# freewym/espresso

Hardware: AMD Instinct MI355X
Metric: audio-hours/sec training (LibriSpeech Conformer-12 + CTC) (higher is better)
Workload: dtype bf16

## Files before the change

### espresso_amd/csrc/engine.hip

```cpp
#include <hip/hip_runtime.h>
#include <stdint.h>
#include <stdlib.h>
#include <string.h>

#include <functional>
#include <cstdio>
#include <map>
#include <mutex>
#include <vector>

#include "espresso_amd.h"

void ea_gemm_corun_hint(int on);

namespace {

struct Arena {
  char* base;
  size_t off;
  size_t peak;
  template <typename T>
  T* get(size_t n) {
    off = (off + 255) & ~(size_t)255;
    T* p = base ? reinterpret_cast<T*>(base + off) : nullptr;
// ... 435 lines not shown

static bool keep_bits_on_side(Ctx& c, const AttnSaved& a, const EaLayerShape& sh, uint64_t seed, const EaAttnParams* w = nullptr,
                              const void* pe = nullptr) {
  if (!(a.bits && attn_fused(sh) && !c.dry && c.rc == 0 && g_flash_bits_side && side_init(c.s))) return false;
  hipEvent_t e0 = g_side.ev[g_side.next];
  g_side.next = (g_side.next + 1) % 32;
  if (hipEventRecord(e0, c.s) != hipSuccess || hipStreamWaitEvent(g_side.stream, e0, 0) != hipSuccess) c.rc = -1;
  RUN(ea_flash_keep_bits(a.bits, sh.H, sh.B, sh.T, seed + kProbs, drop_thr(sh.p_attn), g_side.stream));
  if (w && pe && sh.pos_mode != 1) {
    const int R = 2 * sh.T - 1, C = sh.C;
    G gpp(pe, w->wpos, a.pp, R, C, C, C, C, C);
    gemm_on(c, gpp, g_side.stream);
    c.pp_early = true;
  }
  return true;
}

static void attn_fwd(Ctx& c, const AttnSaved& a, const EaLayerShape& sh, const EaAttnParams& w, const void* x, void* y,
                     const int* key_len, const float* attn_mask, const void* pe, uint64_t seed) {
  const int B = sh.B, T = sh.T, C = sh.C, H = sh.H, M = B * T, dh = C / H, Z = H * B, Sp = pad8(T), R = 2 * T - 1, Rp = pad8(R);
  const float scaling = 1.0f / sqrtf((float)dh);
  Arena& sc = *c.scratch;
  const size_t mark = sc.off;
  bool bits_on_side = c.bits_early;
  c.bits_early = false;
  if (!bits_on_side) bits_on_side = keep_bits_on_side(c, a, sh, seed);
  RUN(ea_layernorm_fwd(x, w.ln_g, w.ln_b, a.xn, a.mean, a.rstd, M, C, 1e-5f, nullptr, 0, 0, 1.f, c.s));
  G gq(a.xn, w.wqkv, a.qkv, M, 3 * C, C, C, C, 3 * C);
  gq.bias(w.bqkv);
  const bool learned = sh.pos_mode == 1;
  const uint16_t* pp = learned ? (const uint16_t*)pe : a.pp;
  const uint16_t* qvv = learned ? a.qu : a.qv;
  const bool split = learned ? gq.qsplit(a.qu, nullptr, nullptr, nullptr, C, C, scaling)
                             : gq.qsplit(a.qu, a.qv, w.pos_u, w.pos_v, C, C, scaling);
  gemm(c, gq);
  if (!split) {
    if (learned) RUN(ea_relpos_q_prep(a.qkv, 3 * C, nullptr, nullptr, a.qu, nullptr, M, C, scaling, c.s));
    else RUN(ea_relpos_q_prep(a.qkv, 3 * C, w.pos_u, w.pos_v, a.qu, a.qv, M, C, scaling, c.s));
  }
  if (attn_fused(sh)) {
    if (!learned && !c.pp_early) {
      G gpp(pe, w.wpos, a.pp, R, C, C, C, C, C);
      gemm(c, gpp);
    }
    c.pp_early = false;
    if (bits_on_side) {
      hipEvent_t e1 = g_side.ev[g_side.next];
      g_side.next = (g_side.next + 1) % 32;
      if (c.rc == 0 && (hipEventRecord(e1, g_side.stream) != hipSuccess || hipStreamWaitEvent(c.s, e1, 0) != hipSuccess)) c.rc = -1;
    }
    RUN(ea_flash_attention_fwd(a.qu, qvv, C, a.qkv + C, a.qkv + 2 * C, 3 * C, pp, C, key_len, a.o, C, a.lse, H, B, T, T, dh,
                               bits_on_side ? 4 : 0, seed + kProbs, drop_thr(sh.p_attn), drop_scale(sh.p_attn), a.bits, c.s));
    G go(a.o, w.wo, y, M, C, C, C, C, C);
    go.bias(w.bo).drop(sh.p_drop, seed + kAttnOut).resid(x, C);
    gemm(c, go);
    sc.off = mark;
    return;
  }
  float* ac = sc.get<float>((size_t)Z * T * Sp);
  float* bd = sc.get<float>((size_t)Z * T * Rp);
  G gac(a.qu, a.qkv + C, ac, T, T, dh, C, 3 * C, Sp);
  gac.f32().batch(Z, B, dh, (long)T * C, dh, (long)T * 3 * C, (long)B * T * Sp, (long)T * Sp);
  gemm(c, gac);
  if (!learned) {
    G gpp(pe, w.wpos, a.pp, R, C, C, C, C, C);
    gemm(c, gpp);
  }
  G gbd(qvv, pp, bd, T, R, dh, C, C, Rp);
  gbd.f32().batch(Z, B, dh, (long)T * C, dh, 0, (long)B * T * Rp, (long)T * Rp);
  gemm(c, gbd);
  RUN(ea_relpos_softmax_fwd(ac, bd, key_len, attn_mask, a.P, sh.p_attn > 0.f ? a.Pd : nullptr, H, B, T, T, Sp, Rp, Sp, 0,
                            seed + kProbs, drop_thr(sh.p_attn), drop_scale(sh.p_attn), c.s));
  G gpv(a.Pd, a.qkv + 2 * C, a.o, T, dh, T, Sp, 3 * C, C);
  gpv.bks().batch(Z, B, (long)B * T * Sp, (long)T * Sp, dh, (long)T * 3 * C, dh, (long)T * C);
  gemm(c, gpv);
  G go(a.o, w.wo, y, M, C, C, C, C, C);
  go.bias(w.bo).drop(sh.p_drop, seed + kAttnOut).resid(x, C);
  gemm(c, go);
  sc.off = mark;
}

static void attn_bwd_tail(Ctx& c, const AttnSaved& a, const EaLayerShape& sh, const EaAttnParams& w, const EaAttnGrads& gw,
                          const void* x, const void* dy, void* dx, const void* pe, uint16_t* dqkv, uint16_t* t1, uint16_t* t2,
                          uint16_t* dBD, const uint16_t* wqkvt, const Pre& next, float* dpe, bool have_dq = false) {
  const int B = sh.B, T = sh.T, C = sh.C, H = sh.H, M = B * T, dh = C / H, R = 2 * T - 1, Rp = pad_bd(R);
  Arena& sc = *c.scratch;
  const bool learned = sh.pos_mode == 1;
  const int tiles = ((R + 127) / 128) * H;
  int sk = (768 + tiles - 1) / tiles;
  if (sk > (B * T) / 256) sk = (B * T) / 256;
  if (sk < 1) sk = 1;
  if (learned) {
    G gpp(dBD, a.qu, dpe, R, dh, B * T, Rp, C, C);
    gpp.aks().bks().f32().batch(H, 1, (long)B * T * Rp, 0, dh, 0, dh, 0);
    gpp.p.splitk = sk;
    if (sk > 1) gpp.p.workspace = sc.get<float>((size_t)sk * H * R * dh);
    if (c.df) {
      gemm(c, gpp);
    } else {
      fork(c);
      gemm_on(c, gpp, wstream(c));
    }
  } else {
    float* dppT32 = sc.get<float>((size_t)C * Rp);
    uint16_t* dppT = sc.get<uint16_t>((size_t)C * Rp);
    G gpp(a.qv, dBD, dppT32, dh, R, B * T, C, Rp, Rp);
    gpp.aks().bks().f32().batch(H, 1, dh, 0, (long)B * T * Rp, 0, (long)dh * Rp, 0);
    gpp.p.splitk = sk;
    if (sk > 1) gpp.p.workspace = sc.get<float>((size_t)sk * H * R * dh);
    const int wt_tiles = ((C + 63) / 64) * ((C + 127) / 128);
    int sk2 = (512 + wt_tiles - 1) / wt_tiles;
    if (sk2 > R / 256) sk2 = R / 256;
    if (sk2 < 1) sk2 = 1;
    G gw2(dppT, pe, gw.wpos, C, C, R, Rp, C, C);
    gw2.bks().f32().acc();
    gw2.p.splitk = sk2;
    if (sk2 > 1) gw2.p.workspace = sc.get<float>((size_t)sk2 * C * C);
    static const bool gpp_grouped = getenv("EA_GPP_SPLITK") == nullptr;
    const bool in_group = c.df && gpp_grouped && dh % 64 == 0 && c.df->grp.count + H + 3 <= EA_WGRAD_MAX;
    if (in_group) {
      for (int h = 0; h < H; ++h) {
        EaWgradProblem& q = c.df->grp.p[c.df->grp.count++];
        if (c.dry) continue;
        q.dy = a.qv + (size_t)h * dh; q.x = dBD + (size_t)h * B * T * Rp; q.dW = dppT32 + (size_t)h * dh * Rp; q.dbias = nullptr;
        q.M = B * T; q.N = dh; q.K = R; q.ld_dy = C; q.ld_x = Rp; q.ldw = Rp;
      }
      if (!c.dry) {
        const EaGemmParams p2 = gw2.p;
        const long ncast = (long)C * Rp;
        c.df->pre.push_back([=](hipStream_t st) { return hipMemsetAsync(dppT32, 0, (size_t)ncast * sizeof(float), st) == hipSuccess ? 0 : -1; });
        c.df->ops.push_back([=](hipStream_t st) {
          int rc = ea_cast_f32_to_bf16(dppT32, dppT, ncast, st);
          if (rc == 0) rc = ea_gemm_bf16(&p2, st);
          return rc;
        });
      }
    } else if (c.df) {
      if (!c.dry) {
        const EaGemmParams p1 = gpp.p, p2 = gw2.p;
        const long ncast = (long)C * Rp;
        c.df->ops.push_back([=](hipStream_t st) {
          int rc = ea_gemm_bf16(&p1, st);
          if (rc == 0) rc = ea_cast_f32_to_bf16(dppT32, dppT, ncast, st);
          if (rc == 0) rc = ea_gemm_bf16(&p2, st);
          return rc;
        });
      }
    } else {
      fork(c);
      gemm_on(c, gpp, wstream(c));
      RUN(ea_cast_f32_to_bf16(dppT32, dppT, (long)C * Rp, wstream(c)));
      gemm_on(c, gw2, wstream(c));
    }
    bias_grad(c, t1, gw.pos_u, M, C, C);
    bias_grad(c, t2, gw.pos_v, M, C, C);
  }
  if (!have_dq) RUN(ea_add2_strided_bf16(t1, C, t2, C, dqkv, 3 * C, M, C, c.s));
  fork(c);
  wgrad(c, dqkv, 3 * C, a.xn, C, gw.wqkv, M, 3 * C, C, gw.bqkv);
  uint16_t* dxn = sc.get<uint16_t>((size_t)M * C);
  dgrad(c, dqkv, w.wqkv, wqkvt, dxn, M, C, 3 * C);
  ln_bwd_block(c, x, dxn, w.ln_g, a.mean, a.rstd, dx, gw.ln_g, gw.ln_b, M, C, dy, next);
}

static void attn_bwd(Ctx& c, const AttnSaved& a, const EaLayerShape& sh, const EaAttnParams& w, const EaAttnGrads& gw, const void* x,
                     const void* dy, void* dx, const int* key_len, const void* pe, uint64_t seed, const uint16_t* wqkvt,
                     const uint16_t* wot, const uint16_t* pre, const Pre& next, float* dpe = nullptr) {
  const int B = sh.B, T = sh.T, C = sh.C, H = sh.H, M = B * T, dh = C / H, Z = H * B, Sp = pad8(T), R = 2 * T - 1, Rp = pad_bd(R);
  const float scaling = 1.0f / sqrtf((float)dh);
  Arena& sc = *c.scratch;
  const size_t mark = sc.off;
  const void* g = dy;
  if (pre) {
    g = pre;
  } else if (sh.p_drop > 0.f) {
    uint16_t* gg = sc.get<uint16_t>((size_t)M * C);
    RUN(ea_scale_dropout_bf16(dy, nullptr, gg, (long)M * C, 1.f, 0.f, seed + kAttnOut, drop_thr(sh.p_drop), drop_scale(sh.p_drop), c.s));
    g = gg;
  }
  fork(c);
  wgrad(c, g, C, a.o, C, gw.wo, M, C, C, gw.bo);
  uint16_t* dO = sc.get<uint16_t>((size_t)M * C);
  dgrad(c, g, w.wo, wot, dO, M, C, C);
  if (attn_fused(sh)) {
    uint16_t* dqkv = sc.get<uint16_t>((size_t)M * 3 * C);
    uint16_t* t1 = sc.get<uint16_t>((size_t)M * C);
    uint16_t* t2 = sc.get<uint16_t>((size_t)M * C);
    uint16_t* dBD = sc.get<uint16_t>((size_t)Z * T * Rp);
    float* Dd = sc.get<float>((size_t)Z * T);
    static const bool fused_dq = getenv("EA_NO_FUSED_DQ") == nullptr;
    RUN(ea_flash_attention_bwd(a.qu, sh.pos_mode == 1 ? a.qu : a.qv, C, a.qkv + C, a.qkv + 2 * C, 3 * C,
                               sh.pos_mode == 1 ? (const uint16_t*)pe : a.pp, C, key_len, a.o, dO, C, a.lse, Dd, t1, t2, C, dBD,
                               Rp, dqkv + C, dqkv + 2 * C, 3 * C, H, B, T, T, dh, (sh.scratch_clean && c.overlap) ? 2 : 0, scaling, seed + kProbs,
                               drop_thr(sh.p_attn),
                               drop_scale(sh.p_attn), a.bits, fused_dq ? dqkv : nullptr, 3 * C, c.s));
    attn_bwd_tail(c, a, sh, w, gw, x, dy, dx, pe, dqkv, t1, t2, dBD, wqkvt, next, dpe, fused_dq);
    release(c, mark);
    return;
  }
  float* dPd = sc.get<float>((size_t)Z * T * Sp);
  G gdp(dO, a.qkv + 2 * C, dPd, T, T, dh, C, 3 * C, Sp);
  gdp.f32().batch(Z, B, dh, (long)T * C, dh, (long)T * 3 * C, (long)B * T * Sp, (long)T * Sp);
  gemm(c, gdp);
  uint16_t* dqkv = sc.get<uint16_t>((size_t)M * 3 * C);
  G gdv(a.Pd, dO, dqkv + 2 * C, T, dh, T, Sp, C, 3 * C);
  gdv.aks().bks().batch(Z, B, (long)B * T * Sp, (long)T * Sp, dh, (long)T * C, dh, (long)T * 3 * C);
  gemm(c, gdv);
  uint16_t* dAC = sc.get<uint16_t>((size_t)Z * T * Sp);
  uint16_t* dBD = sc.get<uint16_t>((size_t)Z * T * Rp);
  RUN(ea_relpos_softmax_bwd(a.P, dPd, dAC, dBD, H, B, T, T, Sp, Sp, Rp, seed + kProbs, drop_thr(sh.p_attn), drop_scale(sh.p_attn), c.s));
  G gdk(dAC, a.qu, dqkv + C, T, dh, T, Sp, C, 3 * C);
  gdk.aks().bks().batch(Z, B, (long)B * T * Sp, (long)T * Sp, dh, (long)T * C, dh, (long)T * 3 * C);
  gemm(c, gdk);
  uint16_t* t1 = sc.get<uint16_t>((size_t)M * C);
  G gt1(dAC, a.qkv + C, t1, T, dh, T, Sp, 3 * C, C);
  gt1.bks().alpha(scaling).batch(Z, B, (long)B * T * Sp, (long)T * Sp, dh, (long)T * 3 * C, dh, (long)T * C);
  gemm(c, gt1);
  uint16_t* t2 = sc.get<uint16_t>((size_t)M * C);
  G gt2(dBD, sh.pos_mode == 1 ? (const uint16_t*)pe : a.pp, t2, T, dh, R, Rp, C, C);
  gt2.bks().alpha(scaling).batch(Z, B, (long)B * T * Rp, (long)T * Rp, dh, 0, dh, (long)T * C);
  gemm(c, gt2);
  attn_bwd_tail(c, a, sh, w, gw, x, dy, dx, pe, dqkv, t1, t2, dBD, wqkvt, next, dpe);
  release(c, mark);
}

struct BnRing {
  double* st[2] = {nullptr, nullptr};
  float* red[2] = {nullptr, nullptr};
  int si = 0, ri = 0, cap = 0;
  bool ok = false, failed = false, dirty = false;
};
static std::mutex g_bn_mu;
static std::map<std::pair<int, hipStream_t>, BnRing> g_bn_rings;
static BnRing* bn_ring(hipStream_t owner, int C) {
  int cur = 0, dev = 0;
  if (hipGetDevice(&cur) != hipSuccess) return nullptr;
  dev = cur;
  if (owner != nullptr) {
    hipDevice_t d;
    if (hipStreamGetDevice(owner, &d) == hipSuccess) dev = (int)d;
  }
  std::lock_guard<std::mutex> lk(g_bn_mu);
  BnRing& R = g_bn_rings[std::make_pair(dev, owner)];
  if (R.failed) return nullptr;
  if (!R.ok) {
    const int cap = 2048;
    if (dev != cur && hipSetDevice(dev) != hipSuccess) { R.failed = true; return nullptr; }
    const size_t bytes = 2 * (size_t)(2 * cap) * (sizeof(double) + sizeof(float));
    char* base = nullptr;
    const bool ok = hipMalloc(reinterpret_cast<void**>(&base), bytes) == hipSuccess && hipMemsetAsync(base, 0, bytes, owner) == hipSuccess;
    if (dev != cur) (void)hipSetDevice(cur);
    if (!ok) { R.failed = true; return nullptr; }
    R.st[0] = reinterpret_cast<double*>(base);
    R.st[1] = R.st[0] + 2 * cap;
    R.red[0] = reinterpret_cast<float*>(R.st[1] + 2 * cap);
    R.red[1] = R.red[0] + 2 * cap;
    R.cap = cap;
    R.ok = true;
  }
  if (C > R.cap) return nullptr;
  if (R.dirty) {
    const size_t bytes = 2 * (size_t)(2 * R.cap) * (sizeof(double) + sizeof(float));
    if (hipMemsetAsync(R.st[0], 0, bytes, owner) != hipSuccess) return nullptr;
    R.dirty = false;
  }
  return &R;
}

struct ConvSaved {
  float *mean, *rstd, *mr;
  uint16_t *xn, *Y, *U, *Z, *Hh;
};
static ConvSaved conv_saved(Arena& sv, const EaLayerShape& sh) {
  const int M = sh.B * sh.T, C = sh.C;
  ConvSaved s;
  s.mean = sv.get<float>(M);
  s.rstd = sv.get<float>(M);
  s.mr = sv.get<float>(2 * C);
  s.xn = sv.get<uint16_t>((size_t)M * C);
  s.Y = sv.get<uint16_t>((size_t)M * 2 * C);
  s.U = sv.get<uint16_t>((size_t)M * C);
  s.Z = sv.get<uint16_t>((size_t)M * C);
  s.Hh = sv.get<uint16_t>((size_t)M * C);
  return s;
}

static void conv_fwd(Ctx& c, const ConvSaved& s, const EaLayerShape& sh, const EaConvParams& w, const void* x, void* y, uint64_t seed) {
  const int B = sh.B, T = sh.T, C = sh.C, M = B * T;
  Arena& sc = *c.scratch;
  const size_t mark = sc.off;
  RUN(ea_layernorm_fwd(x, w.ln_g, w.ln_b, s.xn, s.mean, s.rstd, M, C, 1e-5f, nullptr, 0, 0, 1.f, c.s));
  G g1(s.xn, w.pw1, s.Y, M, 2 * C, C, C, C, 2 * C);
  gemm(c, g1);
  static const bool bn_fused = getenv("EA_BN_UNFUSED") == nullptr;
  const bool ring = sh.training && bn_fused && C <= 2048;
  BnRing* R = nullptr;
  if (ring && !c.dry && c.rc == 0 && !(R = bn_ring(c.s, C))) c.rc = -1;
  double* stats = nullptr;
  if (sh.training && !ring) {
    stats = sc.get<double>(2 * C);
    if (!c.dry && c.rc == 0) c.rc = hipMemsetAsync(stats, 0, 2 * C * sizeof(double), c.s) == hipSuccess ? 0 : -1;
  }
  if (R && c.rc == 0) stats = R->st[R->si];
  RUN(ea_glu_dwconv_fwd(s.Y, w.dw, s.U, s.Z, stats, B, T, C, sh.KW, c.s));
  if (ring) {
    if (R) {
      if (c.rc == 0) RUN(ea_bn_act_fwd_train(s.Z, stats, s.mr, w.bn_rm, w.bn_rv, w.bn_g, w.bn_b, s.Hh, M, C, EA_ACT_SILU, (float)M, 1e-5f, 0.1f,
                                             R->st[R->si ^ 1], 2 * R->cap, c.s));
      if (c.rc == 0) R->si ^= 1;
      else R->dirty = true;
    }
  } else {
    if (sh.training) RUN(ea_bn_finalize(stats, s.mr, w.bn_rm, w.bn_rv, C, (float)M, 1e-5f, 0.1f, c.s));
    else RUN(ea_bn_from_running(w.bn_rm, w.bn_rv, s.mr, C, 1e-5f, c.s));
    RUN(ea_bn_act_fwd(s.Z, s.mr, w.bn_g, w.bn_b, s.Hh, M, C, EA_ACT_SILU, c.s));
  }
  G g2(s.Hh, w.pw2, y, M, C, C, C, C, C);
  g2.drop(sh.p_drop, seed + kConvOut).resid(x, C);
  gemm(c, g2);
  sc.off = mark;
}

static void conv_bwd(Ctx& c, const ConvSaved& s, const EaLayerShape& sh, const EaConvParams& w, const EaConvGrads& gw, const void* x,
                     const void* dy, void* dx, uint64_t seed, const uint16_t* pw1t, const uint16_t* pw2t, const uint16_t* pre,
                     const Pre& next) {
  const int B = sh.B, T = sh.T, C = sh.C, M = B * T;
  Arena& sc = *c.scratch;
  const size_t mark = sc.off;
  const void* g = dy;
  if (pre) {
    g = pre;
  } else if (sh.p_drop > 0.f) {
    uint16_t* gg = sc.get<uint16_t>((size_t)M * C);
    RUN(ea_scale_dropout_bf16(dy, nullptr, gg, (long)M * C, 1.f, 0.f, seed + kConvOut, drop_thr(sh.p_drop), drop_scale(sh.p_drop), c.s));
    g = gg;
  }
  fork(c);
  wgrad(c, g, C, s.Hh, C, gw.pw2, M, C, C);
  uint16_t* dH = sc.get<uint16_t>((size_t)M * C);
  dgrad(c, g, w.pw2, pw2t, dH, M, C, C);
  static const bool bn_fused = getenv("EA_BN_UNFUSED") == nullptr;
  const bool ring = bn_fused && C <= 2048;
  BnRing* R = nullptr;
  if (ring && !c.dry && c.rc == 0 && !(R = bn_ring(c.s, C))) c.rc = -1;
  float* red = nullptr;
  if (!ring) {
    red = sc.get<float>(2 * C);
    if (!c.dry && c.rc == 0) c.rc = hipMemsetAsync(red, 0, 2 * C * sizeof(float), c.s) == hipSuccess ? 0 : -1;
  }
// ... 670 lines not shown
```

### espresso_amd/csrc/flash_attention.hip

```cpp
#include "common.h"
#include "espresso_amd.h"
#include "flash_internal.h"

namespace {

typedef short bf16x4_t __attribute__((ext_vector_type(4)));

constexpr int DH = 64;
constexpr int TQ = 64, TK = 64;
constexpr int ROWB = DH * 2;
constexpr int BDP = 18;

__device__ __forceinline__ uint32_t off16(int row, int chunk) { return (uint32_t)(row * ROWB + ((chunk ^ (row & 7)) << 4)); }




__device__ __forceinline__ int xcd_remap(int id, int total) {
  const int xcd = id & 7, q = total >> 3, r = total & 7;
  return (xcd < r ? xcd * (q + 1) : r * (q + 1) + (xcd - r) * q) + (id >> 3);
}

template <int NP>
struct RowRegs { uint4 v[NP]; };
template <int NP>
__device__ __forceinline__ void load_rows(RowRegs<NP>& r, const bf16_t* src, long ld, int row0, int limit, int tid) {
#pragma unroll
  for (int p = 0; p < NP; ++p) {
    const int g = row0 + (tid >> 3) + 32 * p;
    r.v[p] = make_uint4(0, 0, 0, 0);
    if (g >= 0 && g < limit) r.v[p] = *reinterpret_cast<const uint4*>(src + (long)g * ld + (tid & 7) * 8);
  }
}
template <int NP>
__device__ __forceinline__ void store_rows(char* s, const RowRegs<NP>& r, int tid) {
#pragma unroll
  for (int p = 0; p < NP; ++p) *reinterpret_cast<uint4*>(s + off16((tid >> 3) + 32 * p, tid & 7)) = r.v[p];
}
struct BlkRegs { uint4 v[4]; };
__device__ __forceinline__ void load_blk(BlkRegs& r, const bf16_t* src, long ld, int row0, int limit, int t) {
#pragma unroll
  for (int jj = 0; jj < 4; ++jj) {
    const int g = row0 + (t >> 3) * 4 + jj;
    r.v[jj] = make_uint4(0, 0, 0, 0);
    if (g >= 0 && g < limit) r.v[jj] = *reinterpret_cast<const uint4*>(src + (long)g * ld + (t & 7) * 8);
  }
}
__device__ __forceinline__ void store_blk_rows(char* s, const BlkRegs& r, int t) {
#pragma unroll
  for (int jj = 0; jj < 4; ++jj) *reinterpret_cast<uint4*>(s + off16((t >> 3) * 4 + jj, t & 7)) = r.v[jj];
}
template <int NR>
__device__ __forceinline__ void store_blk_t(char* s, const BlkRegs& r, int t) {
  const int rq = t >> 3, dc = t & 7;
  const uint32_t w[4][4] = {{r.v[0].x, r.v[0].y, r.v[0].z, r.v[0].w}, {r.v[1].x, r.v[1].y, r.v[1].z, r.v[1].w},
                            {r.v[2].x, r.v[2].y, r.v[2].z, r.v[2].w}, {r.v[3].x, r.v[3].y, r.v[3].z, r.v[3].w}};
#pragma unroll
  for (int q = 0; q < 4; ++q) {
    uint2 lo, hi;
    lo.x = (w[0][q] & 0xffffu) | (w[1][q] << 16);
    lo.y = (w[2][q] & 0xffffu) | (w[3][q] << 16);
    hi.x = (w[0][q] >> 16) | (w[1][q] & 0xffff0000u);
    hi.y = (w[2][q] >> 16) | (w[3][q] & 0xffff0000u);
    const int d = dc * 8 + 2 * q;
    *reinterpret_cast<uint2*>(s + d * (NR * 2) + ((rq ^ (d & 15)) << 3)) = lo;
    *reinterpret_cast<uint2*>(s + (d + 1) * (NR * 2) + ((rq ^ ((d + 1) & 15)) << 3)) = hi;
  }
}
template <int NR>
__device__ __forceinline__ bf16x4_t read_t(const char* s, int d, int chunk) {
  return *reinterpret_cast<const bf16x4_t*>(s + d * (NR * 2) + ((chunk ^ (d & 15)) << 3));
}

__device__ __forceinline__ f32x4_t mfma32(bf16x8_t a, bf16x8_t b, f32x4_t c) {
  return __builtin_amdgcn_mfma_f32_16x16x32_bf16(__builtin_bit_cast(__attribute__((ext_vector_type(8))) __bf16, a),
                                                 __builtin_bit_cast(__attribute__((ext_vector_type(8))) __bf16, b), c, 0, 0, 0);
}
__device__ __forceinline__ f32x4_t mfma16(bf16x4_t a, bf16x4_t b, f32x4_t c) {
  return __builtin_amdgcn_mfma_f32_16x16x16bf16_1k(a, b, c, 0, 0, 0);
}

template <bool RELPOS>
__global__ __launch_bounds__(256, 2) void flash_fwd_kernel(const FlashFwdArgs a) {
  __shared__ __attribute__((aligned(16))) char sK[TK * ROWB];
  __shared__ __attribute__((aligned(16))) char sVt[DH * ROWB];
  __shared__ __attribute__((aligned(16))) char sPP[RELPOS ? 128 * ROWB : 16];
  __shared__ float sBD[RELPOS ? 4 * 80 * BDP : 1];

  const int tid = threadIdx.x, lane = tid & 63, w = tid >> 6;
  const int li = lane & 15, g4 = lane >> 4;
  const int vid = xcd_remap(blockIdx.x, gridDim.x);
  const int z = vid / a.nq, qt = vid % a.nq;
  const int h = z / a.B, b = z % a.B;
  const int T = a.T, S = a.S;
  const int i0 = qt * TQ;
  const int i = i0 + 16 * w + li;
  const int kl = a.klen ? min(a.klen[b], S) : S;

  bf16x8_t qu[2], qv[2];
#pragma unroll
  for (int ks = 0; ks < 2; ++ks) {
    uint4 u = make_uint4(0, 0, 0, 0), v = make_uint4(0, 0, 0, 0);
    if (i < T) {
      const long o = ((long)b * T + i) * a.ldq + h * DH + ks * 32 + g4 * 8;
      u = *reinterpret_cast<const uint4*>(a.qu + o);
      if (RELPOS) v = *reinterpret_cast<const uint4*>(a.qv + o);
    }
    qu[ks] = __builtin_bit_cast(bf16x8_t, u);
    qv[ks] = __builtin_bit_cast(bf16x8_t, v);
  }

  f32x4_t acc_o[4];
#pragma unroll
  for (int dt = 0; dt < 4; ++dt) acc_o[dt] = (f32x4_t){0.f, 0.f, 0.f, 0.f};
  float m_run = -INFINITY, l_run = 0.f;

  const bf16_t* Kb = a.k + (long)b * S * a.ldkv + h * DH;
  const bf16_t* Vb = a.v + (long)b * S * a.ldkv + h * DH;
  const bf16_t* PPb = RELPOS ? a.pp + h * DH : nullptr;
  const int R = 2 * T - 1;
  float* bd = sBD + (RELPOS ? w * 80 * BDP : 0);
  const int c0w = 48 - 16 * w;

  int jend = kl;
  if (a.causal) jend = min(jend, i0 + TQ + (S - T));
  RowRegs<2> rK;
  BlkRegs rV;
  RowRegs<4> rP;
  auto load_tile = [&](int j0) {
    load_rows<2>(rK, Kb, a.ldkv, j0, S, tid);
    if (tid < 128) load_blk(rV, Vb, a.ldkv, j0, S, tid);
    if (RELPOS) load_rows<4>(rP, PPb, a.ldpp, (T - 1) - (i0 + TQ - 1) + j0, R, tid);
  };
  if (jend > 0) load_tile(0);
  for (int j0 = 0; j0 < jend; j0 += TK) {
    __syncthreads();
    store_rows<2>(sK, rK, tid);
    if (tid < 128) store_blk_t<64>(sVt, rV, tid);
    if (RELPOS) store_rows<4>(sPP, rP, tid);
    __syncthreads();
    if (j0 + TK < jend) load_tile(j0 + TK);

    f32x4_t acc_s[4];
#pragma unroll
    for (int jt = 0; jt < 4; ++jt) acc_s[jt] = (f32x4_t){0.f, 0.f, 0.f, 0.f};
#pragma unroll
    for (int ks = 0; ks < 2; ++ks)
#pragma unroll
      for (int jt = 0; jt < 4; ++jt) {
        const bf16x8_t kf = *reinterpret_cast<const bf16x8_t*>(sK + off16(jt * 16 + li, ks * 4 + g4));
        acc_s[jt] = mfma32(kf, qu[ks], acc_s[jt]);
      }
    if (RELPOS) {
#pragma unroll
      for (int ct = 0; ct < 5; ++ct) {
// ... 364 lines not shown
  if (j0 >= kl) ibeg = T;
  BlkRegs rQ;
  RowRegs<2> rQv;
  RowRegs<4> rP;
  float rLse = 0.f, rD = 0.f;
  auto load_tile = [&](int i0) {
    if (tid < 128) load_blk(rQ, Qub, a.ldq, i0, T, tid);
    else load_blk(rQ, dOb, a.ldo, i0, T, tid - 128);
    if (RELPOS) {
      load_rows<2>(rQv, Qvb, a.ldq, i0, T, tid);
      load_rows<4>(rP, PPb, a.ldpp, (T - 1) - (i0 + TQ - 1) + j0, R, tid);
    }
    if (tid < TQ) {
      const int ii = i0 + tid;
      rLse = ii < T ? a.lse[(long)z * T + ii] : 0.f;
      rD = ii < T ? a.D[(long)z * T + ii] : 0.f;
    }
  };
  if (ibeg < T) load_tile(ibeg);
  for (int i0 = ibeg; i0 < T; i0 += TQ) {
    __syncthreads();
    if (tid < 128) {
      store_blk_rows(sQu, rQ, tid);
      store_blk_t<64>(sQut, rQ, tid);
    } else {
      store_blk_rows(sdO, rQ, tid - 128);
      store_blk_t<64>(sdOt, rQ, tid - 128);
    }
    if (RELPOS) {
      store_rows<2>(sQv, rQv, tid);
      store_rows<4>(sPP, rP, tid);
    }
    if (tid < TQ) {
      sLse[tid] = rLse;
      sD[tid] = rD;
    }
    __syncthreads();
    if (i0 + TQ < T) load_tile(i0 + TQ);

#pragma unroll
    for (int it = 0; it < 4; ++it) {
      f32x4_t s = (f32x4_t){0.f, 0.f, 0.f, 0.f}, dp = s;
#pragma unroll
      for (int ks = 0; ks < 2; ++ks) {
        const bf16x8_t qf = *reinterpret_cast<const bf16x8_t*>(sQu + off16(it * 16 + li, ks * 4 + g4));
        s = mfma32(qf, kf[ks], s);
        const bf16x8_t gf = *reinterpret_cast<const bf16x8_t*>(sdO + off16(it * 16 + li, ks * 4 + g4));
        dp = mfma32(gf, vf[ks], dp);
      }
      if (RELPOS) {
        const int cbase = 48 - 16 * it + 16 * w;
        wave_lds_sync();
#pragma unroll
        for (int ct = 0; ct < 2; ++ct) {
          f32x4_t t = (f32x4_t){0.f, 0.f, 0.f, 0.f};
#pragma unroll
          for (int ks = 0; ks < 2; ++ks) {
            const bf16x8_t qf = *reinterpret_cast<const bf16x8_t*>(sQv + off16(it * 16 + li, ks * 4 + g4));
            const bf16x8_t pf = *reinterpret_cast<const bf16x8_t*>(sPP + off16(cbase + ct * 16 + li, ks * 4 + g4));
            t = mfma32(qf, pf, t);
          }
#pragma unroll
          for (int r = 0; r < 4; ++r) bd[(g4 * 4 + r) * 33 + ct * 16 + li] = t[r];
        }
        wave_lds_sync();
#pragma unroll
        for (int r = 0; r < 4; ++r) s[r] += bd[(g4 * 4 + r) * 33 + 15 - (g4 * 4 + r) + li];
      }
      float ps[4], dsv[4];
#pragma unroll
      for (int r = 0; r < 4; ++r) {
        const int il = it * 16 + g4 * 4 + r;
        const int i = i0 + il;
        const bool masked = j >= kl || i >= T || (a.causal && j > i + (S - T));
        const float p = masked ? 0.f : __expf(s[r] - sLse[il]);
        float keep = 1.f;
        if (a.thr) keep = ea_keep(a.seed, ((uint64_t)z * T + (uint64_t)i) * (uint64_t)S + (uint64_t)j, a.thr, a.inv_keep);
        ps[r] = p * keep;
        dsv[r] = p * (dp[r] * keep - sD[il]);
      }
      const bf16x4_t pb = pack4(ps[0], ps[1], ps[2], ps[3]);
      const bf16x4_t db = pack4(dsv[0], dsv[1], dsv[2], dsv[3]);
#pragma unroll
      for (int dt = 0; dt < 4; ++dt) {
        acc_dv[dt] = mfma16(read_t<64>(sdOt, dt * 16 + li, it * 4 + g4), pb, acc_dv[dt]);
        acc_dk[dt] = mfma16(read_t<64>(sQut, dt * 16 + li, it * 4 + g4), db, acc_dk[dt]);
      }
    }
  }
  if (j < S) {
    bf16_t* ok = a.dk + ((long)b * S + j) * a.lddkv + h * DH;
    bf16_t* ov = a.dv + ((long)b * S + j) * a.lddkv + h * DH;
#pragma unroll
    for (int dt = 0; dt < 4; ++dt) {
      uint2 pk;
      pk.x = pack_bf2(acc_dk[dt][0], acc_dk[dt][1]);
      pk.y = pack_bf2(acc_dk[dt][2], acc_dk[dt][3]);
      *reinterpret_cast<uint2*>(ok + dt * 16 + g4 * 4) = pk;
      pk.x = pack_bf2(acc_dv[dt][0], acc_dv[dt][1]);
      pk.y = pack_bf2(acc_dv[dt][2], acc_dv[dt][3]);
      *reinterpret_cast<uint2*>(ov + dt * 16 + g4 * 4) = pk;
    }
  }
}

}

extern "C" int ea_flash_attention_supported(int dh, int T, int S, int relpos) {
  return dh == DH && T > 0 && S > 0 && (!relpos || T == S);
}

extern "C" long ea_flash_keep_bits_bytes(int H, int B, int T) {
  const long nkt = (T + TK - 1) / TK;
  return (long)H * B * nkt * (nkt * 64) * 4 * (long)sizeof(uint16_t);
}

extern "C" int ea_flash_keep_bits(void* keep_bits, int H, int B, int T, uint64_t drop_seed, uint32_t drop_thr, hipStream_t stream) {
  if (H <= 0 || B <= 0 || T <= 0 || !keep_bits) return keep_bits ? 0 : -2;
  return ea_rp_keep_bits((uint16_t*)keep_bits, H, B, T, drop_seed, drop_thr, stream);
}

extern "C" int ea_flash_attention_fwd(const void* qu, const void* qv, long ldq, const void* k, const void* v, long ldkv,
                                      const void* pp, long ldpp, const int* key_len, void* out, long ldo, float* lse, int H,
                                      int B, int T, int S, int dh, int causal, uint64_t drop_seed, uint32_t drop_thr,
                                      float drop_scale, void* keep_bits, hipStream_t stream) {
  if (H <= 0 || B <= 0 || T <= 0) return 0;
  const bool relpos = qv != nullptr;
  if (!ea_flash_attention_supported(dh, T, S, relpos) || (relpos && !pp)) return -2;
  if ((ldq | ldkv | ldo) % 8 || (relpos && ldpp % 8)) return -2;
  if ((((uintptr_t)qu | (uintptr_t)qv | (uintptr_t)k | (uintptr_t)v | (uintptr_t)pp) & 15) || ((uintptr_t)out & 7)) return -2;
  FlashFwdArgs a;
  a.qu = (const bf16_t*)qu; a.qv = (const bf16_t*)qv; a.ldq = ldq;
  a.k = (const bf16_t*)k; a.v = (const bf16_t*)v; a.ldkv = ldkv;
  a.pp = (const bf16_t*)pp; a.ldpp = ldpp;
  a.klen = key_len;
  a.out = (bf16_t*)out; a.ldo = ldo;
  a.lse = lse;
  a.H = H; a.B = B; a.T = T; a.S = S; a.causal = causal & 1; a.nq = (T + TQ - 1) / TQ;
  a.seed = drop_seed; a.thr = drop_thr; a.inv_keep = drop_scale;
  a.bits = (const uint16_t*)keep_bits;
  if (ea_rp_eligible(relpos, T, S, causal, drop_thr, keep_bits)) {
    if (drop_thr && !(causal & 4)) {
      const int rc = ea_rp_keep_bits((uint16_t*)keep_bits, H, B, T, drop_seed, drop_thr, stream);
      if (rc) return rc;
    }
    return ea_rp_fwd(a, stream);
  }
  const dim3 grid((unsigned)(a.nq * H * B));
  if (relpos) hipLaunchKernelGGL(flash_fwd_kernel<true>, grid, dim3(256), 0, stream, a);
  else hipLaunchKernelGGL(flash_fwd_kernel<false>, grid, dim3(256), 0, stream, a);
  return EA_CHECK_LAUNCH();
}

extern "C" int ea_flash_attention_bwd(const void* qu, const void* qv, long ldq, const void* k, const void* v, long ldkv,
                                      const void* pp, long ldpp, const int* key_len, const void* out, const void* dout, long ldo,
                                      const float* lse, float* D, void* t1, void* t2, long ldt, void* dBD, int ld_bd, void* dk,
                                      void* dv, long lddkv, int H, int B, int T, int S, int dh, int causal, float scaling,
                                      uint64_t drop_seed, uint32_t drop_thr, float drop_scale, const void* keep_bits,
                                      void* dq, long lddq, hipStream_t stream) {
  if (H <= 0 || B <= 0 || T <= 0) return 0;
  const bool relpos = qv != nullptr;
  if (!ea_flash_attention_supported(dh, T, S, relpos)) return -2;
  if (relpos && (!pp || !t2 || !dBD || ld_bd < 2 * T - 1 || ld_bd % 8 || ((uintptr_t)dBD & 15))) return -2;
  if ((ldq | ldkv | ldo | ldt | lddkv) % 8 || (relpos && ldpp % 8)) return -2;
  if (((uintptr_t)qu | (uintptr_t)qv | (uintptr_t)k | (uintptr_t)v | (uintptr_t)pp | (uintptr_t)out | (uintptr_t)dout) & 15) return -2;
  if (((uintptr_t)t1 | (uintptr_t)t2 | (uintptr_t)dk | (uintptr_t)dv | (uintptr_t)dq) & 7) return -2;
  if (dq && (!relpos || lddq % 4)) return -2;
  FlashBwdArgs a;
  a.qu = (const bf16_t*)qu; a.qv = (const bf16_t*)qv; a.ldq = ldq;
  a.k = (const bf16_t*)k; a.v = (const bf16_t*)v; a.ldkv = ldkv;
  a.pp = (const bf16_t*)pp; a.ldpp = ldpp;
  a.klen = key_len;
  a.out = (const bf16_t*)out; a.dout = (const bf16_t*)dout; a.ldo = ldo;
  a.lse = lse; a.D = D;
  a.t1 = (bf16_t*)t1; a.t2 = (bf16_t*)t2; a.ldt = ldt;
  a.dq = (bf16_t*)dq; a.lddq = lddq;
  a.dBD = (bf16_t*)dBD; a.ld_bd = ld_bd;
  a.dk = (bf16_t*)dk; a.dv = (bf16_t*)dv; a.lddkv = lddkv;
  a.H = H; a.B = B; a.T = T; a.S = S; a.causal = causal & 1; a.dbd_prezeroed = (causal >> 1) & 1;
  a.nq = (T + TQ - 1) / TQ; a.nk = (S + TK - 1) / TK;
  a.scaling = scaling;
  a.seed = drop_seed; a.thr = drop_thr; a.inv_keep = drop_scale;
  a.bits = (const uint16_t*)keep_bits;
  if (ea_rp_eligible(relpos, T, S, causal, drop_thr, keep_bits)) return ea_rp_bwd(a, stream);
  const dim3 gq((unsigned)(a.nq * H * B)), gk((unsigned)(a.nk * H * B));
  if (relpos) {
    hipLaunchKernelGGL(flash_bwd_q_kernel<true>, gq, dim3(256), 0, stream, a);
    hipLaunchKernelGGL(flash_bwd_kv_kernel<true>, gk, dim3(256), 0, stream, a);
  } else {
    hipLaunchKernelGGL(flash_bwd_q_kernel<false>, gq, dim3(256), 0, stream, a);
    hipLaunchKernelGGL(flash_bwd_kv_kernel<false>, gk, dim3(256), 0, stream, a);
  }
  return EA_CHECK_LAUNCH();
}
```

### espresso_amd/csrc/flash_internal.h

```cpp
#pragma once
#include "common.h"

struct FlashFwdArgs {
  const bf16_t* qu; const bf16_t* qv; long ldq;
  const bf16_t* k; const bf16_t* v; long ldkv;
  const bf16_t* pp; long ldpp;
  const int* klen;
  bf16_t* out; long ldo;
  float* lse;
  int H, B, T, S, causal, nq;
  uint64_t seed; uint32_t thr; float inv_keep;
  const uint16_t* bits;
};

struct FlashBwdArgs {
  const bf16_t* qu; const bf16_t* qv; long ldq;
  const bf16_t* k; const bf16_t* v; long ldkv;
  const bf16_t* pp; long ldpp;
  const int* klen;
  const bf16_t* out; const bf16_t* dout; long ldo;
  const float* lse;
  float* D;
  bf16_t* t1; bf16_t* t2; long ldt;
  bf16_t* dq; long lddq;
  bf16_t* dBD; int ld_bd;
  bf16_t* dk; bf16_t* dv; long lddkv;
  int H, B, T, S, causal, nq, nk, dbd_prezeroed;
  float scaling;
  uint64_t seed; uint32_t thr; float inv_keep;
  const uint16_t* bits;
  unsigned long long* prof;
  int dbg;
};

bool ea_rp_eligible(bool relpos, int T, int S, int causal, uint32_t thr, const void* bits);
int ea_rp_keep_bits(uint16_t* bits, int H, int B, int T, uint64_t seed, uint32_t thr, hipStream_t stream);
int ea_rp_fwd(const FlashFwdArgs& a, hipStream_t stream);
int ea_rp_bwd(const FlashBwdArgs& a, hipStream_t stream);
```

### espresso_amd/csrc/flash_relpos.hip

```cpp
#include "flash_internal.h"

namespace {

typedef short bf16x4_t __attribute__((ext_vector_type(4)));
typedef const __attribute__((address_space(1))) void* gptr_t;
typedef __attribute__((address_space(3))) void* lptr_t;
typedef __attribute__((address_space(3))) bf16x4_t* lds_b4_t;

constexpr int DH = 64, TQ = 64, TK = 64;
constexpr int IMG = 64 * 128;
constexpr int BDP = 18;
constexpr int BNC = 80 * BDP * 4;
constexpr int OBP = 88;
constexpr int PP_OFF = 4 * IMG, BNC_OFF = 7 * IMG;
constexpr int LDS_BYTES = 7 * IMG + 4 * BNC;
constexpr int AUX_OFF = LDS_BYTES;
constexpr int LDS_BYTES_KV = LDS_BYTES + 1024;
constexpr float LOG2E = 1.4426950408889634f;

__device__ __forceinline__ int swz(int r) { return ((r >> 2) & 1) | (((r >> 1) & 1) << 1) | ((((r >> 2) ^ (r >> 3)) & 1) << 2); }

__device__ __forceinline__ int xcd_remap(int id, int total) {
  const int xcd = id & 7, q = total >> 3, r = total & 7;
  return (xcd < r ? xcd * (q + 1) : r * (q + 1) + (xcd - r) * q) + (id >> 3);
}
__device__ __forceinline__ f32x4_t mfma32(bf16x8_t a, bf16x8_t b, f32x4_t c) {
  return __builtin_amdgcn_mfma_f32_16x16x32_bf16(__builtin_bit_cast(__attribute__((ext_vector_type(8))) __bf16, a),
                                                 __builtin_bit_cast(__attribute__((ext_vector_type(8))) __bf16, b), c, 0, 0, 0);
}
__device__ __forceinline__ f32x4_t mfma16(bf16x4_t a, bf16x4_t b, f32x4_t c) {
  return __builtin_amdgcn_mfma_f32_16x16x16bf16_1k(a, b, c, 0, 0, 0);
}
__device__ __forceinline__ bf16x8_t cat(bf16x4_t lo, bf16x4_t hi) { return __builtin_shufflevector(lo, hi, 0, 1, 2, 3, 4, 5, 6, 7); }
__device__ __forceinline__ bf16x4_t pack4(float a, float b, float c, float d) {
  uint2 pk;
  pk.x = pack_bf2(a, b);
  pk.y = pack_bf2(c, d);
  return __builtin_bit_cast(bf16x4_t, pk);
}
__device__ __forceinline__ uint32_t lds_addr(const void* p) { return (uint32_t)(uintptr_t)p; }
template <int O0, int O1, int O2, int O3>
__device__ __forceinline__ void trr16(const uint32_t (&ad)[4], uint2 (&o)[16]) {
  asm volatile(
      "ds_read_b64_tr_b16 %0, %16 offset:%20\n\tds_read_b64_tr_b16 %1, %16 offset:%21\n\t"
      "ds_read_b64_tr_b16 %2, %16 offset:%22\n\tds_read_b64_tr_b16 %3, %16 offset:%23\n\t"
      "ds_read_b64_tr_b16 %4, %17 offset:%20\n\tds_read_b64_tr_b16 %5, %17 offset:%21\n\t"
      "ds_read_b64_tr_b16 %6, %17 offset:%22\n\tds_read_b64_tr_b16 %7, %17 offset:%23\n\t"
      "ds_read_b64_tr_b16 %8, %18 offset:%20\n\tds_read_b64_tr_b16 %9, %18 offset:%21\n\t"
      "ds_read_b64_tr_b16 %10, %18 offset:%22\n\tds_read_b64_tr_b16 %11, %18 offset:%23\n\t"
      "ds_read_b64_tr_b16 %12, %19 offset:%20\n\tds_read_b64_tr_b16 %13, %19 offset:%21\n\t"
      "ds_read_b64_tr_b16 %14, %19 offset:%22\n\tds_read_b64_tr_b16 %15, %19 offset:%23\n\t"
      "s_waitcnt lgkmcnt(0)"
      : "=&v"(o[0]), "=&v"(o[1]), "=&v"(o[2]), "=&v"(o[3]), "=&v"(o[4]), "=&v"(o[5]), "=&v"(o[6]), "=&v"(o[7]), "=&v"(o[8]),
        "=&v"(o[9]), "=&v"(o[10]), "=&v"(o[11]), "=&v"(o[12]), "=&v"(o[13]), "=&v"(o[14]), "=&v"(o[15])
      : "v"(ad[0]), "v"(ad[1]), "v"(ad[2]), "v"(ad[3]), "i"(O0), "i"(O1), "i"(O2), "i"(O3)
      : "memory");
}
template <int O0, int O1, int O2, int O3>
__device__ __forceinline__ void trr8(const uint32_t (&ad)[2], uint2 (&o)[8]) {
  asm volatile(
      "ds_read_b64_tr_b16 %0, %8 offset:%10\n\tds_read_b64_tr_b16 %1, %8 offset:%11\n\t"
      "ds_read_b64_tr_b16 %2, %8 offset:%12\n\tds_read_b64_tr_b16 %3, %8 offset:%13\n\t"
      "ds_read_b64_tr_b16 %4, %9 offset:%10\n\tds_read_b64_tr_b16 %5, %9 offset:%11\n\t"
      "ds_read_b64_tr_b16 %6, %9 offset:%12\n\tds_read_b64_tr_b16 %7, %9 offset:%13\n\t"
      "s_waitcnt lgkmcnt(0)"
      : "=&v"(o[0]), "=&v"(o[1]), "=&v"(o[2]), "=&v"(o[3]), "=&v"(o[4]), "=&v"(o[5]), "=&v"(o[6]), "=&v"(o[7])
      : "v"(ad[0]), "v"(ad[1]), "i"(O0), "i"(O1), "i"(O2), "i"(O3)
      : "memory");
}
__device__ __forceinline__ void trr20(const uint32_t (&ad)[20], uint2 (&o)[20]) {
  asm volatile(
      "ds_read_b64_tr_b16 %0, %20\n\tds_read_b64_tr_b16 %1, %21\n\tds_read_b64_tr_b16 %2, %22\n\tds_read_b64_tr_b16 %3, %23\n\t"
      "ds_read_b64_tr_b16 %4, %24\n\tds_read_b64_tr_b16 %5, %25\n\tds_read_b64_tr_b16 %6, %26\n\tds_read_b64_tr_b16 %7, %27\n\t"
      "ds_read_b64_tr_b16 %8, %28\n\tds_read_b64_tr_b16 %9, %29\n\tds_read_b64_tr_b16 %10, %30\n\tds_read_b64_tr_b16 %11, %31\n\t"
      "ds_read_b64_tr_b16 %12, %32\n\tds_read_b64_tr_b16 %13, %33\n\tds_read_b64_tr_b16 %14, %34\n\tds_read_b64_tr_b16 %15, %35\n\t"
      "ds_read_b64_tr_b16 %16, %36\n\tds_read_b64_tr_b16 %17, %37\n\tds_read_b64_tr_b16 %18, %38\n\tds_read_b64_tr_b16 %19, %39\n\t"
      "s_waitcnt lgkmcnt(0)"
      : "=&v"(o[0]), "=&v"(o[1]), "=&v"(o[2]), "=&v"(o[3]), "=&v"(o[4]), "=&v"(o[5]), "=&v"(o[6]), "=&v"(o[7]), "=&v"(o[8]),
        "=&v"(o[9]), "=&v"(o[10]), "=&v"(o[11]), "=&v"(o[12]), "=&v"(o[13]), "=&v"(o[14]), "=&v"(o[15]), "=&v"(o[16]),
        "=&v"(o[17]), "=&v"(o[18]), "=&v"(o[19])
      : "v"(ad[0]), "v"(ad[1]), "v"(ad[2]), "v"(ad[3]), "v"(ad[4]), "v"(ad[5]), "v"(ad[6]), "v"(ad[7]), "v"(ad[8]), "v"(ad[9]),
        "v"(ad[10]), "v"(ad[11]), "v"(ad[12]), "v"(ad[13]), "v"(ad[14]), "v"(ad[15]), "v"(ad[16]), "v"(ad[17]), "v"(ad[18]),
        "v"(ad[19])
      : "memory");
}
__device__ __forceinline__ uint2 lds_u2(const char* p) {
  const float* f = reinterpret_cast<const float*>(p);
  return make_uint2(__float_as_uint(f[0]), __float_as_uint(f[1]));
}
__device__ __forceinline__ bf16x8_t cat2(uint2 lo, uint2 hi) {
  return __builtin_bit_cast(bf16x8_t, make_uint4(lo.x, lo.y, hi.x, hi.y));
}
__device__ __forceinline__ void tr_image(const char* img, const uint32_t (&tro)[4], bf16x8_t (&f)[8]) {
  const uint32_t b = lds_addr(img);
  const uint32_t ad[4] = {b + tro[0], b + tro[1], b + tro[2], b + tro[3]};
  uint2 o[16];
  trr16<0, 2048, 4096, 6144>(ad, o);
#pragma unroll
  for (int dt = 0; dt < 4; ++dt) {
    f[dt * 2 + 0] = cat2(o[dt * 4 + 0], o[dt * 4 + 1]);
    f[dt * 2 + 1] = cat2(o[dt * 4 + 2], o[dt * 4 + 3]);
  }
}
__device__ __forceinline__ bf16x8_t ldf(const char* p) { return *reinterpret_cast<const bf16x8_t*>(p); }
__device__ __forceinline__ void wave_lds_sync() {
  __builtin_amdgcn_fence(__ATOMIC_RELEASE, "wavefront");
  __builtin_amdgcn_wave_barrier();
  __builtin_amdgcn_fence(__ATOMIC_ACQUIRE, "wavefront");
}
__device__ __forceinline__ float fexp2(float x) { return __builtin_amdgcn_exp2f(x); }

#ifdef RP_PROF
#define PROF_DECL unsigned long long prof_t = __builtin_amdgcn_s_memtime(); unsigned prof_acc[10] = {0, 0, 0, 0, 0, 0, 0, 0, 0, 0};
#define PROF_MARK(k) { const unsigned long long n_ = __builtin_amdgcn_s_memtime(); prof_acc[k] += (unsigned)(n_ - prof_t); prof_t = n_; }
#define PROF_DUMP(kern) if (a.prof && (threadIdx.x & 63) == 0) { unsigned long long* o_ = a.prof + ((long)(kern) * 8192 + (long)blockIdx.x * 4 + (threadIdx.x >> 6)) * 10; for (int k_ = 0; k_ < 10; ++k_) o_[k_] = prof_acc[k_]; }
#else
#define PROF_DECL
#define PROF_MARK(k)
#define PROF_DUMP(kern)
#endif

struct LaneK {
  int lane, w, li, g4;
  uint32_t offk[2];
  uint32_t tro[4];
  uint32_t bd_w;
  uint32_t bd_r;
};
__device__ __forceinline__ LaneK lane_consts() {
  LaneK L;
  const int tid = threadIdx.x;
  L.lane = tid & 63;
  L.w = __builtin_amdgcn_readfirstlane(tid >> 6);
  L.li = L.lane & 15;
  L.g4 = L.lane >> 4;
#pragma unroll
  for (int ks = 0; ks < 2; ++ks) L.offk[ks] = L.li * 128 + (((ks * 4 + L.g4) ^ swz(L.li)) << 4);
  const int rowl = 4 * L.g4 + (L.li >> 2);
#pragma unroll
  for (int dt = 0; dt < 4; ++dt)
    L.tro[dt] = rowl * 128 + (((dt * 2 + ((L.li & 3) >> 1)) ^ swz(rowl)) << 4) + (L.li & 1) * 8;
  L.bd_w = (L.g4 * 4) * BDP + L.li;
  L.bd_r = (15 - L.li + L.g4 * 4) * BDP + L.li;
  return L;
}

struct ImgSrc {
  const bf16_t* p[2];
  long ld;
  int rmax;
};
__device__ __forceinline__ ImgSrc img_src(const bf16_t* base, long ld, int rmax, int w, int lane) {
  ImgSrc s;
  s.ld = ld;
  s.rmax = rmax;
#pragma unroll
  for (int n = 0; n < 2; ++n) {
    const int r = (w + 4 * n) * 8 + (lane >> 3);
    s.p[n] = base + (long)r * ld + (((lane & 7) ^ swz(r)) << 3);
  }
  return s;
}
__device__ __forceinline__ void issue_img(char* dst, const ImgSrc& s, int row0, int w, int lane) {
  if (row0 >= 0 && row0 + 63 <= s.rmax) {
    const long off = (long)row0 * s.ld;
#pragma unroll
    for (int n = 0; n < 2; ++n)
      __builtin_amdgcn_global_load_lds((gptr_t)(s.p[n] + off), (lptr_t)(dst + (w + 4 * n) * 1024), 16, 0, 0);
  } else {
#pragma unroll
    for (int n = 0; n < 2; ++n) {
      const int r = (w + 4 * n) * 8 + (lane >> 3);
      const int g = min(max(row0 + r, 0), s.rmax);
      __builtin_amdgcn_global_load_lds((gptr_t)(s.p[n] + (long)(g - r) * s.ld), (lptr_t)(dst + (w + 4 * n) * 1024), 16, 0, 0);
    }
  }
}

__device__ __forceinline__ void add_band(f32x4_t (&acc_s)[4], const bf16x8_t (&qv)[2], const char* blk_lo, const char* blk_hi,
                                         float* bd, const LaneK& L) {
  bf16x8_t pf[2][2];
  auto frag = [&](int ct, bf16x8_t (&f)[2]) {
    const int q = ct - L.w + 3;
    const char* p = ((q >> 2) ? blk_hi : blk_lo) + (q & 3) * 2048;
    f[0] = ldf(p + L.offk[0]);
    f[1] = ldf(p + L.offk[1]);
  };
  frag(0, pf[0]);
#pragma unroll
  for (int ct = 0; ct < 5; ++ct) {
    if (ct + 1 < 5) frag(ct + 1, pf[(ct + 1) & 1]);
    f32x4_t t = (f32x4_t){0.f, 0.f, 0.f, 0.f};
    t = mfma32(pf[ct & 1][0], qv[0], t);
    t = mfma32(pf[ct & 1][1], qv[1], t);
#pragma unroll
    for (int r = 0; r < 4; ++r) bd[L.bd_w + (ct * 16 + r) * BDP] = t[r];
    if (ct >= 1) {
      const int jt = ct - 1;
#pragma unroll
      for (int r = 0; r < 4; ++r) acc_s[jt][r] += bd[L.bd_r + (jt * 16 + r) * BDP];
    }
  }
}

__device__ __forceinline__ uint32_t keep_mask(uint32_t piece, int k) { return (uint32_t)__builtin_amdgcn_sbfe((int)piece, k, 1); }
__device__ __forceinline__ float fand(float x, uint32_t m) { return __uint_as_float(__float_as_uint(x) & m); }

__global__ __launch_bounds__(256) void keep_bits_kernel(uint16_t* bits, uint64_t seed, uint32_t thr, int Z, int T, int nkt) {
  const int Tpad = nkt * 64;
  const long n = (long)Z * nkt * Tpad * 4;
  const long stride = (long)gridDim.x * 256;
  for (long id = (long)blockIdx.x * 256 + threadIdx.x; id < n; id += stride) {
    const int g = (int)(id & 3);
    long t = id >> 2;
    const int i = (int)(t % Tpad);
    t /= Tpad;
    const int kt = (int)(t % nkt);
    const int z = (int)(t / nkt);
    uint32_t piece = 0;
    if (i < T) {
      const uint64_t rowbase = ((uint64_t)z * T + (uint64_t)i) * (uint64_t)T;
#pragma unroll
      for (int jt = 0; jt < 4; ++jt)
#pragma unroll
        for (int r = 0; r < 4; ++r) {
          const int j = kt * 64 + jt * 16 + g * 4 + r;
          if (j < T && ea_hash(seed, rowbase + (uint64_t)j) >= thr) piece |= 1u << (jt * 4 + r);
        }
    }
    bits[id] = (uint16_t)piece;
  }
}

template <bool DROP>
__global__ __launch_bounds__(256, 2) void rp_fwd_kernel(const FlashFwdArgs a) {
  __shared__ __attribute__((aligned(16))) char lds[LDS_BYTES];
  const LaneK L = lane_consts();
  const int lane = L.lane, w = L.w, li = L.li, g4 = L.g4;
  const int vid = xcd_remap(blockIdx.x, gridDim.x);
  const int z = vid / a.nq, qt = vid % a.nq;
  const int h = z / a.B, b = z % a.B;
  const int T = a.T;
  const int i0 = qt * TQ;
  const int i = i0 + 16 * w + li;
  const int kl = a.klen ? min(a.klen[b], T) : T;
  const int nt = (kl + TK - 1) / TK;
  const int nkt = (T + TK - 1) / TK;

  bf16x8_t qu[2], qv[2];
  {
    const int ic = min(i, T - 1);
    const long o = ((long)b * T + ic) * a.ldq + h * DH + g4 * 8;
#pragma unroll
    for (int ks = 0; ks < 2; ++ks) {
      qu[ks] = __builtin_bit_cast(bf16x8_t, *reinterpret_cast<const uint4*>(a.qu + o + ks * 32));
      qv[ks] = __builtin_bit_cast(bf16x8_t, *reinterpret_cast<const uint4*>(a.qv + o + ks * 32));
    }
  }
  const bf16_t* Kb = a.k + (long)b * T * a.ldkv + h * DH;
  const bf16_t* Vb = a.v + (long)b * T * a.ldkv + h * DH;
  const bf16_t* PPb = a.pp + h * DH;
  const int R = 2 * T - 1;
  const ImgSrc srcK = img_src(Kb, a.ldkv, T - 1, w, lane), srcV = img_src(Vb, a.ldkv, T - 1, w, lane);
  const ImgSrc srcP = img_src(PPb, a.ldpp, R - 1, w, lane);
  const int pbase = (T - 1) - (i0 + TQ - 1);
  float* bd = reinterpret_cast<float*>(lds + BNC_OFF + w * BNC);
  const uint32_t* bitp = DROP ? reinterpret_cast<const uint32_t*>(a.bits) + (((long)z * nkt) * (nkt * 64) + i) * 2 + (g4 >> 1) : nullptr;
  const long bit_step = (long)nkt * 64 * 2;
  const int ksh = (g4 & 1) * 16;

  f32x4_t acc_o[4];
#pragma unroll
  for (int dt = 0; dt < 4; ++dt) acc_o[dt] = (f32x4_t){0.f, 0.f, 0.f, 0.f};
  float m_run = -INFINITY, l_run = 0.f;
  uint32_t piece = 0, piece_next = 0;

  if (nt > 0) {
    issue_img(lds, srcK, 0, w, lane);
    issue_img(lds + IMG, srcV, 0, w, lane);
    issue_img(lds + PP_OFF, srcP, pbase, w, lane);
    issue_img(lds + PP_OFF + IMG, srcP, pbase + 64, w, lane);
    if (DROP) piece_next = bitp[0];
  }
  int slot_lo = 0;
  for (int t = 0; t < nt; ++t) {
    const int j0 = t * TK;
    asm volatile("s_waitcnt vmcnt(0)" ::: "memory");
    __builtin_amdgcn_s_barrier();
    const int slot_hi = slot_lo == 2 ? 0 : slot_lo + 1;
    const int slot_nx = slot_hi == 2 ? 0 : slot_hi + 1;
    if (DROP) {
      piece = piece_next;
      asm volatile("" : "+v"(piece));
    }
    if (t + 1 < nt) {
      if (DROP) piece_next = bitp[(long)(t + 1) * bit_step];
      char* st = lds + ((t + 1) & 1) * 2 * IMG;
      issue_img(st, srcK, j0 + TK, w, lane);
      issue_img(st + IMG, srcV, j0 + TK, w, lane);
      issue_img(lds + PP_OFF + slot_nx * IMG, srcP, pbase + 64 * (t + 2), w, lane);
    }
    const char* sK = lds + (t & 1) * 2 * IMG;
    const char* sV = sK + IMG;

    f32x4_t acc_s[4];
#pragma unroll
    for (int jt = 0; jt < 4; ++jt) acc_s[jt] = (f32x4_t){0.f, 0.f, 0.f, 0.f};
    {
      bf16x8_t fr[2][2];
      fr[0][0] = ldf(sK + L.offk[0]);
      fr[0][1] = ldf(sK + L.offk[1]);
#pragma unroll
      for (int jt = 0; jt < 4; ++jt) {
        if (jt + 1 < 4) {
          fr[(jt + 1) & 1][0] = ldf(sK + (jt + 1) * 2048 + L.offk[0]);
          fr[(jt + 1) & 1][1] = ldf(sK + (jt + 1) * 2048 + L.offk[1]);
        }
        acc_s[jt] = mfma32(fr[jt & 1][0], qu[0], acc_s[jt]);
        acc_s[jt] = mfma32(fr[jt & 1][1], qu[1], acc_s[jt]);
      }
    }
    add_band(acc_s, qv, lds + PP_OFF + slot_lo * IMG, lds + PP_OFF + slot_hi * IMG, bd, L);

    if (j0 + TK > kl) {
#pragma unroll
      for (int jt = 0; jt < 4; ++jt)
#pragma unroll
        for (int r = 0; r < 4; ++r)
          if (j0 + jt * 16 + g4 * 4 + r >= kl) acc_s[jt][r] = -INFINITY;
    }
    float tmax = fmaxf(fmaxf(acc_s[0][0], acc_s[0][1]), fmaxf(acc_s[0][2], acc_s[0][3]));
#pragma unroll
    for (int jt = 1; jt < 4; ++jt) tmax = fmaxf(tmax, fmaxf(fmaxf(acc_s[jt][0], acc_s[jt][1]), fmaxf(acc_s[jt][2], acc_s[jt][3])));
    tmax = fmaxf(tmax, __shfl_xor(tmax, 16, 64));
    tmax = fmaxf(tmax, __shfl_xor(tmax, 32, 64));
    const float m_new = fmaxf(m_run, tmax);
    const float msc = (m_new == -INFINITY) ? 0.f : m_new * LOG2E;
    const float alpha = fexp2(m_run * LOG2E - msc);
    float psum = 0.f;
#pragma unroll
    for (int jt = 0; jt < 4; ++jt)
#pragma unroll
      for (int r = 0; r < 4; ++r) {
        const float p = fexp2(fmaf(acc_s[jt][r], LOG2E, -msc));
        psum += p;
        acc_s[jt][r] = DROP ? fand(p, keep_mask(piece, ksh + jt * 4 + r)) : p;
      }
    l_run = l_run * alpha + psum;
    m_run = m_new;
#pragma unroll
    for (int dt = 0; dt < 4; ++dt)
#pragma unroll
      for (int r = 0; r < 4; ++r) acc_o[dt][r] *= alpha;

    {
      bf16x8_t vf[8];
      tr_image(sV, L.tro, vf);
#pragma unroll
      for (int kb = 0; kb < 2; ++kb) {
        const bf16x8_t pb = cat(pack4(acc_s[2 * kb][0], acc_s[2 * kb][1], acc_s[2 * kb][2], acc_s[2 * kb][3]),
                                pack4(acc_s[2 * kb + 1][0], acc_s[2 * kb + 1][1], acc_s[2 * kb + 1][2], acc_s[2 * kb + 1][3]));
#pragma unroll
        for (int dt = 0; dt < 4; ++dt) acc_o[dt] = mfma32(vf[dt * 2 + kb], pb, acc_o[dt]);
      }
    }
    slot_lo = slot_hi;
  }

  l_run += __shfl_xor(l_run, 16, 64);
  l_run += __shfl_xor(l_run, 32, 64);
  if (i < T) {
    const float inv = (DROP ? a.inv_keep : 1.f) / l_run;
    bf16_t* o = a.out + ((long)b * T + i) * a.ldo + h * DH;
#pragma unroll
    for (int dt = 0; dt < 4; ++dt) {
      uint2 pk;
      pk.x = pack_bf2(acc_o[dt][0] * inv, acc_o[dt][1] * inv);
      pk.y = pack_bf2(acc_o[dt][2] * inv, acc_o[dt][3] * inv);
      *reinterpret_cast<uint2*>(o + dt * 16 + g4 * 4) = pk;
    }
    if (a.lse && g4 == 0) a.lse[(long)z * T + i] = m_run + __logf(l_run);
  }
}

template <bool DROP, bool WANT_PD>
__device__ __forceinline__ void softmax_bwd_tile(f32x4_t (&acc_s)[4], const f32x4_t (&acc_dp)[4], bf16x4_t (&dsb)[4], bf16x4_t (&pdb)[4],
                                                 float lse2, float Di, float inv_keep, uint32_t piece, int ksh, int jrel_end, int g4) {
#pragma unroll
  for (int jt = 0; jt < 4; ++jt) {
    float ds[4], pd[4];
#pragma unroll
    for (int r = 0; r < 4; ++r) {
      float p = fexp2(fmaf(acc_s[jt][r], LOG2E, -lse2));
      if (jrel_end < 64 && jt * 16 + g4 * 4 + r >= jrel_end) p = 0.f;
      float dp = acc_dp[jt][r];
      if (DROP) {
        const uint32_t m = keep_mask(piece, ksh + jt * 4 + r);
        dp = fand(dp * inv_keep, m);
        if (WANT_PD) pd[r] = fand(p * inv_keep, m);
      } else if (WANT_PD) {
        pd[r] = p;
      }
      ds[r] = p * (dp - Di);
    }
    dsb[jt] = pack4(ds[0], ds[1], ds[2], ds[3]);
    if (WANT_PD) pdb[jt] = pack4(pd[0], pd[1], pd[2], pd[3]);
  }
}

template <bool DROP>
__global__ __launch_bounds__(256, 2) void rp_bwd_q_kernel(const FlashBwdArgs a) {
  __shared__ __attribute__((aligned(16))) char lds[LDS_BYTES];
  const LaneK L = lane_consts();
  const int lane = L.lane, w = L.w, li = L.li, g4 = L.g4;
  const int vid = xcd_remap(blockIdx.x, gridDim.x);
  const int z = vid / a.nq, qt = vid % a.nq;
  const int h = z / a.B, b = z % a.B;
  const int T = a.T;
  const int i0 = qt * TQ;
  const int i = i0 + 16 * w + li;
  const int kl = a.klen ? min(a.klen[b], T) : T;
  const int nt = (kl + TK - 1) / TK;
  const int nkt = (T + TK - 1) / TK;

  bf16x8_t qu[2], qv[2], dO[2];
  float Di = 0.f;
  {
    const int ic = min(i, T - 1);
    const long oq = ((long)b * T + ic) * a.ldq + h * DH + g4 * 8;
    const long oo = ((long)b * T + ic) * a.ldo + h * DH + g4 * 8;
#pragma unroll
    for (int ks = 0; ks < 2; ++ks) {
      qu[ks] = __builtin_bit_cast(bf16x8_t, *reinterpret_cast<const uint4*>(a.qu + oq + ks * 32));
      qv[ks] = __builtin_bit_cast(bf16x8_t, *reinterpret_cast<const uint4*>(a.qv + oq + ks * 32));
      const uint4 g = *reinterpret_cast<const uint4*>(a.dout + oo + ks * 32);
      const uint4 o = *reinterpret_cast<const uint4*>(a.out + oo + ks * 32);
      dO[ks] = __builtin_bit_cast(bf16x8_t, g);
      const uint32_t wg[4] = {g.x, g.y, g.z, g.w}, wo[4] = {o.x, o.y, o.z, o.w};
#pragma unroll
      for (int e = 0; e < 4; ++e)
        Di += __uint_as_float(wg[e] << 16) * __uint_as_float(wo[e] << 16) +
              __uint_as_float(wg[e] & 0xffff0000u) * __uint_as_float(wo[e] & 0xffff0000u);
    }
  }
  Di += __shfl_xor(Di, 16, 64);
  Di += __shfl_xor(Di, 32, 64);
  const float lse2 = (i < T) ? a.lse[(long)z * T + i] * LOG2E : INFINITY;
  if (i < T && g4 == 0 && a.D) a.D[(long)z * T + i] = Di;

  f32x4_t acc_t1[4], acc_t2[4];
#pragma unroll
  for (int dt = 0; dt < 4; ++dt) {
    acc_t1[dt] = (f32x4_t){0.f, 0.f, 0.f, 0.f};
    acc_t2[dt] = (f32x4_t){0.f, 0.f, 0.f, 0.f};
  }
  const bf16_t* Kb = a.k + (long)b * T * a.ldkv + h * DH;
  const bf16_t* Vb = a.v + (long)b * T * a.ldkv + h * DH;
  const bf16_t* PPb = a.pp + h * DH;
  const int R = 2 * T - 1;
  const ImgSrc srcK = img_src(Kb, a.ldkv, T - 1, w, lane), srcV = img_src(Vb, a.ldkv, T - 1, w, lane);
  const ImgSrc srcP = img_src(PPb, a.ldpp, R - 1, w, lane);
  const int pbase = (T - 1) - (i0 + TQ - 1);
  float* bd = reinterpret_cast<float*>(lds + BNC_OFF + w * BNC);
  bf16_t* ob = reinterpret_cast<bf16_t*>(bd);
  const uint32_t* bitp = DROP ? reinterpret_cast<const uint32_t*>(a.bits) + (((long)z * nkt) * (nkt * 64) + i) * 2 + (g4 >> 1) : nullptr;
  const long bit_step = (long)nkt * 64 * 2;
  const int ksh = (g4 & 1) * 16;
  uint2 mlo, mhi;
  {
    uint32_t m[4], n[4];
#pragma unroll
    for (int e = 0; e < 4; ++e) {
      m[e] = (4 * g4 + e >= 15 - li) ? 0xffffu : 0u;
      n[e] = (64 + 4 * g4 + e <= 78 - li) ? 0xffffu : 0u;
    }
    mlo = make_uint2(m[0] | (m[1] << 16), m[2] | (m[3] << 16));
    mhi = make_uint2(n[0] | (n[1] << 16), n[2] | (n[3] << 16));
  }
  const int ob_w = li * (OBP - 1) + 15 + g4 * 4;
  const char* ob_rd = reinterpret_cast<const char*>(ob) + li * (OBP * 2) + g4 * 8;

  uint32_t piece = 0, piece_next = 0;
  int jcov = 0;
  uint32_t dbd_pk[8];
  int dbd_j0 = -1;
  auto store_dbd = [&]() {
    const int j = dbd_j0 + lane;
    if (dbd_j0 >= 0 && j < T) {
      const int row_w = i0 + 16 * w, nrow = T - row_w;
      bf16_t* dp = a.dBD + ((long)z * T + row_w) * a.ld_bd + (T - 1 - row_w) + j;
      if (nrow >= 16) {
#pragma unroll
        for (int iw = 0; iw < 16; ++iw) dp[(long)iw * (a.ld_bd - 1)] = (bf16_t)(dbd_pk[iw >> 1] >> (16 * (iw & 1)));
      } else {
#pragma unroll
        for (int iw = 0; iw < 16; ++iw)
          if (iw < nrow) dp[(long)iw * (a.ld_bd - 1)] = (bf16_t)(dbd_pk[iw >> 1] >> (16 * (iw & 1)));
      }
    }
  };
  if (nt > 0) {
    issue_img(lds, srcK, 0, w, lane);
    issue_img(lds + IMG, srcV, 0, w, lane);
    issue_img(lds + PP_OFF, srcP, pbase, w, lane);
    issue_img(lds + PP_OFF + IMG, srcP, pbase + 64, w, lane);
    if (DROP) piece_next = bitp[0];
  }
  int slot_lo = 0;
  PROF_DECL
  for (int t = 0; t < nt; ++t) {
    const int j0 = t * TK;
    jcov = min(T, j0 + TK);
    PROF_MARK(9)
    asm volatile("s_waitcnt vmcnt(0)" ::: "memory");
    __builtin_amdgcn_s_barrier();
    PROF_MARK(0)
    store_dbd();
    const int slot_hi = slot_lo == 2 ? 0 : slot_lo + 1;
    const int slot_nx = slot_hi == 2 ? 0 : slot_hi + 1;
    if (DROP) {
      piece = piece_next;
      asm volatile("" : "+v"(piece));
    }
    if (t + 1 < nt) {
      if (DROP) piece_next = bitp[(long)(t + 1) * bit_step];
      char* st = lds + ((t + 1) & 1) * 2 * IMG;
      issue_img(st, srcK, j0 + TK, w, lane);
      issue_img(st + IMG, srcV, j0 + TK, w, lane);
      issue_img(lds + PP_OFF + slot_nx * IMG, srcP, pbase + 64 * (t + 2), w, lane);
    }
    PROF_MARK(1)
    const char* sK = lds + (t & 1) * 2 * IMG;
    const char* sV = sK + IMG;
    const char* blk_lo = lds + PP_OFF + slot_lo * IMG;
    const char* blk_hi = lds + PP_OFF + slot_hi * IMG;

    f32x4_t acc_s[4], acc_dp[4];
#pragma unroll
    for (int jt = 0; jt < 4; ++jt) {
      acc_s[jt] = (f32x4_t){0.f, 0.f, 0.f, 0.f};
      acc_dp[jt] = (f32x4_t){0.f, 0.f, 0.f, 0.f};
    }
    {
      bf16x8_t fr[2][4];
      auto frag = [&](int jt, bf16x8_t (&f)[4]) {
        f[0] = ldf(sK + jt * 2048 + L.offk[0]);
        f[1] = ldf(sK + jt * 2048 + L.offk[1]);
        f[2] = ldf(sV + jt * 2048 + L.offk[0]);
        f[3] = ldf(sV + jt * 2048 + L.offk[1]);
      };
      frag(0, fr[0]);
#pragma unroll
      for (int jt = 0; jt < 4; ++jt) {
        if (jt + 1 < 4) frag(jt + 1, fr[(jt + 1) & 1]);
        acc_s[jt] = mfma32(fr[jt & 1][0], qu[0], acc_s[jt]);
        acc_dp[jt] = mfma32(fr[jt & 1][2], dO[0], acc_dp[jt]);
        acc_s[jt] = mfma32(fr[jt & 1][1], qu[1], acc_s[jt]);
        acc_dp[jt] = mfma32(fr[jt & 1][3], dO[1], acc_dp[jt]);
      }
    }
    PROF_MARK(2)
    add_band(acc_s, qv, blk_lo, blk_hi, bd, L);
    PROF_MARK(3)
    bf16x4_t dsb[4], pdb[4];
    softmax_bwd_tile<DROP, false>(acc_s, acc_dp, dsb, pdb, lse2, Di, a.inv_keep, piece, ksh, kl - j0, g4);
    PROF_MARK(4)

    if (!(a.dbg & 4)) {
      bf16x8_t kf[8];
      tr_image(sK, L.tro, kf);
#pragma unroll
      for (int kb = 0; kb < 2; ++kb) {
        const bf16x8_t db = cat(dsb[2 * kb], dsb[2 * kb + 1]);
#pragma unroll
        for (int dt = 0; dt < 4; ++dt) acc_t1[dt] = mfma32(kf[dt * 2 + kb], db, acc_t1[dt]);
      }
    }
    PROF_MARK(5)
    wave_lds_sync();
#pragma unroll
    for (int jt = 0; jt < 4; ++jt) {
      const uint2 pk = __builtin_bit_cast(uint2, dsb[jt]);
      ob[ob_w + jt * 16 + 0] = (bf16_t)(pk.x & 0xffffu);
      ob[ob_w + jt * 16 + 1] = (bf16_t)(pk.x >> 16);
      ob[ob_w + jt * 16 + 2] = (bf16_t)(pk.y & 0xffffu);
      ob[ob_w + jt * 16 + 3] = (bf16_t)(pk.y >> 16);
    }
    wave_lds_sync();
    if (!(a.dbg & 2)) {
      uint32_t ad[20];
      uint2 pf[20];
#pragma unroll
      for (int q16 = 0; q16 < 5; ++q16) {
        const int qq = q16 - w + 3;
        const uint32_t pbk = lds_addr(((qq >> 2) ? blk_hi : blk_lo) + (qq & 3) * 2048);
#pragma unroll
        for (int dt = 0; dt < 4; ++dt) ad[q16 * 4 + dt] = pbk + L.tro[dt];
      }
      trr20(ad, pf);
#pragma unroll
      for (int cb = 0; cb < 2; ++cb) {
        uint2 blo = lds_u2(ob_rd + cb * 64);
        const uint2 bhi = lds_u2(ob_rd + cb * 64 + 32);
        if (cb == 0) {
          blo.x &= mlo.x;
          blo.y &= mlo.y;
        }
        const bf16x8_t db = cat2(blo, bhi);
#pragma unroll
        for (int dt = 0; dt < 4; ++dt) acc_t2[dt] = mfma32(cat2(pf[(2 * cb) * 4 + dt], pf[(2 * cb + 1) * 4 + dt]), db, acc_t2[dt]);
      }
      uint2 bl = lds_u2(ob_rd + 128);
      bl.x &= mhi.x;
      bl.y &= mhi.y;
#pragma unroll
      for (int dt = 0; dt < 4; ++dt)
        acc_t2[dt] = mfma16(__builtin_bit_cast(bf16x4_t, pf[16 + dt]), __builtin_bit_cast(bf16x4_t, bl), acc_t2[dt]);
    }
    PROF_MARK(6)
    if (!(a.dbg & 1)) {
      const bf16_t* bs = ob + 15 + lane;
#pragma unroll
      for (int k = 0; k < 8; ++k)
        dbd_pk[k] = (uint32_t)bs[(2 * k) * (OBP - 1)] | ((uint32_t)bs[(2 * k + 1) * (OBP - 1)] << 16);
      dbd_j0 = j0;
    }
    wave_lds_sync();
    slot_lo = slot_hi;
    PROF_MARK(7)
  }
  store_dbd();

  if (i < T) {
    bf16_t* o1 = a.t1 + ((long)b * T + i) * a.ldt + h * DH;
    bf16_t* o2 = a.t2 + ((long)b * T + i) * a.ldt + h * DH;
#pragma unroll
    for (int dt = 0; dt < 4; ++dt) {
      uint2 pk;
      pk.x = pack_bf2(acc_t1[dt][0] * a.scaling, acc_t1[dt][1] * a.scaling);
      pk.y = pack_bf2(acc_t1[dt][2] * a.scaling, acc_t1[dt][3] * a.scaling);
      *reinterpret_cast<uint2*>(o1 + dt * 16 + g4 * 4) = pk;
      pk.x = pack_bf2(acc_t2[dt][0] * a.scaling, acc_t2[dt][1] * a.scaling);
      pk.y = pack_bf2(acc_t2[dt][2] * a.scaling, acc_t2[dt][3] * a.scaling);
      *reinterpret_cast<uint2*>(o2 + dt * 16 + g4 * 4) = pk;
    }
    if (a.dq) {
      bf16_t* oq = a.dq + ((long)b * T + i) * a.lddq + h * DH;
#pragma unroll
      for (int dt = 0; dt < 4; ++dt) {
        uint2 pk;
        pk.x = pack_bf2((acc_t1[dt][0] + acc_t2[dt][0]) * a.scaling, (acc_t1[dt][1] + acc_t2[dt][1]) * a.scaling);
        pk.y = pack_bf2((acc_t1[dt][2] + acc_t2[dt][2]) * a.scaling, (acc_t1[dt][3] + acc_t2[dt][3]) * a.scaling);
        *reinterpret_cast<uint2*>(oq + dt * 16 + g4 * 4) = pk;
      }
    }
  }
  PROF_MARK(9)
  if (!a.dbd_prezeroed) {
    for (int iw = 0; iw < 16; ++iw) {
      const int row = i0 + 16 * w + iw;
      if (row >= T) break;
      const int lo = T - 1 - row, hi = lo + jcov;
      bf16_t* dr = a.dBD + ((long)z * T + row) * a.ld_bd;
      for (int c = lane; c * 8 < a.ld_bd; c += 64) {
        const int e0 = c * 8;
        if (e0 + 8 <= lo || e0 >= hi) {
          *reinterpret_cast<uint4*>(dr + e0) = make_uint4(0, 0, 0, 0);
        } else if (e0 < lo || e0 + 8 > hi) {
#pragma unroll
          for (int e = 0; e < 8; ++e)
            if (e0 + e < lo || e0 + e >= hi) dr[e0 + e] = 0;
        }
      }
    }
  }
  PROF_MARK(8)
  PROF_DUMP(0)
}

template <bool DROP>
__global__ __launch_bounds__(256, 2) void rp_bwd_kv_kernel(const FlashBwdArgs a) {
  __shared__ __attribute__((aligned(16))) char lds[LDS_BYTES_KV];
  const LaneK L = lane_consts();
  const int lane = L.lane, w = L.w, li = L.li, g4 = L.g4;
  const int vid = xcd_remap(blockIdx.x, gridDim.x);
  const int z = vid / a.nk, kt = vid % a.nk;
  const int h = z / a.B, b = z % a.B;
  const int T = a.T;
  const int j0 = kt * TK;
  const int kl = a.klen ? min(a.klen[b], T) : T;
  const int nq = (j0 < kl) ? a.nq : 0;
  const int nkt = a.nk;

  bf16x8_t kf[4][2], vf[4][2];
#pragma unroll
  for (int jt = 0; jt < 4; ++jt) {
    const int j = min(j0 + jt * 16 + li, T - 1);
    const long o = ((long)b * T + j) * a.ldkv + h * DH + g4 * 8;
#pragma unroll
    for (int ks = 0; ks < 2; ++ks) {
      kf[jt][ks] = __builtin_bit_cast(bf16x8_t, *reinterpret_cast<const uint4*>(a.k + o + ks * 32));
      vf[jt][ks] = __builtin_bit_cast(bf16x8_t, *reinterpret_cast<const uint4*>(a.v + o + ks * 32));
    }
  }
  f32x4_t acc_dk[4], acc_dv[4];
#pragma unroll
  for (int dt = 0; dt < 4; ++dt) {
    acc_dk[dt] = (f32x4_t){0.f, 0.f, 0.f, 0.f};
    acc_dv[dt] = (f32x4_t){0.f, 0.f, 0.f, 0.f};
  }
  const bf16_t* Qub = a.qu + (long)b * T * a.ldq + h * DH;
  const bf16_t* Qvb = a.qv + (long)b * T * a.ldq + h * DH;
  const bf16_t* dOb = a.dout + (long)b * T * a.ldo + h * DH;
  const bf16_t* PPb = a.pp + h * DH;
  const int R = 2 * T - 1;
  const ImgSrc srcQ = img_src(Qub, a.ldq, T - 1, w, lane), srcG = img_src(dOb, a.ldo, T - 1, w, lane);
  const ImgSrc srcP = img_src(PPb, a.ldpp, R - 1, w, lane);
  const int pb0 = (T - 1) - (TQ - 1) + j0;
  float* bd = reinterpret_cast<float*>(lds + BNC_OFF + w * BNC);
  char* exw = lds + BNC_OFF + w * BNC;
  const uint32_t exo = li * 128 + ((((g4 >> 1) ^ swz(li))) << 4) + (g4 & 1) * 8;
  uint32_t exr[2], trk[2];
#pragma unroll
  for (int hh = 0; hh < 2; ++hh) {
    const int rl = 8 * (g4 & 1) + 4 * hh + (li >> 2);
    exr[hh] = (g4 >> 1) * BNC + rl * 128 + (((2 * w + ((li & 3) >> 1)) ^ swz(rl)) << 4) + (li & 1) * 8;
    const int rr = 8 * g4 + 4 * hh + (li >> 2);
    trk[hh] = rr * 128 + ((((li & 3) >> 1) ^ swz(rr)) << 4) + (li & 1) * 8;
  }
  const char* exbase = lds + BNC_OFF;
  const uint32_t* bitp = DROP ? reinterpret_cast<const uint32_t*>(a.bits) + (((long)z * nkt + kt) * (nkt * 64) + 16 * w + li) * 2 + (g4 >> 1) : nullptr;
  const int ksh = (g4 & 1) * 16;

  bf16x8_t qv[2], qv_next[2];
  uint32_t piece_next = 0;
  auto row_loads = [&](int i0, int stage) {
    const int i = i0 + 16 * w + li;
    const int ic = min(i, T - 1);
    const long o = (long)ic * a.ldq + g4 * 8;
    qv_next[0] = __builtin_bit_cast(bf16x8_t, *reinterpret_cast<const uint4*>(Qvb + o));
    qv_next[1] = __builtin_bit_cast(bf16x8_t, *reinterpret_cast<const uint4*>(Qvb + o + 32));
    if (DROP) piece_next = bitp[(long)i0 * 2];
    if (w < 2) {
      const float* src = (w == 0 ? a.lse : a.D) + (long)z * T + min(i0 + lane, T - 1);
      __builtin_amdgcn_global_load_lds((gptr_t)src, (lptr_t)(lds + AUX_OFF + stage * 512 + w * 256), 4, 0, 0);
    }
  };
  if (nq > 0) {
    issue_img(lds, srcQ, 0, w, lane);
    issue_img(lds + IMG, srcG, 0, w, lane);
    issue_img(lds + PP_OFF, srcP, pb0, w, lane);
    issue_img(lds + PP_OFF + 2 * IMG, srcP, pb0 + 64, w, lane);
    row_loads(0, 0);
  }
  int slot_lo = 0;
  PROF_DECL
  for (int it = 0; it < nq; ++it) {
    const int i0 = it * TQ;
    PROF_MARK(9)
    asm volatile("s_waitcnt vmcnt(0)" ::: "memory");
    __builtin_amdgcn_s_barrier();
    PROF_MARK(0)
    const int slot_hi = slot_lo == 0 ? 2 : slot_lo - 1;
    const int slot_nx = slot_lo == 2 ? 0 : slot_lo + 1;
    qv[0] = qv_next[0];
    qv[1] = qv_next[1];
    const float* aux = reinterpret_cast<const float*>(lds + AUX_OFF + (it & 1) * 512) + 16 * w + li;
    const float lse_raw = aux[0], Di = aux[64];
    uint32_t piece = piece_next;
    {
      uint4 q0 = __builtin_bit_cast(uint4, qv[0]), q1 = __builtin_bit_cast(uint4, qv[1]);
      asm volatile("" : "+v"(q0.x), "+v"(q0.y), "+v"(q0.z), "+v"(q0.w), "+v"(q1.x), "+v"(q1.y), "+v"(q1.z), "+v"(q1.w), "+v"(piece));
      qv[0] = __builtin_bit_cast(bf16x8_t, q0);
      qv[1] = __builtin_bit_cast(bf16x8_t, q1);
    }
    const float lse2 = (i0 + 16 * w + li < T) ? lse_raw * LOG2E : INFINITY;
    if (it + 1 < nq) {
      row_loads(i0 + TQ, (it + 1) & 1);
      char* st = lds + ((it + 1) & 1) * 2 * IMG;
      issue_img(st, srcQ, i0 + TQ, w, lane);
      issue_img(st + IMG, srcG, i0 + TQ, w, lane);
      issue_img(lds + PP_OFF + slot_nx * IMG, srcP, pb0 - 64 * (it + 1), w, lane);
    }
    PROF_MARK(1)
    const char* sQ = lds + (it & 1) * 2 * IMG;
    const char* sG = sQ + IMG;
    bf16x8_t qu[2], dO[2];
#pragma unroll
    for (int ks = 0; ks < 2; ++ks) {
      qu[ks] = ldf(sQ + w * 2048 + L.offk[ks]);
      dO[ks] = ldf(sG + w * 2048 + L.offk[ks]);
    }
    f32x4_t acc_s[4], acc_dp[4];
#pragma unroll
    for (int jt = 0; jt < 4; ++jt) {
      acc_s[jt] = (f32x4_t){0.f, 0.f, 0.f, 0.f};
      acc_dp[jt] = (f32x4_t){0.f, 0.f, 0.f, 0.f};
    }
#pragma unroll
    for (int ks = 0; ks < 2; ++ks)
#pragma unroll
      for (int jt = 0; jt < 4; ++jt) {
        acc_s[jt] = mfma32(kf[jt][ks], qu[ks], acc_s[jt]);
        acc_dp[jt] = mfma32(vf[jt][ks], dO[ks], acc_dp[jt]);
      }
    PROF_MARK(2)
    add_band(acc_s, qv, lds + PP_OFF + slot_lo * IMG, lds + PP_OFF + slot_hi * IMG, bd, L);
    PROF_MARK(3)
    bf16x4_t dsb[4], pdb[4];
    softmax_bwd_tile<DROP, true>(acc_s, acc_dp, dsb, pdb, lse2, Di, a.inv_keep, piece, ksh, kl - j0, g4);
    PROF_MARK(4)
    wave_lds_sync();
#pragma unroll
    for (int jt = 0; jt < 4; ++jt) {
      *reinterpret_cast<bf16x4_t*>(exw + (exo ^ (jt << 5))) = dsb[jt];
      *reinterpret_cast<bf16x4_t*>(exw + 2048 + (exo ^ (jt << 5))) = pdb[jt];
    }
    PROF_MARK(5)
    asm volatile("s_waitcnt lgkmcnt(0)" ::: "memory");
    __builtin_amdgcn_s_barrier();
    PROF_MARK(6)
    {
      const uint32_t eb = lds_addr(exbase);
      const uint32_t ead[2] = {eb + exr[0], eb + exr[1]};
      uint2 bx[8];
      trr8<0, 2048, 2 * BNC, 2 * BNC + 2048>(ead, bx);
      const uint32_t qb = lds_addr(sQ);
#pragma unroll
      for (int half = 0; half < 2; ++half) {
        const int d0 = half * 2;
        const uint32_t aad[4] = {qb + (trk[0] ^ (uint32_t)(d0 << 5)), qb + (trk[1] ^ (uint32_t)(d0 << 5)),
                                 qb + (trk[0] ^ (uint32_t)((d0 + 1) << 5)), qb + (trk[1] ^ (uint32_t)((d0 + 1) << 5))};
        uint2 ax[16];
        trr16<0, 4096, IMG, IMG + 4096>(aad, ax);
#pragma unroll
        for (int dd = 0; dd < 2; ++dd)
#pragma unroll
          for (int ks2 = 0; ks2 < 2; ++ks2) {
            const bf16x8_t aq = cat2(ax[(dd * 2 + 0) * 4 + ks2], ax[(dd * 2 + 1) * 4 + ks2]);
            const bf16x8_t ag = cat2(ax[(dd * 2 + 0) * 4 + 2 + ks2], ax[(dd * 2 + 1) * 4 + 2 + ks2]);
            acc_dk[d0 + dd] = mfma32(aq, cat2(bx[0 * 4 + 2 * ks2], bx[1 * 4 + 2 * ks2]), acc_dk[d0 + dd]);
            acc_dv[d0 + dd] = mfma32(ag, cat2(bx[0 * 4 + 2 * ks2 + 1], bx[1 * 4 + 2 * ks2 + 1]), acc_dv[d0 + dd]);
          }
      }
    }
    slot_lo = slot_nx;
    PROF_MARK(7)
  }
  const int j = j0 + 16 * w + li;
  if (j < T) {
    bf16_t* ok = a.dk + ((long)b * T + j) * a.lddkv + h * DH;
    bf16_t* ov = a.dv + ((long)b * T + j) * a.lddkv + h * DH;
#pragma unroll
    for (int dt = 0; dt < 4; ++dt) {
      uint2 pk;
      pk.x = pack_bf2(acc_dk[dt][0], acc_dk[dt][1]);
      pk.y = pack_bf2(acc_dk[dt][2], acc_dk[dt][3]);
      *reinterpret_cast<uint2*>(ok + dt * 16 + g4 * 4) = pk;
      pk.x = pack_bf2(acc_dv[dt][0], acc_dv[dt][1]);
      pk.y = pack_bf2(acc_dv[dt][2], acc_dv[dt][3]);
      *reinterpret_cast<uint2*>(ov + dt * 16 + g4 * 4) = pk;
    }
  }
  PROF_MARK(8)
  PROF_DUMP(1)
}

}

static int g_rp_on = [] { const char* e = getenv("EA_FLASH_V1"); return e && e[0] == '1' ? 0 : 1; }();
extern "C" int ea_set_flash_relpos(int on) {
  const int prev = g_rp_on;
  g_rp_on = on ? 1 : 0;
  return prev;
}
bool ea_rp_eligible(bool relpos, int T, int S, int causal, uint32_t thr, const void* bits) {
  return g_rp_on && relpos && T == S && !(causal & 1) && (thr == 0 || bits != nullptr);
}

int ea_rp_keep_bits(uint16_t* bits, int H, int B, int T, uint64_t seed, uint32_t thr, hipStream_t stream) {
  const int nkt = (T + TK - 1) / TK;
  const long n = (long)H * B * nkt * (nkt * 64) * 4;
  static const long cap = [] { const char* e = getenv("EA_KEEP_BITS_WGS"); return e ? atol(e) : 256L; }();
  long blocks = (n + 255) / 256;
  if (cap > 0 && blocks > cap) blocks = cap;
  hipLaunchKernelGGL(keep_bits_kernel, dim3((unsigned)blocks), dim3(256), 0, stream, bits, seed, thr, H * B, T, nkt);
  return EA_CHECK_LAUNCH();
}

int ea_rp_fwd(const FlashFwdArgs& a, hipStream_t stream) {
  const dim3 grid((unsigned)(a.nq * a.H * a.B));
  if (a.thr) hipLaunchKernelGGL(rp_fwd_kernel<true>, grid, dim3(256), 0, stream, a);
  else hipLaunchKernelGGL(rp_fwd_kernel<false>, grid, dim3(256), 0, stream, a);
  return EA_CHECK_LAUNCH();
}

int ea_rp_bwd(const FlashBwdArgs& a_in, hipStream_t stream) {
  static const int dbg = [] { const char* e = getenv("EA_RP_DBG"); return e ? atoi(e) : 0; }();
  FlashBwdArgs a = a_in;
  a.dbg = dbg;
  a.prof = nullptr;
#ifdef RP_PROF
  static unsigned long long* prof_buf = nullptr;
  static const int prof_on = [] { const char* e = getenv("EA_RP_PROF"); return e && e[0] == '1' ? 1 : 0; }();
  if (prof_on) {
    if (!prof_buf) hipMalloc(&prof_buf, 2 * 8192 * 10 * sizeof(unsigned long long));
    hipMemsetAsync(prof_buf, 0, 2 * 8192 * 10 * sizeof(unsigned long long), stream);
    a.prof = prof_buf;
  }
#endif
  const dim3 gq((unsigned)(a.nq * a.H * a.B)), gk((unsigned)(a.nk * a.H * a.B));
  if (a.thr) {
    hipLaunchKernelGGL(rp_bwd_q_kernel<true>, gq, dim3(256), 0, stream, a);
    hipLaunchKernelGGL(rp_bwd_kv_kernel<true>, gk, dim3(256), 0, stream, a);
  } else {
    hipLaunchKernelGGL(rp_bwd_q_kernel<false>, gq, dim3(256), 0, stream, a);
    hipLaunchKernelGGL(rp_bwd_kv_kernel<false>, gk, dim3(256), 0, stream, a);
  }
#ifdef RP_PROF
  if (a.prof) {
    static int calls = 0;
    if (++calls == 20) {
      hipStreamSynchronize(stream);
      static unsigned long long h[2 * 8192 * 10];
      hipMemcpy(h, a.prof, sizeof(h), hipMemcpyDeviceToHost);
      const char* names[2] = {"Q ", "KV"};
      const int nw[2] = {(int)gq.x * 4, (int)gk.x * 4};
      for (int k = 0; k < 2; ++k) {
        double sum[10] = {0};
        int cnt = 0;
        for (int wv = 0; wv < nw[k] && wv < 8192; ++wv) {
          const unsigned long long* o = h + ((long)k * 8192 + wv) * 10;
          unsigned long long tot = 0;
          for (int p = 0; p < 10; ++p) tot += o[p];
          if (!tot) continue;
          ++cnt;
          for (int p = 0; p < 10; ++p) sum[p] += (double)o[p];
        }
        fprintf(stderr, "[rp prof] %s waves %d, mean s_memtime ticks per wave by phase:", names[k], cnt);
        for (int p = 0; p < 10; ++p) fprintf(stderr, " p%d=%.0f", p, cnt ? sum[p] / cnt : 0.0);
        fprintf(stderr, "\n");
      }
    }
  }
#endif
  return EA_CHECK_LAUNCH();
}
```

### espresso_amd/kernels.py

```python
import ctypes
from typing import Optional

import torch

from . import _lib
from ._lib import EaGemmParams, check

ACT_NONE, ACT_RELU, ACT_SILU = 0, 1, 2
_ACT = {None: 0, "none": 0, "relu": 1, "silu": 2, "swish": 2}


def _stream():
    return ctypes.c_void_p(torch._C._cuda_getCurrentRawStream(torch._C._cuda_getDevice()))


def _p(t: Optional[torch.Tensor]):
    if t is None:
        return None
    if not t.is_cuda:
        raise RuntimeError("espresso_amd kernels need device tensors (no CPU path)")
    return ctypes.c_void_p(t.data_ptr())


def drop_params(p: float):
# ... 80 lines not shown
        ws = torch.empty(p.splitk * batch * M * N, dtype=torch.float32, device=C.device)
        p.workspace = ws.data_ptr()
    if qsplit is not None:
        q_u, q_v, pos_u, pos_v, qn, ld_q, qscale = qsplit
        assert q_u.dtype == torch.bfloat16 and (q_v is None or q_v.dtype == torch.bfloat16)
        assert (pos_u is None or pos_u.dtype == torch.float32) and (pos_v is None or pos_v.dtype == torch.float32)
        p.q_u, p.q_v, p.pos_u, p.pos_v = _p(q_u), _p(q_v), _p(pos_u), _p(pos_v)
        p.qsplit_n, p.ld_q, p.qscale = int(qn), int(ld_q), float(qscale)
    check(_lib.lib().ea_gemm_bf16(ctypes.byref(p), _stream()), "ea_gemm_bf16")
    return C


def layernorm_fwd(x, gamma, beta, eps=1e-5, row_zero=None, drop_p=0.0, drop_seed=0, save_stats=True, out_f32=False):
    M, C = x.shape
    assert x.dtype == torch.bfloat16 and x.is_contiguous()
    y = torch.empty(M, C, dtype=torch.float32, device=x.device) if out_f32 else torch.empty_like(x)
    mean = torch.empty(M, dtype=torch.float32, device=x.device) if save_stats else None
    rstd = torch.empty(M, dtype=torch.float32, device=x.device) if save_stats else None
    thr, scale = drop_params(drop_p)
    fn = _lib.lib().ea_layernorm_fwd_f32out if out_f32 else _lib.lib().ea_layernorm_fwd
    check(fn(_p(x), _p(gamma), _p(beta), _p(y), _p(mean), _p(rstd), M, C, eps, _p(row_zero), drop_seed, thr, scale, _stream()),
          "ea_layernorm_fwd")
    return y, mean, rstd


def layernorm_bwd(x, dy, gamma, mean, rstd, dgamma, dbeta, row_zero=None, drop_p=0.0, drop_seed=0, dx_add=None):
    M, C = x.shape
    assert dy.is_contiguous() and dy.dtype in (torch.bfloat16, torch.float32)
    dx = torch.empty_like(x)
    thr, scale = drop_params(drop_p)
    ws = torch.empty(_lib.lib().ea_layernorm_bwd_workspace_bytes(M, C) // 4, dtype=torch.float32, device=x.device)
    fn = _lib.lib().ea_layernorm_bwd_f32dy if dy.dtype == torch.float32 else _lib.lib().ea_layernorm_bwd
    check(fn(_p(x), _p(dy), _p(gamma), _p(mean), _p(rstd), _p(dx), _p(dgamma), _p(dbeta), M, C, _p(row_zero), drop_seed, thr, scale,
             _p(dx_add), _p(ws), _stream()), "ea_layernorm_bwd")
    return dx


def cast_f32_to_bf16(src, dst=None):
    if dst is None:
        dst = torch.empty(src.shape, dtype=torch.bfloat16, device=src.device)
    check(_lib.lib().ea_cast_f32_to_bf16(_p(src), _p(dst), src.numel(), _stream()), "ea_cast_f32_to_bf16")
    return dst


def cast_f32_to_bf16_rows(src, ld_dst):
    M, N = src.shape
    assert src.dtype == torch.float32 and src.stride(1) == 1 and ld_dst >= N
    dst = torch.empty(M, ld_dst, dtype=torch.bfloat16, device=src.device)
    check(_lib.lib().ea_cast_f32_to_bf16_rows(_p(src), src.stride(0), _p(dst), ld_dst, M, N, _stream()), "ea_cast_f32_to_bf16_rows")
    return dst if ld_dst == N else dst[:, :N]


def cast_bf16_to_f32(src, dst=None):
    if dst is None:
        dst = torch.empty(src.shape, dtype=torch.float32, device=src.device)
    check(_lib.lib().ea_cast_bf16_to_f32(_p(src), _p(dst), src.numel(), _stream()), "ea_cast_bf16_to_f32")
    return dst


def scale_dropout(x, a=1.0, y=None, b=0.0, drop_p=0.0, drop_seed=0, out=None):
    assert x.dtype == torch.bfloat16 and x.is_contiguous()
    if out is None:
        out = torch.empty_like(x)
    thr, scale = drop_params(drop_p)
    check(_lib.lib().ea_scale_dropout_bf16(_p(x), _p(y), _p(out), x.numel(), a, b, drop_seed, thr, scale, _stream()),
          "ea_scale_dropout_bf16")
    return out


def colsum(X, out, M, N, ld):
    assert X.dtype == torch.bfloat16 and out.dtype == torch.float32
    check(_lib.lib().ea_colsum_bf16(_p(X), _p(out), M, N, ld, _stream()), "ea_colsum_bf16")
    return out


def colsum_ptr(X_ptr: int, out, M, N, ld):
    check(_lib.lib().ea_colsum_bf16(ctypes.c_void_p(X_ptr), _p(out), M, N, ld, _stream()), "ea_colsum_bf16")
    return out


def zero_rows(x, row_zero):
    M, C = x.shape
    check(_lib.lib().ea_zero_rows_bf16(_p(x), _p(row_zero), M, C, _stream()), "ea_zero_rows_bf16")
    return x


def relpos_q_prep(qkv, ldq, u, v, M, C, scaling, want_qv=True):
    qu = torch.empty(M, C, dtype=torch.bfloat16, device=qkv.device)
    qv = torch.empty(M, C, dtype=torch.bfloat16, device=qkv.device) if want_qv else None
    check(_lib.lib().ea_relpos_q_prep(_p(qkv), ldq, _p(u), _p(v), _p(qu), _p(qv), M, C, scaling, _stream()),
          "ea_relpos_q_prep")
    return qu, qv


def relpos_softmax_fwd(ac, bd, key_len, attn_mask, H, B, T, S, ld_ac, ld_bd, ld_p, causal=False, drop_p=0.0,
                       drop_seed=0):
    P = torch.empty(H * B * T, ld_p, dtype=torch.bfloat16, device=ac.device)
    Pd = torch.empty_like(P) if drop_p > 0 else None
    thr, scale = drop_params(drop_p)
    check(
        _lib.lib().ea_relpos_softmax_fwd(_p(ac), _p(bd), _p(key_len), _p(attn_mask), _p(P), _p(Pd), H, B, T, S, ld_ac,
                                         ld_bd, ld_p, int(causal), drop_seed, thr, scale, _stream()),
        "ea_relpos_softmax_fwd",
    )
    return P, (Pd if Pd is not None else P)


def flash_attention_supported(dh, T, S, relpos):
    return bool(_lib.lib().ea_flash_attention_supported(dh, T, S, int(relpos)))


def flash_keep_bits_buffer(H, B, T, device):
    return torch.empty(int(_lib.lib().ea_flash_keep_bits_bytes(H, B, T)) // 2, dtype=torch.int16, device=device)


def flash_attention_fwd(qu, qv, k, v, pp, key_len, H, B, T, S, ldq, ldkv, ldpp=0, causal=False, drop_p=0.0, drop_seed=0,
                        want_lse=True, want_bits=False):
    dh = 64
    out = torch.empty(B * T, H * dh, dtype=torch.bfloat16, device=qu.device)
    lse = torch.empty(H * B, T, dtype=torch.float32, device=qu.device) if want_lse else None
    thr, scale = drop_params(drop_p)
    bits = None
    if want_bits and thr and qv is not None and T == S and not causal:
        bits = flash_keep_bits_buffer(H, B, T, qu.device)
    check(
        _lib.lib().ea_flash_attention_fwd(_p(qu), _p(qv), ldq, _p(k), _p(v), ldkv, _p(pp), ldpp, _p(key_len), _p(out),
                                          H * dh, _p(lse), H, B, T, S, dh, int(causal), drop_seed, thr, scale, _p(bits), _stream()),
        "ea_flash_attention_fwd",
    )
    return (out, lse, bits) if want_bits else (out, lse)


def flash_attention_bwd(qu, qv, k, v, pp, key_len, out, dout, lse, dk, dv, H, B, T, S, ldq, ldkv, lddkv, ldpp=0, causal=False,
                        scaling=1.0, drop_p=0.0, drop_seed=0, keep_bits=None, dq=None, lddq=0):
    dh = 64
    C = H * dh
    relpos = qv is not None
    t1 = torch.empty(B * T, C, dtype=torch.bfloat16, device=qu.device)
    t2 = torch.empty_like(t1) if relpos else None
    Rp = (2 * T - 1 + 7) // 8 * 8
    dBD = torch.empty(H * B * T, Rp, dtype=torch.bfloat16, device=qu.device) if relpos else None
    D = torch.empty(H * B, T, dtype=torch.float32, device=qu.device)
    thr, scale = drop_params(drop_p)
    check(
        _lib.lib().ea_flash_attention_bwd(_p(qu), _p(qv), ldq, _p(k), _p(v), ldkv, _p(pp), ldpp, _p(key_len), _p(out), _p(dout),
                                          C, _p(lse), _p(D), _p(t1), _p(t2), C, _p(dBD), Rp, _p(dk), _p(dv), lddkv, H, B, T, S,
                                          dh, int(causal), scaling, drop_seed, thr, scale, _p(keep_bits), _p(dq), lddq,
                                          _stream()),
        "ea_flash_attention_bwd",
    )
    return t1, t2, dBD


def relpos_softmax_bwd(P, dPd, H, B, T, S, ld_p, ld_dp, ld_bd, want_bd=True, drop_p=0.0, drop_seed=0):
    dAC = torch.empty(H * B * T, ld_p, dtype=torch.bfloat16, device=P.device)
    dBD = torch.empty(H * B * T, ld_bd, dtype=torch.bfloat16, device=P.device) if want_bd else None
    thr, scale = drop_params(drop_p)
    check(
        _lib.lib().ea_relpos_softmax_bwd(_p(P), _p(dPd), _p(dAC), _p(dBD), H, B, T, S, ld_p, ld_dp, ld_bd, drop_seed,
                                         thr, scale, _stream()),
        "ea_relpos_softmax_bwd",
    )
    return dAC, dBD


def add2_strided(a, lda, b, ldb, out, ldo, M, C, out_off=0):
    check(
        _lib.lib().ea_add2_strided_bf16(_p(a), lda, _p(b), ldb, ctypes.c_void_p(out.data_ptr() + 2 * out_off), ldo, M,
                                        C, _stream()),
        "ea_add2_strided_bf16",
    )
    return out


def glu_dwconv_fwd(Y, w, B, T, C, KW, stats):
    U = torch.empty(B * T, C, dtype=torch.bfloat16, device=Y.device)
    Z = torch.empty(B * T, C, dtype=torch.bfloat16, device=Y.device)
    check(_lib.lib().ea_glu_dwconv_fwd(_p(Y), _p(w), _p(U), _p(Z), _p(stats), B, T, C, KW, _stream()),
          "ea_glu_dwconv_fwd")
    return U, Z


def bn_finalize(stats, C, n, eps, momentum, running_mean=None, running_var=None):
    mean_rstd = torch.empty(2, C, dtype=torch.float32, device=stats.device)
    check(_lib.lib().ea_bn_finalize(_p(stats), _p(mean_rstd), _p(running_mean), _p(running_var), C, float(n), eps,
                                    momentum, _stream()), "ea_bn_finalize")
    return mean_rstd


def bn_from_running(running_mean, running_var, eps):
    C = running_mean.numel()
    mean_rstd = torch.empty(2, C, dtype=torch.float32, device=running_mean.device)
    check(_lib.lib().ea_bn_from_running(_p(running_mean), _p(running_var), _p(mean_rstd), C, eps, _stream()),
          "ea_bn_from_running")
    return mean_rstd


def bn_act_fwd(Z, mean_rstd, gamma, beta, act):
    M, C = Z.shape
    H = torch.empty_like(Z)
    check(_lib.lib().ea_bn_act_fwd(_p(Z), _p(mean_rstd), _p(gamma), _p(beta), _p(H), M, C, _ACT[act], _stream()),
          "ea_bn_act_fwd")
    return H


def conv1_bn_bwd(X, Z, dH, mean_rstd, gamma, beta, dgamma, dbeta, dW, dbias, B, T, F, CO, sy, sx, act, training=True):
    from . import functional as _F

    red = _F._pool_zeros((2, CO), torch.float32, Z.device)
    check(_lib.lib().ea_conv1_bn_bwd(_p(X), _p(Z), _p(dH), _p(mean_rstd), _p(gamma), _p(beta), _p(red), _p(dgamma), _p(dbeta), _p(dW),
                                     _p(dbias), B, T, F, CO, sy, sx, _ACT[act], int(training), _stream()), "ea_conv1_bn_bwd")


def bn_act_bwd(Z, dH, mean_rstd, gamma, beta, dgamma, dbeta, act, training=True):
    M, C = Z.shape
    from . import functional as _F

    red = _F._pool_zeros((2, C), torch.float32, Z.device)
    dZ = torch.empty_like(Z)
    check(
        _lib.lib().ea_bn_act_bwd(_p(Z), _p(dH), _p(mean_rstd), _p(gamma), _p(beta), _p(red), _p(dZ), _p(dgamma),
                                 _p(dbeta), M, C, _ACT[act], int(training), _stream()),
        "ea_bn_act_bwd",
    )
    return dZ


def glu_dwconv_bwd(dZ, Y, U, w, dw, B, T, C, KW):
    dY = torch.empty(B * T, 2 * C, dtype=torch.bfloat16, device=Y.device)
    ws = torch.empty(int(_lib.lib().ea_dwconv_wgrad_workspace_bytes(B, T, C, KW)), dtype=torch.uint8, device=Y.device)
    check(_lib.lib().ea_glu_dwconv_bwd(_p(dZ), _p(Y), _p(U), _p(w), _p(dY), _p(dw), _p(ws), B, T, C, KW, _stream()),
          "ea_glu_dwconv_bwd")
    return dY


def conv1_fwd(X, W, bias, B, T, F, CO, sy, sx, stats):
    To, Fo = (T - 1) // sy + 1, (F - 1) // sx + 1
    Z = torch.empty(B * To * Fo, CO, dtype=torch.bfloat16, device=X.device)
    check(_lib.lib().ea_conv1_fwd(_p(X), _p(W), _p(bias), _p(Z), _p(stats), B, T, F, CO, sy, sx, _stream()),
          "ea_conv1_fwd")
    return Z


def conv1_wgrad(X, dZ, dW, dbias, B, T, F, CO, sy, sx):
    check(_lib.lib().ea_conv1_wgrad(_p(X), _p(dZ), _p(dW), _p(dbias), B, T, F, CO, sy, sx, _stream()), "ea_conv1_wgrad")


def conv3x3_fwd(X, W16, bias, B, T, F, Cin, Cout, sy, sx, stats=None):
    To, Fo = (T - 1) // sy + 1, (F - 1) // sx + 1
    Z = torch.empty((B * To * Fo, Cout), dtype=torch.bfloat16, device=X.device)
    check(_lib.lib().ea_conv3x3_fwd(_p(X), _p(W16), _p(bias), _p(Z), _p(stats), B, T, F, Cin, Cout, sy, sx, _stream()), "ea_conv3x3_fwd")
    return Z


def conv3x3_dgrad(dZ, Wd16, B, T, F, Cin, Cout, sy, sx):
    dX = torch.empty((B * T * F, Cin), dtype=torch.bfloat16, device=dZ.device)
    check(_lib.lib().ea_conv3x3_dgrad(_p(dZ), _p(Wd16), _p(dX), B, T, F, Cin, Cout, sy, sx, _stream()), "ea_conv3x3_dgrad")
    return dX


def conv3x3_wgrad(X, dZ, dW, B, T, F, Cin, Cout, sy, sx, param_layout=False):
    lib = _lib.lib()
    nb = lib.ea_conv3x3_wgrad_workspace_bytes(B, T, F, Cin, Cout, sy, sx)
    ws = torch.empty(nb, dtype=torch.uint8, device=X.device)
    fn = lib.ea_conv3x3_wgrad_param_layout if param_layout else lib.ea_conv3x3_wgrad
    check(fn(_p(X), _p(dZ), _p(dW), _p(ws), B, T, F, Cin, Cout, sy, sx, _stream()), "ea_conv3x3_wgrad")
    return dW


def im2col3x3(A, B, T, F, C, sy, sx):
    To, Fo = (T - 1) // sy + 1, (F - 1) // sx + 1
    col = torch.empty(B * To * Fo, 9 * C, dtype=torch.bfloat16, device=A.device)
    check(_lib.lib().ea_im2col3x3(_p(A), _p(col), B, T, F, C, sy, sx, _stream()), "ea_im2col3x3")
    return col


def col2im3x3(dcol, B, T, F, C, sy, sx):
    dA = torch.empty(B * T * F, C, dtype=torch.bfloat16, device=dcol.device)
    check(_lib.lib().ea_col2im3x3(_p(dcol), _p(dA), B, T, F, C, sy, sx, _stream()), "ea_col2im3x3")
    return dA


def colstats(X, stats):
    M, C = X.shape
    check(_lib.lib().ea_colstats_bf16(_p(X), _p(stats), M, C, _stream()), "ea_colstats_bf16")
    return stats


def log_softmax(x, M, V, ld):
    out = torch.empty(M, V, dtype=torch.float32, device=x.device)
    if x.dtype == torch.float32:
        check(_lib.lib().ea_log_softmax_f32(_p(x), ld, _p(out), M, V, _stream()), "ea_log_softmax_f32")
    else:
        assert x.dtype == torch.bfloat16
        check(_lib.lib().ea_log_softmax_bf16(_p(x), ld, _p(out), M, V, _stream()), "ea_log_softmax_bf16")
    return out


def ctc_loss_fwd(lprobs, targets, in_len, tgt_len, B, T, V, Lmax, blank):
    assert lprobs.dtype == torch.float32 and lprobs.is_contiguous()
    assert targets.dtype == torch.int32 and in_len.dtype == torch.int32 and tgt_len.dtype == torch.int32
    dev = lprobs.device
    nll = torch.empty(B, dtype=torch.float32, device=dev)
    ws = torch.empty(int(_lib.lib().ea_ctc_workspace_bytes(B, T, Lmax)), dtype=torch.uint8, device=dev)
    check(
        _lib.lib().ea_ctc_loss(_p(lprobs), _p(targets), _p(in_len), _p(tgt_len), _p(nll), _p(ws), B, T, V, Lmax, blank,
# ... 303 lines not shown
```

### include/espresso_amd.h

```cpp
#ifndef ESPRESSO_AMD_H
#define ESPRESSO_AMD_H

#include <stdint.h>

#ifdef __cplusplus
extern "C" {
#endif

typedef struct ihipStream_t* ea_stream_t;

int ea_version(void);

enum { EA_ACT_NONE = 0, EA_ACT_RELU = 1, EA_ACT_SILU = 2 };

typedef struct EaGemmParams {
  const void* A;
  const void* B;
  void* C;
  void* C2;
  const float* bias;
  const void* resid;
  const void* aux;
  int M, N, K, batch, zdiv;
  int a_kstrided, b_kstrided, c_f32, accumulate, resid_f32, act;
  long lda, ldb, ldc, ldc2, ldr, ldaux;
  long sA_hi, sA_lo, sB_hi, sB_lo, sC_hi, sC_lo, sR_hi, sR_lo, sX_hi, sX_lo;
  float alpha, out_scale;
  uint64_t drop_seed;
  uint32_t drop_thr;
  float drop_scale;
  int splitk, kchunk;
  void* workspace;
  void* q_u;
  void* q_v;
  const float* pos_u;
  const float* pos_v;
  long ld_q;
  int qsplit_n;
  float qscale;
} EaGemmParams;

int ea_gemm_bf16(const EaGemmParams* p, ea_stream_t stream);
long ea_gemm_splitk_workspace_bytes(int M, int N, int batch, int splitk);
int ea_set_gemm_variant(int v);
int ea_set_gemm_xcd_swizzle(int mask);
int ea_set_gemm_glds(int stages);
long ea_set_gemm_nt_store_min_bytes(long bytes);
int ea_set_gemm_w8(int mode);
int ea_gemm_profile_enable(int on);
long ea_gemm_profile_read(double* total_ms, double* total_flops);
int ea_gemm_profile_bytes(double* total_bytes);
long ea_gemm_profile_dump(const char* path);

#define EA_WGRAD_MAX 16
typedef struct EaWgradProblem {
  const void* dy;
  const void* x;
  float* dW;
  float* dbias;
  int M, N, K;
  long ld_dy, ld_x, ldw;
} EaWgradProblem;
typedef struct EaWgradGroup {
  int count;
  EaWgradProblem p[EA_WGRAD_MAX];
} EaWgradGroup;
int ea_wgrad_group(const EaWgradGroup* group, ea_stream_t stream);
int ea_set_wgrad_transposing_reads(int on);
int ea_set_wgrad_w8(int mode);

int ea_layernorm_fwd(const void* x, const float* gamma, const float* beta, void* y, float* mean, float* rstd,
                     int M, int C, float eps, const uint8_t* row_zero, uint64_t drop_seed, uint32_t drop_thr,
                     float drop_scale, ea_stream_t stream);
int ea_layernorm_fwd_f32out(const void* x, const float* gamma, const float* beta, float* y, float* mean, float* rstd,
                            int M, int C, float eps, const uint8_t* row_zero, uint64_t drop_seed, uint32_t drop_thr,
                            float drop_scale, ea_stream_t stream);
int ea_layernorm_bwd_f32dy(const void* x, const float* dy, const float* gamma, const float* mean, const float* rstd,
                           void* dx, float* dgamma, float* dbeta, int M, int C, const uint8_t* row_zero,
                           uint64_t drop_seed, uint32_t drop_thr, float drop_scale, const void* dx_add,
                           void* workspace, ea_stream_t stream);
long ea_layernorm_bwd_workspace_bytes(int M, int C);
int ea_layernorm_bwd(const void* x, const void* dy, const float* gamma, const float* mean, const float* rstd,
                     void* dx, float* dgamma, float* dbeta, int M, int C, const uint8_t* row_zero,
                     uint64_t drop_seed, uint32_t drop_thr, float drop_scale, const void* dx_add,
                     void* workspace, ea_stream_t stream);
int ea_layernorm_bwd_dx(const void* x, const void* dy, const float* gamma, const float* mean, const float* rstd, void* dx,
                        float* dgamma, float* dbeta, int M, int C, const uint8_t* row_zero, uint64_t drop_seed,
                        uint32_t drop_thr, float drop_scale, const void* dx_add, void* workspace, ea_stream_t stream);
int ea_layernorm_param_reduce(const void* workspace, float* dgamma, float* dbeta, int M, int C, ea_stream_t stream);
#define EA_LNRED_MAX 8
typedef struct EaLnReduceItem { const void* workspace; float* dgamma; float* dbeta; int M, C; } EaLnReduceItem;
typedef struct EaLnReduceGroup { int count; EaLnReduceItem item[EA_LNRED_MAX]; } EaLnReduceGroup;
int ea_layernorm_param_reduce_group(const EaLnReduceGroup* group, ea_stream_t stream);
int ea_layernorm_bwd_dx2(const void* x, const void* dy, const float* gamma, const float* mean, const float* rstd, void* dx,
                         float* dgamma, float* dbeta, int M, int C, const void* dx_add, void* workspace, void* out2, float a2,
                         uint64_t seed2, uint32_t thr2, float scale2, ea_stream_t stream);
int ea_layernorm_fwd2(const void* x, const float* g1, const float* b1, void* y1, float* mean1, float* rstd1, const float* g2,
                      const float* b2, void* y2, float* mean2, float* rstd2, int M, int C, float eps, ea_stream_t stream);
int ea_layernorm_bwd2_dx(const void* x1, const void* dy1, const float* gamma1, const float* mean1, const float* rstd1,
                         const void* dx_add, void* ws1, const void* x2, const float* gamma2, const float* mean2, const float* rstd2,
                         void* ws2, void* dx, int M, int C, void* out2, float a2, uint64_t seed2, uint32_t thr2, float scale2,
                         ea_stream_t stream);

int ea_cast_f32_to_bf16(const float* src, void* dst, long n, ea_stream_t stream);
int ea_transpose_bf16_batch(const void* const* src, void* const* dst, const int* rows, const int* cols, int n, ea_stream_t stream);
int ea_audio_probe(const char* path, long* num_samples, int* sample_rate, int* channels, int* bits);
long ea_audio_read_i16(const char* path, int16_t* dst, long capacity, int* sample_rate);
int ea_audio_verify(const char* path);
int ea_audio_read_batch_i16(const char* const* paths, int n, int16_t* dst, const long* offsets, int num_threads, long* lengths,
                            int* sample_rates);

int ea_cast_f32_to_bf16_rows(const float* src, long ld_src, void* dst, long ld_dst, long M, int N, ea_stream_t stream);
int ea_cast_bf16_to_f32(const void* src, float* dst, long n, ea_stream_t stream);
int ea_scale_dropout_bf16(const void* x, const void* y, void* out, long n, float a, float b, uint64_t seed,
                          uint32_t thr, float inv_keep, ea_stream_t stream);
int ea_colsum_bf16(const void* X, float* out, int M, int N, long ld, ea_stream_t stream);
int ea_embedding_fwd(const int* tokens, const int* positions, const float* W, const float* pos_table, void* out, int M,
                     int C, float scale, ea_stream_t stream);
int ea_embedding_bwd(const int* tokens, const void* dy, float* dW, int M, int C, float scale, int pad_idx,
                     ea_stream_t stream);
int ea_zero_rows_bf16(void* x, const uint8_t* row_zero, int M, int C, ea_stream_t stream);

int ea_flash_attention_supported(int dh, int T, int S, int relpos);
int ea_flash_attention_fwd(const void* qu, const void* qv, long ldq, const void* k, const void* v, long ldkv,
                           const void* pp, long ldpp, const int* key_len, void* out, long ldo, float* lse, int H, int B,
                           int T, int S, int dh, int causal, uint64_t drop_seed, uint32_t drop_thr, float drop_scale,
                           void* keep_bits, ea_stream_t stream);
long ea_flash_keep_bits_bytes(int H, int B, int T);
int ea_set_flash_relpos(int on);
int ea_flash_keep_bits(void* keep_bits, int H, int B, int T, uint64_t drop_seed, uint32_t drop_thr, ea_stream_t stream);
int ea_flash_attention_bwd(const void* qu, const void* qv, long ldq, const void* k, const void* v, long ldkv,
                           const void* pp, long ldpp, const int* key_len, const void* out, const void* dout, long ldo,
                           const float* lse, float* D, void* t1, void* t2, long ldt, void* dBD, int ld_bd, void* dk,
                           void* dv, long lddkv, int H, int B, int T, int S, int dh, int causal, float scaling,
                           uint64_t drop_seed, uint32_t drop_thr, float drop_scale, const void* keep_bits,
                           void* dq, long lddq, ea_stream_t stream);

int ea_relpos_q_prep(const void* qkv, long ldq, const float* u, const float* v, void* qu, void* qv, int M,
                     int C, float scaling, ea_stream_t stream);
int ea_relpos_softmax_fwd(const float* ac, const float* bd, const int* key_len, const float* attn_mask, void* P,
                          void* Pd, int H, int B, int T, int S, int ld_ac, int ld_bd, int ld_p, int causal,
                          uint64_t drop_seed, uint32_t drop_thr, float drop_scale, ea_stream_t stream);
int ea_relpos_softmax_bwd(const void* P, const float* dPd, void* dAC, void* dBD, int H, int B, int T, int S,
                          int ld_p, int ld_dp, int ld_bd, uint64_t drop_seed, uint32_t drop_thr,
                          float drop_scale, ea_stream_t stream);
int ea_add2_strided_bf16(const void* a, long lda, const void* b, long ldb, void* out, long ldo, int M, int C,
                         ea_stream_t stream);

int ea_glu_dwconv_fwd(const void* Y, const float* w, void* U, void* Z, double* stats, int B, int T, int C, int KW,
                      ea_stream_t stream);
int ea_bn_finalize(const double* stats, float* mean_rstd, float* running_mean, float* running_var, int C, float n,
                   float eps, float momentum, ea_stream_t stream);
int ea_bn_from_running(const float* running_mean, const float* running_var, float* mean_rstd, int C, float eps,
                       ea_stream_t stream);
int ea_bn_act_fwd(const void* Z, const float* mean_rstd, const float* gamma, const float* beta, void* H, long M,
                  int C, int act, ea_stream_t stream);
int ea_bn_act_bwd(const void* Z, const void* dH, const float* mean_rstd, const float* gamma, const float* beta,
                  float* red, void* dZ, float* dgamma, float* dbeta, long M, int C, int act, int training,
                  ea_stream_t stream);
long ea_dwconv_wgrad_workspace_bytes(int B, int T, int C, int KW);
int ea_glu_dwconv_bwd(const void* dZ, const void* Y, const void* U, const float* w, void* dY, float* dw,
                      void* wgrad_ws, int B, int T, int C, int KW, ea_stream_t stream);
int ea_dwconv_bwd_weight(const void* dZ, const void* U, float* dw, void* wgrad_ws, int B, int T, int C, int KW, ea_stream_t stream);
int ea_bn_act_fwd_train(const void* Z, const double* stats, float* mean_rstd, float* running_mean, float* running_var,
                        const float* gamma, const float* beta, void* H, long M, int C, int act, float n, float eps,
                        float momentum, double* zero_next, int zero_n, ea_stream_t stream);
int ea_bn_act_bwd_fused(const void* Z, const void* dH, const float* mean_rstd, const float* gamma, const float* beta,
                        float* red, void* dZ, float* dgamma, float* dbeta, long M, int C, int act, int training,
                        float* zero_next, int zero_n, ea_stream_t stream);
int ea_bn_glu_dwconv_bwd_fused(const void* Z, const void* dH, const float* mean_rstd, const float* gamma, const float* beta, float* red,
                               void* dZ, float* dgamma, float* dbeta, int act, int training, float* zero_next, int zero_n,
                               const void* Y, const float* w, void* dY, int B, int T, int C, int KW, ea_stream_t stream);
int ea_bn_param_grad(const float* red, float* dgamma, float* dbeta, int C, ea_stream_t stream);
int ea_conv1_bn_bwd(const float* X, const void* Z, const void* dH, const float* mean_rstd, const float* gamma, const float* beta,
                    float* red, float* dgamma, float* dbeta, float* dW, float* dbias, int B, int T, int F, int CO, int sy, int sx,
                    int act, int training, ea_stream_t stream);

int ea_conv1_fwd(const float* X, const float* W, const float* bias, void* Z, double* stats, int B, int T, int F,
                 int CO, int sy, int sx, ea_stream_t stream);
int ea_conv1_wgrad(const float* X, const void* dZ, float* dW, float* dbias, int B, int T, int F, int CO, int sy,
                   int sx, ea_stream_t stream);
int ea_conv3x3_fwd(const void* X, const void* W, const float* bias, void* Z, double* stats, int B, int T, int F, int Cin,
                   int Cout, int sy, int sx, ea_stream_t stream);
int ea_conv3x3_dgrad(const void* dZ, const void* Wd, void* dX, int B, int T, int F, int Cin, int Cout, int sy, int sx,
                     ea_stream_t stream);
long ea_conv3x3_wgrad_workspace_bytes(int B, int T, int F, int Cin, int Cout, int sy, int sx);
int ea_conv3x3_wgrad(const void* X, const void* dZ, float* dW, void* workspace, int B, int T, int F, int Cin, int Cout, int sy,
                     int sx, ea_stream_t stream);
int ea_conv3x3_wgrad_param_layout(const void* X, const void* dZ, float* dW, void* workspace, int B, int T, int F, int Cin, int Cout,
                                  int sy, int sx, ea_stream_t stream);
int ea_im2col3x3(const void* A, void* col, int B, int T, int F, int C, int sy, int sx, ea_stream_t stream);
int ea_col2im3x3(const void* dcol, void* dA, int B, int T, int F, int C, int sy, int sx, ea_stream_t stream);
int ea_colstats_bf16(const void* X, double* stats, long M, int C, ea_stream_t stream);

int ea_log_softmax_f32(const float* in, long ld_in, float* out, long M, int V, ea_stream_t stream);
int ea_log_softmax_bf16(const void* in, long ld_in, float* out, long M, int V, ea_stream_t stream);
long ea_ctc_workspace_bytes(int B, int T, int Lmax);
int ea_ctc_loss(const float* lprobs, const int* targets, const int* in_len, const int* tgt_len, float* nll,
                void* workspace, int B, int T, int V, int Lmax, int blank, ea_stream_t stream);
int ea_ctc_grad(const float* lprobs, const void* workspace, const float* nll, const int* targets,
                const int* in_len, const int* tgt_len, void* dlogits, long ld_out, int dlogits_bf16, int B, int T,
                int V, int Lmax, int blank, float grad_scale, const float* grad_scale_dev, int zero_infinity,
                ea_stream_t stream);
int ea_ctc_greedy_decode(const void* x, long ld, int x_bf16, const int* in_len, int* best, float* bestv, int* tokens,
                         int* align, int* out_len, float* score, int B, int T, int V, int blank, int pad,
                         ea_stream_t stream);
int ea_label_smoothed_ce(const void* logits, long ld, int logits_bf16, const int* target, float* out_loss,
                         void* dlogits, long ld_out, int dlogits_bf16, long M, int V, int pad_idx, float eps,
                         float grad_scale, int smoothing, const float* prior, int tgt_len, ea_stream_t stream);

int ea_fbank_batch(const float* wav, const long* offsets, int B, const float* window, const float* twiddle,
                   const int* mel_start, const int* mel_len, const int* mel_woff, const float* mel_w,
                   const float* cmvn_mean, const float* cmvn_std, float* feat, float* utt_sum, int* out_len,
                   int Tmax, int nmel, int frame_len, int frame_shift, float preemph, float log_floor,
                   ea_stream_t stream);
int ea_fbank_batch_i16(const int16_t* wav, const long* offsets, int B, const float* window, const float* twiddle,
                   const int* mel_start, const int* mel_len, const int* mel_woff, const float* mel_w,
                   const float* cmvn_mean, const float* cmvn_std, float* feat, float* utt_sum, int* out_len,
                   int Tmax, int nmel, int frame_len, int frame_shift, float preemph, float log_floor,
                   ea_stream_t stream);
int ea_specaugment(float* feat, const int* lengths, const float* utt_sum, const int* fmask, const int* tmask,
                   int nf, int nt, int B, int Tmax, int nmel, int use_mean, float mask_value, ea_stream_t stream);

int ea_feature_stats(const float* feat, const int* lengths, double* acc, int B, int Tmax, int nmel, ea_stream_t stream);

int ea_grad_sumsq(const float* g, long n, float* out, ea_stream_t stream);
int ea_clip_coef(const float* sumsq, float pre_scale, const float* denom_dev, float max_norm, float* coef,
                 ea_stream_t stream);
int ea_adam_step(float* p, float* g, float* m, float* v, void* p_bf16, long n, const float* coef, float lr,
                 float beta1, float beta2, float eps, float weight_decay, int step, int zero_grad,
                 ea_stream_t stream);

typedef struct EaFfnParams { const float *ln_g, *ln_b; const void* w1; const float* b1; const void* w2; const float* b2; } EaFfnParams;
typedef struct EaFfnGrads { float *ln_g, *ln_b, *w1, *b1, *w2, *b2; } EaFfnGrads;
typedef struct EaAttnParams {
  const float *ln_g, *ln_b; const void* wqkv; const float* bqkv; const void* wo; const float* bo;
  const float *pos_u, *pos_v; const void* wpos;
} EaAttnParams;
typedef struct EaAttnGrads { float *ln_g, *ln_b, *wqkv, *bqkv, *wo, *bo, *pos_u, *pos_v, *wpos; } EaAttnGrads;
typedef struct EaConvParams {
  const float *ln_g, *ln_b; const void* pw1; const float* dw; const float *bn_g, *bn_b; float *bn_rm, *bn_rv; const void* pw2;
} EaConvParams;
typedef struct EaConvGrads { float *ln_g, *ln_b, *pw1, *dw, *bn_g, *bn_b, *pw2; } EaConvGrads;
typedef struct EaLayerGrads { EaFfnGrads ffn1; EaAttnGrads attn; EaConvGrads conv; EaFfnGrads ffn2; float *final_ln_g, *final_ln_b; } EaLayerGrads;
typedef struct EaConformerLayer {
  EaFfnParams ffn1; EaAttnParams attn; EaConvParams conv; EaFfnParams ffn2; const float *final_ln_g, *final_ln_b;
  EaLayerGrads grads;
  void* wt;
} EaConformerLayer;
typedef struct EaLayerShape {
  int B, T, C, H, F, KW, training; float p_drop, p_act, p_attn; uint64_t seed; int has_attn_mask;
  int scratch_clean;
  int pos_mode, act;
  int S;
  int defer;
  int wt_fresh;
} EaLayerShape;

enum {
  EA_SITE_FFN1_ACT = 0, EA_SITE_FFN1_OUT = 1, EA_SITE_ATTN_PROBS = 2, EA_SITE_ATTN_OUT = 3, EA_SITE_CONV_OUT = 4,
  EA_SITE_FFN2_ACT = 5, EA_SITE_FFN2_OUT = 6, EA_SITE_CROSS_PROBS = 7, EA_SITE_CROSS_OUT = 8
};
uint64_t ea_layer_dropout_seed(uint64_t layer_seed, int site);
int ea_dropout_hash_host(uint64_t seed, uint64_t idx0, long n, uint32_t* out);

int ea_set_backward_overlap(int on);
int ea_set_backward_deferred(int on);
int ea_set_backward_deferred_inline(int on);
int ea_backward_flush(ea_stream_t stream);
int ea_streams_share_queue(ea_stream_t a, ea_stream_t b);
int ea_side_stream_report(int* rejected, int* unprobed);
int ea_conformer_layer_workspace(const EaLayerShape* shape, long* saved_bytes, long* scratch_bytes);
int ea_conformer_layer_refresh_wt(const EaConformerLayer* layer, const EaLayerShape* shape, ea_stream_t stream);
int ea_conformer_layer_fwd(const EaConformerLayer* layer, const EaLayerShape* shape, const void* x_in, void* x_out,
                           const int* key_len, const float* attn_mask, const void* pe, void* saved, long saved_bytes,
                           void* scratch, long scratch_bytes, ea_stream_t stream);
int ea_conformer_layer_bwd(const EaConformerLayer* layer, const EaLayerShape* shape, const void* x_in, const void* dy,
                           void* dx, const int* key_len, const void* pe, void* saved, long saved_bytes, void* scratch,
                           long scratch_bytes, ea_stream_t stream);
typedef struct EaLayerChain {
  const EaConformerLayer* next; void* next_saved; long next_saved_bytes; int ln1_done;
  const EaConformerLayer* prev; void* prev_saved; long prev_saved_bytes; uint64_t prev_seed; void* prev_pre;
  int final_ln_done; const void* pre_in;
} EaLayerChain;
int ea_conformer_layer_fwd_chained(const EaConformerLayer* layer, const EaLayerShape* shape, const EaLayerChain* chain, const void* x_in,
                                   void* x_out, const int* key_len, const float* attn_mask, const void* pe, void* saved,
                                   long saved_bytes, void* scratch, long scratch_bytes, ea_stream_t stream);
int ea_conformer_layer_bwd_chained(const EaConformerLayer* layer, const EaLayerShape* shape, const EaLayerChain* chain, const void* x_in,
                                   const void* dy, void* dx, const int* key_len, const void* pe, void* saved, long saved_bytes,
// ... 93 lines not shown
```

Baseline: 5.361.

## Fuse relpos flash-attention backward into single KV-tiled kernel with in-kernel bias grads

Replaces the separate Q-side and KV-side relative-position flash backward kernels with a delta kernel, one KV-tiled backward kernel and a finish kernel. The main kernel writes per-key-tile dQ partials to an fp32 slab, and the finish kernel reduces them straight into the fused dqkv buffer. The pos_u/pos_v bias gradients are column-summed in-kernel instead of materialising the t1/t2 tensors and launching separate bias_grad passes. This removes the recomputation done in the separate Q kernel and the t1/t2 traffic, at the cost of a large fp32 workspace, extra reduction traffic and an additional launch.

Result: slower. 5.267 (median of 6 runs) (-1.7%).

```diff
diff --git a/espresso_amd/csrc/engine.hip b/espresso_amd/csrc/engine.hip
--- a/espresso_amd/csrc/engine.hip
+++ b/espresso_amd/csrc/engine.hip
@@ -611,8 +611,10 @@
       RUN(ea_cast_f32_to_bf16(dppT32, dppT, (long)C * Rp, wstream(c)));
       gemm_on(c, gw2, wstream(c));
     }
-    bias_grad(c, t1, gw.pos_u, M, C, C);
-    bias_grad(c, t2, gw.pos_v, M, C, C);
+    if (t1) {
+      bias_grad(c, t1, gw.pos_u, M, C, C);
+      bias_grad(c, t2, gw.pos_v, M, C, C);
+    }
   }
   if (!have_dq) RUN(ea_add2_strided_bf16(t1, C, t2, C, dqkv, 3 * C, M, C, c.s));
   fork(c);
@@ -643,17 +645,14 @@
   dgrad(c, g, w.wo, wot, dO, M, C, C);
   if (attn_fused(sh)) {
     uint16_t* dqkv = sc.get<uint16_t>((size_t)M * 3 * C);
-    uint16_t* t1 = sc.get<uint16_t>((size_t)M * C);
-    uint16_t* t2 = sc.get<uint16_t>((size_t)M * C);
     uint16_t* dBD = sc.get<uint16_t>((size_t)Z * T * Rp);
     float* Dd = sc.get<float>((size_t)Z * T);
-    static const bool fused_dq = getenv("EA_NO_FUSED_DQ") == nullptr;
-    RUN(ea_flash_attention_bwd(a.qu, sh.pos_mode == 1 ? a.qu : a.qv, C, a.qkv + C, a.qkv + 2 * C, 3 * C,
-                               sh.pos_mode == 1 ? (const uint16_t*)pe : a.pp, C, key_len, a.o, dO, C, a.lse, Dd, t1, t2, C, dBD,
-                               Rp, dqkv + C, dqkv + 2 * C, 3 * C, H, B, T, T, dh, (sh.scratch_clean && c.overlap) ? 2 : 0, scaling, seed + kProbs,
-                               drop_thr(sh.p_attn),
-                               drop_scale(sh.p_attn), a.bits, fused_dq ? dqkv : nullptr, 3 * C, c.s));
-    attn_bwd_tail(c, a, sh, w, gw, x, dy, dx, pe, dqkv, t1, t2, dBD, wqkvt, next, dpe, fused_dq);
+    float* ws = sc.get<float>((size_t)(ea_flash_relpos_bwd_workspace_bytes(H, B, T) + 3) / 4);
+    RUN(ea_flash_relpos_bwd(a.qu, sh.pos_mode == 1 ? a.qu : a.qv, C, a.qkv + C, a.qkv + 2 * C, 3 * C,
+                            sh.pos_mode == 1 ? (const uint16_t*)pe : a.pp, C, key_len, a.o, dO, C, a.lse, Dd, dBD, Rp, dqkv, 3 * C,
+                            dqkv + C, dqkv + 2 * C, 3 * C, gw.pos_u, gw.pos_v, H, B, T, (sh.scratch_clean && c.overlap) ? 2 : 0, scaling,
+                            seed + kProbs, drop_thr(sh.p_attn), drop_scale(sh.p_attn), a.bits, ws, c.s));
+    attn_bwd_tail(c, a, sh, w, gw, x, dy, dx, pe, dqkv, nullptr, nullptr, dBD, wqkvt, next, dpe, true);
     release(c, mark);
     return;
   }
diff --git a/espresso_amd/csrc/flash_attention.hip b/espresso_amd/csrc/flash_attention.hip
--- a/espresso_amd/csrc/flash_attention.hip
+++ b/espresso_amd/csrc/flash_attention.hip
@@ -1,6 +1,9 @@
 #include "common.h"
 #include "espresso_amd.h"
 #include "flash_internal.h"
+
+#include <map>
+#include <mutex>
 
 namespace {
 
@@ -671,21 +674,19 @@
   return EA_CHECK_LAUNCH();
 }
 
-extern "C" int ea_flash_attention_bwd(const void* qu, const void* qv, long ldq, const void* k, const void* v, long ldkv,
-                                      const void* pp, long ldpp, const int* key_len, const void* out, const void* dout, long ldo,
-                                      const float* lse, float* D, void* t1, void* t2, long ldt, void* dBD, int ld_bd, void* dk,
-                                      void* dv, long lddkv, int H, int B, int T, int S, int dh, int causal, float scaling,
-                                      uint64_t drop_seed, uint32_t drop_thr, float drop_scale, const void* keep_bits,
-                                      void* dq, long lddq, hipStream_t stream) {
-  if (H <= 0 || B <= 0 || T <= 0) return 0;
+static int bwd_args(FlashBwdArgs& a, const void* qu, const void* qv, long ldq, const void* k, const void* v, long ldkv, const void* pp,
+                    long ldpp, const int* key_len, const void* out, const void* dout, long ldo, const float* lse, float* D, void* t1,
+                    void* t2, long ldt, void* dBD, int ld_bd, void* dk, void* dv, long lddkv, int H, int B, int T, int S, int dh,
+                    int causal, float scaling, uint64_t drop_seed, uint32_t drop_thr, float drop_scale, const void* keep_bits,
+                    void* dq, long lddq) {
   const bool relpos = qv != nullptr;
   if (!ea_flash_attention_supported(dh, T, S, relpos)) return -2;
-  if (relpos && (!pp || !t2 || !dBD || ld_bd < 2 * T - 1 || ld_bd % 8 || ((uintptr_t)dBD & 15))) return -2;
+  if (relpos && (!pp || !dBD || ld_bd < 2 * T - 1 || ld_bd % 8 || ((uintptr_t)dBD & 15))) return -2;
   if ((ldq | ldkv | ldo | ldt | lddkv) % 8 || (relpos && ldpp % 8)) return -2;
   if (((uintptr_t)qu | (uintptr_t)qv | (uintptr_t)k | (uintptr_t)v | (uintptr_t)pp | (uintptr_t)out | (uintptr_t)dout) & 15) return -2;
   if (((uintptr_t)t1 | (uintptr_t)t2 | (uintptr_t)dk | (uintptr_t)dv | (uintptr_t)dq) & 7) return -2;
   if (dq && (!relpos || lddq % 4)) return -2;
-  FlashBwdArgs a;
+  a = FlashBwdArgs{};
   a.qu = (const bf16_t*)qu; a.qv = (const bf16_t*)qv; a.ldq = ldq;
   a.k = (const bf16_t*)k; a.v = (const bf16_t*)v; a.ldkv = ldkv;
   a.pp = (const bf16_t*)pp; a.ldpp = ldpp;
@@ -701,9 +702,12 @@
   a.scaling = scaling;
   a.seed = drop_seed; a.thr = drop_thr; a.inv_keep = drop_scale;
   a.bits = (const uint16_t*)keep_bits;
-  if (ea_rp_eligible(relpos, T, S, causal, drop_thr, keep_bits)) return ea_rp_bwd(a, stream);
-  const dim3 gq((unsigned)(a.nq * H * B)), gk((unsigned)(a.nk * H * B));
-  if (relpos) {
+  return 0;
+}
+
+static int general_bwd(const FlashBwdArgs& a, hipStream_t stream) {
+  const dim3 gq((unsigned)(a.nq * a.H * a.B)), gk((unsigned)(a.nk * a.H * a.B));
+  if (a.qv) {
     hipLaunchKernelGGL(flash_bwd_q_kernel<true>, gq, dim3(256), 0, stream, a);
     hipLaunchKernelGGL(flash_bwd_kv_kernel<true>, gk, dim3(256), 0, stream, a);
   } else {
@@ -712,3 +716,77 @@
   }
   return EA_CHECK_LAUNCH();
 }
+
+static float* rp_internal_workspace(long bytes) {
+  static std::mutex mu;
+  static std::map<int, std::pair<void*, long>> bufs;
+  int dev = 0;
+  if (hipGetDevice(&dev) != hipSuccess) return nullptr;
+  std::lock_guard<std::mutex> lk(mu);
+  std::pair<void*, long>& e = bufs[dev];
+  if (e.second < bytes) {
+    if (e.first) (void)hipFree(e.first);
+    e = {nullptr, 0};
+    if (hipMalloc(&e.first, (size_t)bytes) != hipSuccess) return nullptr;
+    e.second = bytes;
+  }
+  return (float*)e.first;
+}
+
+extern "C" int ea_flash_attention_bwd(const void* qu, const void* qv, long ldq, const void* k, const void* v, long ldkv,
+                                      const void* pp, long ldpp, const int* key_len, const void* out, const void* dout, long ldo,
+                                      const float* lse, float* D, void* t1, void* t2, long ldt, void* dBD, int ld_bd, void* dk,
+                                      void* dv, long lddkv, int H, int B, int T, int S, int dh, int causal, float scaling,
+                                      uint64_t drop_seed, uint32_t drop_thr, float drop_scale, const void* keep_bits,
+                                      void* dq, long lddq, hipStream_t stream) {
+  if (H <= 0 || B <= 0 || T <= 0) return 0;
+  const bool relpos = qv != nullptr;
+  if (relpos && !t2) return -2;
+  FlashBwdArgs a;
+  int rc = bwd_args(a, qu, qv, ldq, k, v, ldkv, pp, ldpp, key_len, out, dout, ldo, lse, D, t1, t2, ldt, dBD, ld_bd, dk, dv, lddkv, H, B, T,
+                    S, dh, causal, scaling, drop_seed, drop_thr, drop_scale, keep_bits, dq, lddq);
+  if (rc) return rc;
+  if (ea_rp_eligible(relpos, T, S, causal, drop_thr, keep_bits)) {
+    if (!t1) return -2;
+    a.slab = rp_internal_workspace(ea_rp_bwd_workspace_bytes(H, B, T, true));
+    if (!a.slab) return -3;
+    return ea_rp_bwd(a, stream);
+  }
+  return general_bwd(a, stream);
+}
+
+extern "C" long ea_flash_relpos_bwd_workspace_bytes(int H, int B, int T) {
+  if (H <= 0 || B <= 0 || T <= 0) return 0;
+  const long m = (long)B * T * H * DH * 2 * (long)sizeof(bf16_t) + 256;
+  const long r = ea_rp_bwd_workspace_bytes(H, B, T, false);
+  return r > m ? r : m;
+}
+
+extern "C" int ea_flash_relpos_bwd(const void* qu, const void* qv, long ldq, const void* k, const void* v, long ldkv, const void* pp,
+                                   long ldpp, const int* key_len, const void* out, const void* dout, long ldo, const float* lse, float* D,
+                                   void* dBD, int ld_bd, void* dq, long lddq, void* dk, void* dv, long lddkv, float* dpos_u,
+                                   float* dpos_v, int H, int B, int T, int flags, float scaling, uint64_t drop_seed, uint32_t drop_thr,
+                                   float drop_scale, const void* keep_bits, void* workspace, hipStream_t stream) {
+  if (H <= 0 || B <= 0 || T <= 0) return 0;
+  if (!qv || !dq || !dpos_u != !dpos_v || !workspace || ((uintptr_t)workspace & 255) || (flags & 1)) return -2;
+  FlashBwdArgs a;
+  int rc = bwd_args(a, qu, qv, ldq, k, v, ldkv, pp, ldpp, key_len, out, dout, ldo, lse, D, nullptr, nullptr, 0, dBD, ld_bd, dk, dv,
+                    lddkv, H, B, T, T, DH, flags & 2, scaling, drop_seed, drop_thr, drop_scale, keep_bits, dq, lddq);
+  if (rc) return rc;
+  if (ea_rp_eligible(true, T, T, 0, drop_thr, keep_bits)) {
+    a.slab = (float*)workspace;
+    const long slab = ea_rp_bwd_workspace_bytes(H, B, T, false) - (long)H * B * a.nk * 128 * (long)sizeof(float);
+    a.bsum = dpos_u ? (float*)((char*)workspace + slab) : nullptr;
+    a.dpos_u = dpos_u;
+    a.dpos_v = dpos_v;
+    return ea_rp_bwd(a, stream);
+  }
+  const long n = (long)B * T * H * DH;
+  a.t1 = (bf16_t*)workspace;
+  a.t2 = a.t1 + n;
+  a.ldt = (long)H * DH;
+  rc = general_bwd(a, stream);
+  if (rc == 0 && dpos_u) rc = ea_colsum_bf16(a.t1, dpos_u, B * T, H * DH, a.ldt, stream);
+  if (rc == 0 && dpos_v) rc = ea_colsum_bf16(a.t2, dpos_v, B * T, H * DH, a.ldt, stream);
+  return rc;
+}
diff --git a/espresso_amd/csrc/flash_internal.h b/espresso_amd/csrc/flash_internal.h
--- a/espresso_amd/csrc/flash_internal.h
+++ b/espresso_amd/csrc/flash_internal.h
@@ -29,11 +29,12 @@
   float scaling;
   uint64_t seed; uint32_t thr; float inv_keep;
   const uint16_t* bits;
-  unsigned long long* prof;
-  int dbg;
+  float* slab; float* bsum;
+  float* dpos_u; float* dpos_v;
 };
 
 bool ea_rp_eligible(bool relpos, int T, int S, int causal, uint32_t thr, const void* bits);
 int ea_rp_keep_bits(uint16_t* bits, int H, int B, int T, uint64_t seed, uint32_t thr, hipStream_t stream);
 int ea_rp_fwd(const FlashFwdArgs& a, hipStream_t stream);
+long ea_rp_bwd_workspace_bytes(int H, int B, int T, bool t12);
 int ea_rp_bwd(const FlashBwdArgs& a, hipStream_t stream);
diff --git a/espresso_amd/csrc/flash_relpos.hip b/espresso_amd/csrc/flash_relpos.hip
--- a/espresso_amd/csrc/flash_relpos.hip
+++ b/espresso_amd/csrc/flash_relpos.hip
@@ -84,6 +84,15 @@
         "v"(ad[19])
       : "memory");
 }
+__device__ __forceinline__ void trr8n(const uint32_t (&ad)[8], uint2 (&o)[8]) {
+  asm volatile(
+      "ds_read_b64_tr_b16 %0, %8\n\tds_read_b64_tr_b16 %1, %9\n\tds_read_b64_tr_b16 %2, %10\n\tds_read_b64_tr_b16 %3, %11\n\t"
+      "ds_read_b64_tr_b16 %4, %12\n\tds_read_b64_tr_b16 %5, %13\n\tds_read_b64_tr_b16 %6, %14\n\tds_read_b64_tr_b16 %7, %15\n\t"
+      "s_waitcnt lgkmcnt(0)"
+      : "=&v"(o[0]), "=&v"(o[1]), "=&v"(o[2]), "=&v"(o[3]), "=&v"(o[4]), "=&v"(o[5]), "=&v"(o[6]), "=&v"(o[7])
+      : "v"(ad[0]), "v"(ad[1]), "v"(ad[2]), "v"(ad[3]), "v"(ad[4]), "v"(ad[5]), "v"(ad[6]), "v"(ad[7])
+      : "memory");
+}
 __device__ __forceinline__ uint2 lds_u2(const char* p) {
   const float* f = reinterpret_cast<const float*>(p);
   return make_uint2(__float_as_uint(f[0]), __float_as_uint(f[1]));
@@ -109,16 +118,27 @@
   __builtin_amdgcn_fence(__ATOMIC_ACQUIRE, "wavefront");
 }
 __device__ __forceinline__ float fexp2(float x) { return __builtin_amdgcn_exp2f(x); }
-
-#ifdef RP_PROF
-#define PROF_DECL unsigned long long prof_t = __builtin_amdgcn_s_memtime(); unsigned prof_acc[10] = {0, 0, 0, 0, 0, 0, 0, 0, 0, 0};
-#define PROF_MARK(k) { const unsigned long long n_ = __builtin_amdgcn_s_memtime(); prof_acc[k] += (unsigned)(n_ - prof_t); prof_t = n_; }
-#define PROF_DUMP(kern) if (a.prof && (threadIdx.x & 63) == 0) { unsigned long long* o_ = a.prof + ((long)(kern) * 8192 + (long)blockIdx.x * 4 + (threadIdx.x >> 6)) * 10; for (int k_ = 0; k_ < 10; ++k_) o_[k_] = prof_acc[k_]; }
-#else
-#define PROF_DECL
-#define PROF_MARK(k)
-#define PROF_DUMP(kern)
-#endif
+__device__ __forceinline__ float colsum16(const f32x4_t (&c)[4], int li) {
+  float v8[8], v4[4], v2[2];
+#pragma unroll
+  for (int k = 0; k < 8; ++k) {
+    const bool up = li & 8;
+    const float lo = c[k >> 2][k & 3], hi = c[(k + 8) >> 2][(k + 8) & 3];
+    v8[k] = (up ? hi : lo) + __shfl_xor(up ? lo : hi, 8, 64);
+  }
+#pragma unroll
+  for (int k = 0; k < 4; ++k) {
+    const bool up = li & 4;
+    v4[k] = (up ? v8[k + 4] : v8[k]) + __shfl_xor(up ? v8[k] : v8[k + 4], 4, 64);
+  }
+#pragma unroll
+  for (int k = 0; k < 2; ++k) {
+    const bool up = li & 2;
+    v2[k] = (up ? v4[k + 2] : v4[k]) + __shfl_xor(up ? v4[k] : v4[k + 2], 2, 64);
+  }
+  const bool up = li & 1;
+  return (up ? v2[1] : v2[0]) + __shfl_xor(up ? v2[0] : v2[1], 1, 64);
+}
 
 struct LaneK {
   int lane, w, li, g4;
@@ -408,278 +428,10 @@
   }
 }
 
+constexpr int K_OFF = 6 * IMG;
+
 template <bool DROP>
-__global__ __launch_bounds__(256, 2) void rp_bwd_q_kernel(const FlashBwdArgs a) {
-  __shared__ __attribute__((aligned(16))) char lds[LDS_BYTES];
-  const LaneK L = lane_consts();
-  const int lane = L.lane, w = L.w, li = L.li, g4 = L.g4;
-  const int vid = xcd_remap(blockIdx.x, gridDim.x);
-  const int z = vid / a.nq, qt = vid % a.nq;
-  const int h = z / a.B, b = z % a.B;
-  const int T = a.T;
-  const int i0 = qt * TQ;
-  const int i = i0 + 16 * w + li;
-  const int kl = a.klen ? min(a.klen[b], T) : T;
-  const int nt = (kl + TK - 1) / TK;
-  const int nkt = (T + TK - 1) / TK;
-
-  bf16x8_t qu[2], qv[2], dO[2];
-  float Di = 0.f;
-  {
-    const int ic = min(i, T - 1);
-    const long oq = ((long)b * T + ic) * a.ldq + h * DH + g4 * 8;
-    const long oo = ((long)b * T + ic) * a.ldo + h * DH + g4 * 8;
-#pragma unroll
-    for (int ks = 0; ks < 2; ++ks) {
-      qu[ks] = __builtin_bit_cast(bf16x8_t, *reinterpret_cast<const uint4*>(a.qu + oq + ks * 32));
-      qv[ks] = __builtin_bit_cast(bf16x8_t, *reinterpret_cast<const uint4*>(a.qv + oq + ks * 32));
-      const uint4 g = *reinterpret_cast<const uint4*>(a.dout + oo + ks * 32);
-      const uint4 o = *reinterpret_cast<const uint4*>(a.out + oo + ks * 32);
-      dO[ks] = __builtin_bit_cast(bf16x8_t, g);
-      const uint32_t wg[4] = {g.x, g.y, g.z, g.w}, wo[4] = {o.x, o.y, o.z, o.w};
-#pragma unroll
-      for (int e = 0; e < 4; ++e)
-        Di += __uint_as_float(wg[e] << 16) * __uint_as_float(wo[e] << 16) +
-              __uint_as_float(wg[e] & 0xffff0000u) * __uint_as_float(wo[e] & 0xffff0000u);
-    }
-  }
-  Di += __shfl_xor(Di, 16, 64);
-  Di += __shfl_xor(Di, 32, 64);
-  const float lse2 = (i < T) ? a.lse[(long)z * T + i] * LOG2E : INFINITY;
-  if (i < T && g4 == 0 && a.D) a.D[(long)z * T + i] = Di;
-
-  f32x4_t acc_t1[4], acc_t2[4];
-#pragma unroll
-  for (int dt = 0; dt < 4; ++dt) {
-    acc_t1[dt] = (f32x4_t){0.f, 0.f, 0.f, 0.f};
-    acc_t2[dt] = (f32x4_t){0.f, 0.f, 0.f, 0.f};
-  }
-  const bf16_t* Kb = a.k + (long)b * T * a.ldkv + h * DH;
-  const bf16_t* Vb = a.v + (long)b * T * a.ldkv + h * DH;
-  const bf16_t* PPb = a.pp + h * DH;
-  const int R = 2 * T - 1;
-  const ImgSrc srcK = img_src(Kb, a.ldkv, T - 1, w, lane), srcV = img_src(Vb, a.ldkv, T - 1, w, lane);
-  const ImgSrc srcP = img_src(PPb, a.ldpp, R - 1, w, lane);
-  const int pbase = (T - 1) - (i0 + TQ - 1);
-  float* bd = reinterpret_cast<float*>(lds + BNC_OFF + w * BNC);
-  bf16_t* ob = reinterpret_cast<bf16_t*>(bd);
-  const uint32_t* bitp = DROP ? reinterpret_cast<const uint32_t*>(a.bits) + (((long)z * nkt) * (nkt * 64) + i) * 2 + (g4 >> 1) : nullptr;
-  const long bit_step = (long)nkt * 64 * 2;
-  const int ksh = (g4 & 1) * 16;
-  uint2 mlo, mhi;
-  {
-    uint32_t m[4], n[4];
-#pragma unroll
-    for (int e = 0; e < 4; ++e) {
-      m[e] = (4 * g4 + e >= 15 - li) ? 0xffffu : 0u;
-      n[e] = (64 + 4 * g4 + e <= 78 - li) ? 0xffffu : 0u;
-    }
-    mlo = make_uint2(m[0] | (m[1] << 16), m[2] | (m[3] << 16));
-    mhi = make_uint2(n[0] | (n[1] << 16), n[2] | (n[3] << 16));
-  }
-  const int ob_w = li * (OBP - 1) + 15 + g4 * 4;
-  const char* ob_rd = reinterpret_cast<const char*>(ob) + li * (OBP * 2) + g4 * 8;
-
-  uint32_t piece = 0, piece_next = 0;
-  int jcov = 0;
-  uint32_t dbd_pk[8];
-  int dbd_j0 = -1;
-  auto store_dbd = [&]() {
-    const int j = dbd_j0 + lane;
-    if (dbd_j0 >= 0 && j < T) {
-      const int row_w = i0 + 16 * w, nrow = T - row_w;
-      bf16_t* dp = a.dBD + ((long)z * T + row_w) * a.ld_bd + (T - 1 - row_w) + j;
-      if (nrow >= 16) {
-#pragma unroll
-        for (int iw = 0; iw < 16; ++iw) dp[(long)iw * (a.ld_bd - 1)] = (bf16_t)(dbd_pk[iw >> 1] >> (16 * (iw & 1)));
-      } else {
-#pragma unroll
-        for (int iw = 0; iw < 16; ++iw)
-          if (iw < nrow) dp[(long)iw * (a.ld_bd - 1)] = (bf16_t)(dbd_pk[iw >> 1] >> (16 * (iw & 1)));
-      }
-    }
-  };
-  if (nt > 0) {
-    issue_img(lds, srcK, 0, w, lane);
-    issue_img(lds + IMG, srcV, 0, w, lane);
-    issue_img(lds + PP_OFF, srcP, pbase, w, lane);
-    issue_img(lds + PP_OFF + IMG, srcP, pbase + 64, w, lane);
-    if (DROP) piece_next = bitp[0];
-  }
-  int slot_lo = 0;
-  PROF_DECL
-  for (int t = 0; t < nt; ++t) {
-    const int j0 = t * TK;
-    jcov = min(T, j0 + TK);
-    PROF_MARK(9)
-    asm volatile("s_waitcnt vmcnt(0)" ::: "memory");
-    __builtin_amdgcn_s_barrier();
-    PROF_MARK(0)
-    store_dbd();
-    const int slot_hi = slot_lo == 2 ? 0 : slot_lo + 1;
-    const int slot_nx = slot_hi == 2 ? 0 : slot_hi + 1;
-    if (DROP) {
-      piece = piece_next;
-      asm volatile("" : "+v"(piece));
-    }
-    if (t + 1 < nt) {
-      if (DROP) piece_next = bitp[(long)(t + 1) * bit_step];
-      char* st = lds + ((t + 1) & 1) * 2 * IMG;
-      issue_img(st, srcK, j0 + TK, w, lane);
-      issue_img(st + IMG, srcV, j0 + TK, w, lane);
-      issue_img(lds + PP_OFF + slot_nx * IMG, srcP, pbase + 64 * (t + 2), w, lane);
-    }
-    PROF_MARK(1)
-    const char* sK = lds + (t & 1) * 2 * IMG;
-    const char* sV = sK + IMG;
-    const char* blk_lo = lds + PP_OFF + slot_lo * IMG;
-    const char* blk_hi = lds + PP_OFF + slot_hi * IMG;
-
-    f32x4_t acc_s[4], acc_dp[4];
-#pragma unroll
-    for (int jt = 0; jt < 4; ++jt) {
-      acc_s[jt] = (f32x4_t){0.f, 0.f, 0.f, 0.f};
-      acc_dp[jt] = (f32x4_t){0.f, 0.f, 0.f, 0.f};
-    }
-    {
-      bf16x8_t fr[2][4];
-      auto frag = [&](int jt, bf16x8_t (&f)[4]) {
-        f[0] = ldf(sK + jt * 2048 + L.offk[0]);
-        f[1] = ldf(sK + jt * 2048 + L.offk[1]);
-        f[2] = ldf(sV + jt * 2048 + L.offk[0]);
-        f[3] = ldf(sV + jt * 2048 + L.offk[1]);
-      };
-      frag(0, fr[0]);
-#pragma unroll
-      for (int jt = 0; jt < 4; ++jt) {
-        if (jt + 1 < 4) frag(jt + 1, fr[(jt + 1) & 1]);
-        acc_s[jt] = mfma32(fr[jt & 1][0], qu[0], acc_s[jt]);
-        acc_dp[jt] = mfma32(fr[jt & 1][2], dO[0], acc_dp[jt]);
-        acc_s[jt] = mfma32(fr[jt & 1][1], qu[1], acc_s[jt]);
-        acc_dp[jt] = mfma32(fr[jt & 1][3], dO[1], acc_dp[jt]);
-      }
-    }
-    PROF_MARK(2)
-    add_band(acc_s, qv, blk_lo, blk_hi, bd, L);
-    PROF_MARK(3)
-    bf16x4_t dsb[4], pdb[4];
-    softmax_bwd_tile<DROP, false>(acc_s, acc_dp, dsb, pdb, lse2, Di, a.inv_keep, piece, ksh, kl - j0, g4);
-    PROF_MARK(4)
-
-    if (!(a.dbg & 4)) {
-      bf16x8_t kf[8];
-      tr_image(sK, L.tro, kf);
-#pragma unroll
-      for (int kb = 0; kb < 2; ++kb) {
-        const bf16x8_t db = cat(dsb[2 * kb], dsb[2 * kb + 1]);
-#pragma unroll
-        for (int dt = 0; dt < 4; ++dt) acc_t1[dt] = mfma32(kf[dt * 2 + kb], db, acc_t1[dt]);
-      }
-    }
-    PROF_MARK(5)
-    wave_lds_sync();
-#pragma unroll
-    for (int jt = 0; jt < 4; ++jt) {
-      const uint2 pk = __builtin_bit_cast(uint2, dsb[jt]);
-      ob[ob_w + jt * 16 + 0] = (bf16_t)(pk.x & 0xffffu);
-      ob[ob_w + jt * 16 + 1] = (bf16_t)(pk.x >> 16);
-      ob[ob_w + jt * 16 + 2] = (bf16_t)(pk.y & 0xffffu);
-      ob[ob_w + jt * 16 + 3] = (bf16_t)(pk.y >> 16);
-    }
-    wave_lds_sync();
-    if (!(a.dbg & 2)) {
-      uint32_t ad[20];
-      uint2 pf[20];
-#pragma unroll
-      for (int q16 = 0; q16 < 5; ++q16) {
-        const int qq = q16 - w + 3;
-        const uint32_t pbk = lds_addr(((qq >> 2) ? blk_hi : blk_lo) + (qq & 3) * 2048);
-#pragma unroll
-        for (int dt = 0; dt < 4; ++dt) ad[q16 * 4 + dt] = pbk + L.tro[dt];
-      }
-      trr20(ad, pf);
-#pragma unroll
-      for (int cb = 0; cb < 2; ++cb) {
-        uint2 blo = lds_u2(ob_rd + cb * 64);
-        const uint2 bhi = lds_u2(ob_rd + cb * 64 + 32);
-        if (cb == 0) {
-          blo.x &= mlo.x;
-          blo.y &= mlo.y;
-        }
-        const bf16x8_t db = cat2(blo, bhi);
-#pragma unroll
-        for (int dt = 0; dt < 4; ++dt) acc_t2[dt] = mfma32(cat2(pf[(2 * cb) * 4 + dt], pf[(2 * cb + 1) * 4 + dt]), db, acc_t2[dt]);
-      }
-      uint2 bl = lds_u2(ob_rd + 128);
-      bl.x &= mhi.x;
-      bl.y &= mhi.y;
-#pragma unroll
-      for (int dt = 0; dt < 4; ++dt)
-        acc_t2[dt] = mfma16(__builtin_bit_cast(bf16x4_t, pf[16 + dt]), __builtin_bit_cast(bf16x4_t, bl), acc_t2[dt]);
-    }
-    PROF_MARK(6)
-    if (!(a.dbg & 1)) {
-      const bf16_t* bs = ob + 15 + lane;
-#pragma unroll
-      for (int k = 0; k < 8; ++k)
-        dbd_pk[k] = (uint32_t)bs[(2 * k) * (OBP - 1)] | ((uint32_t)bs[(2 * k + 1) * (OBP - 1)] << 16);
-      dbd_j0 = j0;
-    }
-    wave_lds_sync();
-    slot_lo = slot_hi;
-    PROF_MARK(7)
-  }
-  store_dbd();
-
-  if (i < T) {
-    bf16_t* o1 = a.t1 + ((long)b * T + i) * a.ldt + h * DH;
-    bf16_t* o2 = a.t2 + ((long)b * T + i) * a.ldt + h * DH;
-#pragma unroll
-    for (int dt = 0; dt < 4; ++dt) {
-      uint2 pk;
-      pk.x = pack_bf2(acc_t1[dt][0] * a.scaling, acc_t1[dt][1] * a.scaling);
-      pk.y = pack_bf2(acc_t1[dt][2] * a.scaling, acc_t1[dt][3] * a.scaling);
-      *reinterpret_cast<uint2*>(o1 + dt * 16 + g4 * 4) = pk;
-      pk.x = pack_bf2(acc_t2[dt][0] * a.scaling, acc_t2[dt][1] * a.scaling);
-      pk.y = pack_bf2(acc_t2[dt][2] * a.scaling, acc_t2[dt][3] * a.scaling);
-      *reinterpret_cast<uint2*>(o2 + dt * 16 + g4 * 4) = pk;
-    }
-    if (a.dq) {
-      bf16_t* oq = a.dq + ((long)b * T + i) * a.lddq + h * DH;
-#pragma unroll
-      for (int dt = 0; dt < 4; ++dt) {
-        uint2 pk;
-        pk.x = pack_bf2((acc_t1[dt][0] + acc_t2[dt][0]) * a.scaling, (acc_t1[dt][1] + acc_t2[dt][1]) * a.scaling);
-        pk.y = pack_bf2((acc_t1[dt][2] + acc_t2[dt][2]) * a.scaling, (acc_t1[dt][3] + acc_t2[dt][3]) * a.scaling);
-        *reinterpret_cast<uint2*>(oq + dt * 16 + g4 * 4) = pk;
-      }
-    }
-  }
-  PROF_MARK(9)
-  if (!a.dbd_prezeroed) {
-    for (int iw = 0; iw < 16; ++iw) {
-      const int row = i0 + 16 * w + iw;
-      if (row >= T) break;
-      const int lo = T - 1 - row, hi = lo + jcov;
-      bf16_t* dr = a.dBD + ((long)z * T + row) * a.ld_bd;
-      for (int c = lane; c * 8 < a.ld_bd; c += 64) {
-        const int e0 = c * 8;
-        if (e0 + 8 <= lo || e0 >= hi) {
-          *reinterpret_cast<uint4*>(dr + e0) = make_uint4(0, 0, 0, 0);
-        } else if (e0 < lo || e0 + 8 > hi) {
-#pragma unroll
-          for (int e = 0; e < 8; ++e)
-            if (e0 + e < lo || e0 + e >= hi) dr[e0 + e] = 0;
-        }
-      }
-    }
-  }
-  PROF_MARK(8)
-  PROF_DUMP(0)
-}
-
-template <bool DROP>
-__global__ __launch_bounds__(256, 2) void rp_bwd_kv_kernel(const FlashBwdArgs a) {
+__global__ __launch_bounds__(256, 2) void rp_bwd_kernel(const FlashBwdArgs a) {
   __shared__ __attribute__((aligned(16))) char lds[LDS_BYTES_KV];
   const LaneK L = lane_consts();
   const int lane = L.lane, w = L.w, li = L.li, g4 = L.g4;
@@ -691,17 +443,16 @@
   const int kl = a.klen ? min(a.klen[b], T) : T;
   const int nq = (j0 < kl) ? a.nq : 0;
   const int nkt = a.nk;
-
-  bf16x8_t kf[4][2], vf[4][2];
+  const long C = (long)a.H * DH;
+  const long slab_q = (long)a.nk * a.B * T * C;
+
+  bf16x8_t vf[4][2];
 #pragma unroll
   for (int jt = 0; jt < 4; ++jt) {
     const int j = min(j0 + jt * 16 + li, T - 1);
     const long o = ((long)b * T + j) * a.ldkv + h * DH + g4 * 8;
 #pragma unroll
-    for (int ks = 0; ks < 2; ++ks) {
-      kf[jt][ks] = __builtin_bit_cast(bf16x8_t, *reinterpret_cast<const uint4*>(a.k + o + ks * 32));
-      vf[jt][ks] = __builtin_bit_cast(bf16x8_t, *reinterpret_cast<const uint4*>(a.v + o + ks * 32));
-    }
+    for (int ks = 0; ks < 2; ++ks) vf[jt][ks] = __builtin_bit_cast(bf16x8_t, *reinterpret_cast<const uint4*>(a.v + o + ks * 32));
   }
   f32x4_t acc_dk[4], acc_dv[4];
 #pragma unroll
@@ -709,6 +460,8 @@
     acc_dk[dt] = (f32x4_t){0.f, 0.f, 0.f, 0.f};
     acc_dv[dt] = (f32x4_t){0.f, 0.f, 0.f, 0.f};
   }
+  float cs1 = 0.f, cs2 = 0.f;
+  const bf16_t* Kb = a.k + (long)b * T * a.ldkv + h * DH;
   const bf16_t* Qub = a.qu + (long)b * T * a.ldq + h * DH;
   const bf16_t* Qvb = a.qv + (long)b * T * a.ldq + h * DH;
   const bf16_t* dOb = a.dout + (long)b * T * a.ldo + h * DH;
@@ -718,6 +471,7 @@
   const ImgSrc srcP = img_src(PPb, a.ldpp, R - 1, w, lane);
   const int pb0 = (T - 1) - (TQ - 1) + j0;
   float* bd = reinterpret_cast<float*>(lds + BNC_OFF + w * BNC);
+  bf16_t* ob = reinterpret_cast<bf16_t*>(bd);
   char* exw = lds + BNC_OFF + w * BNC;
   const uint32_t exo = li * 128 + ((((g4 >> 1) ^ swz(li))) << 4) + (g4 & 1) * 8;
   uint32_t exr[2], trk[2];
@@ -731,6 +485,19 @@
   const char* exbase = lds + BNC_OFF;
   const uint32_t* bitp = DROP ? reinterpret_cast<const uint32_t*>(a.bits) + (((long)z * nkt + kt) * (nkt * 64) + 16 * w + li) * 2 + (g4 >> 1) : nullptr;
   const int ksh = (g4 & 1) * 16;
+  uint2 mlo, mhi;
+  {
+    uint32_t m[4], n[4];
+#pragma unroll
+    for (int e = 0; e < 4; ++e) {
+      m[e] = (4 * g4 + e >= 15 - li) ? 0xffffu : 0u;
+      n[e] = (64 + 4 * g4 + e <= 78 - li) ? 0xffffu : 0u;
+    }
+    mlo = make_uint2(m[0] | (m[1] << 16), m[2] | (m[3] << 16));
+    mhi = make_uint2(n[0] | (n[1] << 16), n[2] | (n[3] << 16));
+  }
+  const int ob_w = li * (OBP - 1) + 15 + g4 * 4;
+  const char* ob_rd = reinterpret_cast<const char*>(ob) + li * (OBP * 2) + g4 * 8;
 
   bf16x8_t qv[2], qv_next[2];
   uint32_t piece_next = 0;
@@ -750,19 +517,15 @@
     issue_img(lds, srcQ, 0, w, lane);
     issue_img(lds + IMG, srcG, 0, w, lane);
     issue_img(lds + PP_OFF, srcP, pb0, w, lane);
-    issue_img(lds + PP_OFF + 2 * IMG, srcP, pb0 + 64, w, lane);
+    issue_img(lds + PP_OFF + IMG, srcP, pb0 + 64, w, lane);
+    issue_img(lds + K_OFF, img_src(Kb, a.ldkv, T - 1, w, lane), j0, w, lane);
     row_loads(0, 0);
   }
-  int slot_lo = 0;
-  PROF_DECL
   for (int it = 0; it < nq; ++it) {
     const int i0 = it * TQ;
-    PROF_MARK(9)
     asm volatile("s_waitcnt vmcnt(0)" ::: "memory");
     __builtin_amdgcn_s_barrier();
-    PROF_MARK(0)
-    const int slot_hi = slot_lo == 0 ? 2 : slot_lo - 1;
-    const int slot_nx = slot_lo == 2 ? 0 : slot_lo + 1;
+    const int slot_lo = it & 1, slot_hi = slot_lo ^ 1;
     qv[0] = qv_next[0];
     qv[1] = qv_next[1];
     const float* aux = reinterpret_cast<const float*>(lds + AUX_OFF + (it & 1) * 512) + 16 * w + li;
@@ -774,52 +537,142 @@
       qv[0] = __builtin_bit_cast(bf16x8_t, q0);
       qv[1] = __builtin_bit_cast(bf16x8_t, q1);
     }
-    const float lse2 = (i0 + 16 * w + li < T) ? lse_raw * LOG2E : INFINITY;
+    const int i = i0 + 16 * w + li;
+    const float lse2 = (i < T) ? lse_raw * LOG2E : INFINITY;
     if (it + 1 < nq) {
       row_loads(i0 + TQ, (it + 1) & 1);
       char* st = lds + ((it + 1) & 1) * 2 * IMG;
       issue_img(st, srcQ, i0 + TQ, w, lane);
       issue_img(st + IMG, srcG, i0 + TQ, w, lane);
-      issue_img(lds + PP_OFF + slot_nx * IMG, srcP, pb0 - 64 * (it + 1), w, lane);
-    }
-    PROF_MARK(1)
+    }
     const char* sQ = lds + (it & 1) * 2 * IMG;
     const char* sG = sQ + IMG;
-    bf16x8_t qu[2], dO[2];
-#pragma unroll
-    for (int ks = 0; ks < 2; ++ks) {
-      qu[ks] = ldf(sQ + w * 2048 + L.offk[ks]);
-      dO[ks] = ldf(sG + w * 2048 + L.offk[ks]);
-    }
-    f32x4_t acc_s[4], acc_dp[4];
+    const char* sK = lds + K_OFF;
+    const char* blk_lo = lds + PP_OFF + slot_lo * IMG;
+    const char* blk_hi = lds + PP_OFF + slot_hi * IMG;
+    bf16x4_t dsb[4], pdb[4];
+    {
+      bf16x8_t qu[2], dO[2];
+#pragma unroll
+      for (int ks = 0; ks < 2; ++ks) {
+        qu[ks] = ldf(sQ + w * 2048 + L.offk[ks]);
+        dO[ks] = ldf(sG + w * 2048 + L.offk[ks]);
+      }
+      f32x4_t acc_s[4], acc_dp[4];
+#pragma unroll
+      for (int jt = 0; jt < 4; ++jt) {
+        acc_s[jt] = (f32x4_t){0.f, 0.f, 0.f, 0.f};
+        acc_dp[jt] = (f32x4_t){0.f, 0.f, 0.f, 0.f};
+      }
+#pragma unroll
+      for (int ks = 0; ks < 2; ++ks)
+#pragma unroll
+        for (int jt = 0; jt < 4; ++jt) {
+          acc_s[jt] = mfma32(ldf(sK + jt * 2048 + L.offk[ks]), qu[ks], acc_s[jt]);
+          acc_dp[jt] = mfma32(vf[jt][ks], dO[ks], acc_dp[jt]);
+        }
+      add_band(acc_s, qv, blk_lo, blk_hi, bd, L);
+      softmax_bwd_tile<DROP, true>(acc_s, acc_dp, dsb, pdb, lse2, Di, a.inv_keep, piece, ksh, kl - j0, g4);
+    }
+    float* sp = a.slab + ((long)kt * a.B * T + (long)b * T + i) * C + h * DH + g4 * 4;
+    f32x4_t acc_t[4];
+#pragma unroll
+    for (int dt = 0; dt < 4; ++dt) acc_t[dt] = (f32x4_t){0.f, 0.f, 0.f, 0.f};
+    {
+      bf16x8_t kT[8];
+      tr_image(sK, L.tro, kT);
+#pragma unroll
+      for (int kb = 0; kb < 2; ++kb) {
+        const bf16x8_t db = cat(dsb[2 * kb], dsb[2 * kb + 1]);
+#pragma unroll
+        for (int dt = 0; dt < 4; ++dt) acc_t[dt] = mfma32(kT[dt * 2 + kb], db, acc_t[dt]);
+      }
+    }
+    if (a.t1) {
+      if (i < T) {
+#pragma unroll
+        for (int dt = 0; dt < 4; ++dt) *reinterpret_cast<f32x4_t*>(sp + dt * 16) = acc_t[dt];
+      }
+      sp += slab_q;
+    }
+    cs1 += colsum16(acc_t, li);
+    if (a.t1) {
+#pragma unroll
+      for (int dt = 0; dt < 4; ++dt) acc_t[dt] = (f32x4_t){0.f, 0.f, 0.f, 0.f};
+    }
+    wave_lds_sync();
 #pragma unroll
     for (int jt = 0; jt < 4; ++jt) {
-      acc_s[jt] = (f32x4_t){0.f, 0.f, 0.f, 0.f};
-      acc_dp[jt] = (f32x4_t){0.f, 0.f, 0.f, 0.f};
-    }
-#pragma unroll
-    for (int ks = 0; ks < 2; ++ks)
-#pragma unroll
-      for (int jt = 0; jt < 4; ++jt) {
-        acc_s[jt] = mfma32(kf[jt][ks], qu[ks], acc_s[jt]);
-        acc_dp[jt] = mfma32(vf[jt][ks], dO[ks], acc_dp[jt]);
-      }
-    PROF_MARK(2)
-    add_band(acc_s, qv, lds + PP_OFF + slot_lo * IMG, lds + PP_OFF + slot_hi * IMG, bd, L);
-    PROF_MARK(3)
-    bf16x4_t dsb[4], pdb[4];
-    softmax_bwd_tile<DROP, true>(acc_s, acc_dp, dsb, pdb, lse2, Di, a.inv_keep, piece, ksh, kl - j0, g4);
-    PROF_MARK(4)
+      const uint2 pk = __builtin_bit_cast(uint2, dsb[jt]);
+      ob[ob_w + jt * 16 + 0] = (bf16_t)(pk.x & 0xffffu);
+      ob[ob_w + jt * 16 + 1] = (bf16_t)(pk.x >> 16);
+      ob[ob_w + jt * 16 + 2] = (bf16_t)(pk.y & 0xffffu);
+      ob[ob_w + jt * 16 + 3] = (bf16_t)(pk.y >> 16);
+    }
+    wave_lds_sync();
+    {
+      auto blk16 = [&](int q16) -> uint32_t {
+        const int qq = q16 - w + 3;
+        return lds_addr(((qq >> 2) ? blk_hi : blk_lo) + (qq & 3) * 2048);
+      };
+#pragma unroll
+      for (int cb = 0; cb < 3; ++cb) {
+        uint32_t ad[8];
+        uint2 pf[8];
+        const uint32_t p0 = blk16(2 * cb), p1 = blk16(cb < 2 ? 2 * cb + 1 : 2 * cb);
+#pragma unroll
+        for (int dt = 0; dt < 4; ++dt) {
+          ad[dt] = p0 + L.tro[dt];
+          ad[4 + dt] = p1 + L.tro[dt];
+        }
+        trr8n(ad, pf);
+        if (cb < 2) {
+          uint2 blo = lds_u2(ob_rd + cb * 64);
+          const uint2 bhi = lds_u2(ob_rd + cb * 64 + 32);
+          if (cb == 0) {
+            blo.x &= mlo.x;
+            blo.y &= mlo.y;
+          }
+          const bf16x8_t db = cat2(blo, bhi);
+#pragma unroll
+          for (int dt = 0; dt < 4; ++dt) acc_t[dt] = mfma32(cat2(pf[dt], pf[4 + dt]), db, acc_t[dt]);
+        } else {
+          uint2 bl = lds_u2(ob_rd + 128);
+          bl.x &= mhi.x;
+          bl.y &= mhi.y;
+#pragma unroll
+          for (int dt = 0; dt < 4; ++dt)
+            acc_t[dt] = mfma16(__builtin_bit_cast(bf16x4_t, pf[dt]), __builtin_bit_cast(bf16x4_t, bl), acc_t[dt]);
+        }
+      }
+    }
+    {
+      const int j = j0 + lane, row_w = i0 + 16 * w, nrow = T - row_w;
+      const bf16_t* bs = ob + 15 + lane;
+      bf16_t* dp = a.dBD + ((long)z * T + row_w) * a.ld_bd + (T - 1 - row_w) + j;
+      if (j < T) {
+        if (nrow >= 16) {
+#pragma unroll
+          for (int iw = 0; iw < 16; ++iw) dp[(long)iw * (a.ld_bd - 1)] = bs[iw * (OBP - 1)];
+        } else {
+          for (int iw = 0; iw < nrow; ++iw) dp[(long)iw * (a.ld_bd - 1)] = bs[iw * (OBP - 1)];
+        }
+      }
+    }
+    if (i < T) {
+#pragma unroll
+      for (int dt = 0; dt < 4; ++dt) *reinterpret_cast<f32x4_t*>(sp + dt * 16) = acc_t[dt];
+    }
+    cs2 += colsum16(acc_t, li);
     wave_lds_sync();
 #pragma unroll
     for (int jt = 0; jt < 4; ++jt) {
       *reinterpret_cast<bf16x4_t*>(exw + (exo ^ (jt << 5))) = dsb[jt];
       *reinterpret_cast<bf16x4_t*>(exw + 2048 + (exo ^ (jt << 5))) = pdb[jt];
     }
-    PROF_MARK(5)
     asm volatile("s_waitcnt lgkmcnt(0)" ::: "memory");
     __builtin_amdgcn_s_barrier();
-    PROF_MARK(6)
+    if (it + 1 < nq) issue_img(lds + PP_OFF + slot_hi * IMG, srcP, pb0 - 64 * (it + 1), w, lane);
     {
       const uint32_t eb = lds_addr(exbase);
       const uint32_t ead[2] = {eb + exr[0], eb + exr[1]};
@@ -844,26 +697,134 @@
           }
       }
     }
-    slot_lo = slot_nx;
-    PROF_MARK(7)
-  }
-  const int j = j0 + 16 * w + li;
-  if (j < T) {
-    bf16_t* ok = a.dk + ((long)b * T + j) * a.lddkv + h * DH;
-    bf16_t* ov = a.dv + ((long)b * T + j) * a.lddkv + h * DH;
-#pragma unroll
-    for (int dt = 0; dt < 4; ++dt) {
+  }
+  {
+    const int j = j0 + 16 * w + li;
+    if (j < T) {
+      bf16_t* ok = a.dk + ((long)b * T + j) * a.lddkv + h * DH;
+      bf16_t* ov = a.dv + ((long)b * T + j) * a.lddkv + h * DH;
+#pragma unroll
+      for (int dt = 0; dt < 4; ++dt) {
+        uint2 pk;
+        pk.x = pack_bf2(acc_dk[dt][0], acc_dk[dt][1]);
+        pk.y = pack_bf2(acc_dk[dt][2], acc_dk[dt][3]);
+        *reinterpret_cast<uint2*>(ok + dt * 16 + g4 * 4) = pk;
+        pk.x = pack_bf2(acc_dv[dt][0], acc_dv[dt][1]);
+        pk.y = pack_bf2(acc_dv[dt][2], acc_dv[dt][3]);
+        *reinterpret_cast<uint2*>(ov + dt * 16 + g4 * 4) = pk;
+      }
+    }
+  }
+  if (a.bsum) {
+    __syncthreads();
+    float* red = reinterpret_cast<float*>(lds + BNC_OFF);
+    const int d = (li >> 2) * 16 + g4 * 4 + (li & 3);
+    red[w * 128 + d] = cs1;
+    red[w * 128 + 64 + d] = cs2 - cs1;
+    __syncthreads();
+    if (w == 0) {
+      float* o = a.bsum + ((long)z * a.nk + kt) * 128;
+      for (int k = lane; k < 128; k += 64) o[k] = ((red[k] + red[128 + k]) + red[256 + k]) + red[384 + k];
+    }
+  }
+  if (nq == 0) {
+    const int j = j0 + lane;
+    if (j < T)
+      for (int row = w; row < T; row += 4) a.dBD[((long)z * T + row) * a.ld_bd + (T - 1 - row) + j] = 0;
+  }
+  if (!a.dbd_prezeroed && kt == 0) {
+    for (int row = w; row < T; row += 4) {
+      const int lo = T - 1 - row, hi = lo + T;
+      bf16_t* dr = a.dBD + ((long)z * T + row) * a.ld_bd;
+      for (int c = lane; c * 8 < a.ld_bd; c += 64) {
+        const int e0 = c * 8;
+        if (e0 + 8 <= lo || e0 >= hi) {
+          *reinterpret_cast<uint4*>(dr + e0) = make_uint4(0, 0, 0, 0);
+        } else if (e0 < lo || e0 + 8 > hi) {
+#pragma unroll
+          for (int e = 0; e < 8; ++e)
+            if (e0 + e < lo || e0 + e >= hi) dr[e0 + e] = 0;
+        }
+      }
+    }
+  }
+}
+
+__global__ __launch_bounds__(256) void rp_delta_kernel(const FlashBwdArgs a) {
+  const long id = (long)blockIdx.x * 256 + threadIdx.x;
+  const long row = id >> 3;
+  const int part = (int)(id & 7);
+  if (row >= (long)a.H * a.B * a.T) return;
+  const int z = (int)(row / a.T), i = (int)(row % a.T);
+  const int h = z / a.B, b = z % a.B;
+  const long o = ((long)b * a.T + i) * a.ldo + h * DH + part * 8;
+  const uint4 g = *reinterpret_cast<const uint4*>(a.dout + o);
+  const uint4 x = *reinterpret_cast<const uint4*>(a.out + o);
+  const uint32_t wg[4] = {g.x, g.y, g.z, g.w}, wo[4] = {x.x, x.y, x.z, x.w};
+  float s = 0.f;
+#pragma unroll
+  for (int e = 0; e < 4; ++e)
+    s += __uint_as_float(wg[e] << 16) * __uint_as_float(wo[e] << 16) + __uint_as_float(wg[e] & 0xffff0000u) * __uint_as_float(wo[e] & 0xffff0000u);
+  s += __shfl_xor(s, 1, 64);
+  s += __shfl_xor(s, 2, 64);
+  s += __shfl_xor(s, 4, 64);
+  if (part == 0) a.D[row] = s;
+}
+
+constexpr int BIAS_OUT = 32, BIAS_SPLIT = 8;
+__global__ __launch_bounds__(256) void rp_bwd_finish_kernel(const FlashBwdArgs a, int nbias) {
+  const int T = a.T;
+  const long C = (long)a.H * DH;
+  if ((int)blockIdx.x < nbias) {
+    __shared__ float red[BIAS_SPLIT][BIAS_OUT];
+    const int h = blockIdx.x / (128 / BIAS_OUT), k = (blockIdx.x % (128 / BIAS_OUT)) * BIAS_OUT + (threadIdx.x % BIAS_OUT);
+    const int c = threadIdx.x / BIAS_OUT, ne = a.B * a.nk;
+    const float* src = a.bsum + (long)h * ne * 128 + k;
+    float s = 0.f;
+#pragma unroll 4
+    for (int e = c; e < ne; e += BIAS_SPLIT) s += src[(long)e * 128];
+    red[c][threadIdx.x % BIAS_OUT] = s;
+    __syncthreads();
+    if (threadIdx.x < BIAS_OUT) {
+      float t = 0.f;
+#pragma unroll
+      for (int q = 0; q < BIAS_SPLIT; ++q) t += red[q][threadIdx.x];
+      if (k < 64) a.dpos_u[h * DH + k] += t * a.scaling;
+      else a.dpos_v[h * DH + k - 64] += t * a.scaling;
+    }
+    return;
+  }
+  {
+    const long id = (long)(blockIdx.x - nbias) * 256 + threadIdx.x;
+    const long row = id / (C / 4);
+    const long col = (id % (C / 4)) * 4;
+    if (row >= (long)a.B * T) return;
+    const int b = (int)(row / T);
+    const int kl = a.klen ? min(a.klen[b], T) : T;
+    const int nkb = (kl + TK - 1) / TK;
+    const long kstep = (long)a.B * T * C, slab_q = (long)a.nk * kstep;
+    const float* p = a.slab + row * C + col;
+    f32x4_t s0 = (f32x4_t){0.f, 0.f, 0.f, 0.f}, s1 = s0;
+    const bool two = a.t1 != nullptr;
+    for (int kb = 0; kb < nkb; ++kb) {
+      s0 += *reinterpret_cast<const f32x4_t*>(p + kb * kstep);
+      if (two) s1 += *reinterpret_cast<const f32x4_t*>(p + slab_q + kb * kstep);
+    }
+    const float sc = a.scaling;
+    auto put = [&](bf16_t* dst, f32x4_t v) {
       uint2 pk;
-      pk.x = pack_bf2(acc_dk[dt][0], acc_dk[dt][1]);
-      pk.y = pack_bf2(acc_dk[dt][2], acc_dk[dt][3]);
-      *reinterpret_cast<uint2*>(ok + dt * 16 + g4 * 4) = pk;
-      pk.x = pack_bf2(acc_dv[dt][0], acc_dv[dt][1]);
-      pk.y = pack_bf2(acc_dv[dt][2], acc_dv[dt][3]);
-      *reinterpret_cast<uint2*>(ov + dt * 16 + g4 * 4) = pk;
-    }
-  }
-  PROF_MARK(8)
-  PROF_DUMP(1)
+      pk.x = pack_bf2(v[0] * sc, v[1] * sc);
+      pk.y = pack_bf2(v[2] * sc, v[3] * sc);
+      *reinterpret_cast<uint2*>(dst) = pk;
+    };
+    if (two) {
+      put(a.t1 + row * a.ldt + col, s0);
+      if (a.t2) put(a.t2 + row * a.ldt + col, s1);
+      if (a.dq) put(a.dq + row * a.lddq + col, s0 + s1);
+    } else if (a.dq) {
+      put(a.dq + row * a.lddq + col, s0);
+    }
+  }
 }
 
 }
@@ -895,54 +856,21 @@
   return EA_CHECK_LAUNCH();
 }
 
-int ea_rp_bwd(const FlashBwdArgs& a_in, hipStream_t stream) {
-  static const int dbg = [] { const char* e = getenv("EA_RP_DBG"); return e ? atoi(e) : 0; }();
-  FlashBwdArgs a = a_in;
-  a.dbg = dbg;
-  a.prof = nullptr;
-#ifdef RP_PROF
-  static unsigned long long* prof_buf = nullptr;
-  static const int prof_on = [] { const char* e = getenv("EA_RP_PROF"); return e && e[0] == '1' ? 1 : 0; }();
-  if (prof_on) {
-    if (!prof_buf) hipMalloc(&prof_buf, 2 * 8192 * 10 * sizeof(unsigned long long));
-    hipMemsetAsync(prof_buf, 0, 2 * 8192 * 10 * sizeof(unsigned long long), stream);
-    a.prof = prof_buf;
-  }
-#endif
-  const dim3 gq((unsigned)(a.nq * a.H * a.B)), gk((unsigned)(a.nk * a.H * a.B));
-  if (a.thr) {
-    hipLaunchKernelGGL(rp_bwd_q_kernel<true>, gq, dim3(256), 0, stream, a);
-    hipLaunchKernelGGL(rp_bwd_kv_kernel<true>, gk, dim3(256), 0, stream, a);
-  } else {
-    hipLaunchKernelGGL(rp_bwd_q_kernel<false>, gq, dim3(256), 0, stream, a);
-    hipLaunchKernelGGL(rp_bwd_kv_kernel<false>, gk, dim3(256), 0, stream, a);
-  }
-#ifdef RP_PROF
-  if (a.prof) {
-    static int calls = 0;
-    if (++calls == 20) {
-      hipStreamSynchronize(stream);
-      static unsigned long long h[2 * 8192 * 10];
-      hipMemcpy(h, a.prof, sizeof(h), hipMemcpyDeviceToHost);
-      const char* names[2] = {"Q ", "KV"};
-      const int nw[2] = {(int)gq.x * 4, (int)gk.x * 4};
-      for (int k = 0; k < 2; ++k) {
-        double sum[10] = {0};
-        int cnt = 0;
-        for (int wv = 0; wv < nw[k] && wv < 8192; ++wv) {
-          const unsigned long long* o = h + ((long)k * 8192 + wv) * 10;
-          unsigned long long tot = 0;
-          for (int p = 0; p < 10; ++p) tot += o[p];
-          if (!tot) continue;
-          ++cnt;
-          for (int p = 0; p < 10; ++p) sum[p] += (double)o[p];
-        }
-        fprintf(stderr, "[rp prof] %s waves %d, mean s_memtime ticks per wave by phase:", names[k], cnt);
-        for (int p = 0; p < 10; ++p) fprintf(stderr, " p%d=%.0f", p, cnt ? sum[p] / cnt : 0.0);
-        fprintf(stderr, "\n");
-      }
-    }
-  }
-#endif
+long ea_rp_bwd_workspace_bytes(int H, int B, int T, bool t12) {
+  const long nk = (T + TK - 1) / TK;
+  const long slab = (t12 ? 2 : 1) * nk * B * T * (long)H * DH * (long)sizeof(float);
+  return ((slab + 255) & ~255L) + (long)H * B * nk * 128 * (long)sizeof(float);
+}
+
+int ea_rp_bwd(const FlashBwdArgs& a, hipStream_t stream) {
+  const long rows = (long)a.H * a.B * a.T;
+  hipLaunchKernelGGL(rp_delta_kernel, dim3((unsigned)((rows * 8 + 255) / 256)), dim3(256), 0, stream, a);
+  const dim3 grid((unsigned)(a.nk * a.H * a.B));
+  if (a.thr) hipLaunchKernelGGL(rp_bwd_kernel<true>, grid, dim3(256), 0, stream, a);
+  else hipLaunchKernelGGL(rp_bwd_kernel<false>, grid, dim3(256), 0, stream, a);
+  const long quads = (long)a.B * a.T * a.H * (DH / 4);
+  const int nrowblk = (int)((quads + 255) / 256);
+  const int nbias = a.bsum ? a.H * (128 / BIAS_OUT) : 0;
+  hipLaunchKernelGGL(rp_bwd_finish_kernel, dim3((unsigned)(nbias + nrowblk)), dim3(256), 0, stream, a, nbias);
   return EA_CHECK_LAUNCH();
 }
diff --git a/espresso_amd/kernels.py b/espresso_amd/kernels.py
--- a/espresso_amd/kernels.py
+++ b/espresso_amd/kernels.py
@@ -256,6 +256,23 @@
     return t1, t2, dBD
 
 
+def flash_relpos_bwd(qu, qv, k, v, pp, key_len, out, dout, lse, dq, dk, dv, dpos_u, dpos_v, H, B, T, ldq, ldkv, lddq, lddkv,
+                     ldpp=0, scaling=1.0, drop_p=0.0, drop_seed=0, keep_bits=None, dbd_prezeroed=False):
+    dh = 64
+    Rp = (2 * T - 1 + 7) // 8 * 8
+    dBD = torch.empty(H * B * T, Rp, dtype=torch.bfloat16, device=qu.device)
+    D = torch.empty(H * B, T, dtype=torch.float32, device=qu.device)
+    ws = torch.empty(int(_lib.lib().ea_flash_relpos_bwd_workspace_bytes(H, B, T)), dtype=torch.uint8, device=qu.device)
+    thr, scale = drop_params(drop_p)
+    check(
+        _lib.lib().ea_flash_relpos_bwd(_p(qu), _p(qv), ldq, _p(k), _p(v), ldkv, _p(pp), ldpp, _p(key_len), _p(out), _p(dout), H * dh,
+                                       _p(lse), _p(D), _p(dBD), Rp, _p(dq), lddq, _p(dk), _p(dv), lddkv, _p(dpos_u), _p(dpos_v), H, B,
+                                       T, 2 if dbd_prezeroed else 0, scaling, drop_seed, thr, scale, _p(keep_bits), _p(ws), _stream()),
+        "ea_flash_relpos_bwd",
+    )
+    return dBD
+
+
 def relpos_softmax_bwd(P, dPd, H, B, T, S, ld_p, ld_dp, ld_bd, want_bd=True, drop_p=0.0, drop_seed=0):
     dAC = torch.empty(H * B * T, ld_p, dtype=torch.bfloat16, device=P.device)
     dBD = torch.empty(H * B * T, ld_bd, dtype=torch.bfloat16, device=P.device) if want_bd else None
diff --git a/include/espresso_amd.h b/include/espresso_amd.h
--- a/include/espresso_amd.h
+++ b/include/espresso_amd.h
@@ -135,6 +135,12 @@
                            void* dv, long lddkv, int H, int B, int T, int S, int dh, int causal, float scaling,
                            uint64_t drop_seed, uint32_t drop_thr, float drop_scale, const void* keep_bits,
                            void* dq, long lddq, ea_stream_t stream);
+long ea_flash_relpos_bwd_workspace_bytes(int H, int B, int T);
+int ea_flash_relpos_bwd(const void* qu, const void* qv, long ldq, const void* k, const void* v, long ldkv, const void* pp,
+                        long ldpp, const int* key_len, const void* out, const void* dout, long ldo, const float* lse, float* D,
+                        void* dBD, int ld_bd, void* dq, long lddq, void* dk, void* dv, long lddkv, float* dpos_u, float* dpos_v,
+                        int H, int B, int T, int flags, float scaling, uint64_t drop_seed, uint32_t drop_thr, float drop_scale,
+                        const void* keep_bits, void* workspace, ea_stream_t stream);
 
 int ea_relpos_q_prep(const void* qkv, long ldq, const float* u, const float* v, void* qu, void* qv, int M,
                      int C, float scaling, ea_stream_t stream);
```
